# Hydr10n/DirectX-Physically-Based-Raytracer

Hardware: AMD Instinct MI355X
Metric: Mrays/s per GPU + frames/s at 1080p, Cornell Box 4spp/8bounce (higher is better)
Workload: dtype f32

## Files before the change

### directx-physically-based-raytracer_amd/csrc/pt_api.hip

```cpp
#include "pt_internal.hpp"

#include <cmath>
#include <cstdio>
#include <cstring>

using namespace pt;

static thread_local std::string g_createError;
namespace pt { std::string& create_error() { return g_createError; } }

int pt::fail(Context* c, int status, const std::string& msg)
{
    if (c) c->lastError = msg; else g_createError = msg;
    return status;
}
int pt::fail_hip(Context* c, hipError_t e, const char* what)
{
    return fail(c, e == hipErrorOutOfMemory ? PT_ERROR_OUT_OF_MEMORY : PT_ERROR_HIP, std::string(what) + ": " + hipGetErrorString(e));
}

static int poll_tlas_header(Context& c, bool wait);

extern "C" {

// ... 438 lines not shown
        const hipError_t es = hipStreamSynchronize(c.stream);
        if (e == hipSuccess) e = es;
    }
    if (e != hipSuccess) {
        if (newCopy) (void)hipStreamSynchronize(c.stream);
        return fail_hip(&c, e, "top-level build");
    }

    if (newBlob) c.blobDev = std::move(newCopy);
    for (Blas* b : adopting) { b->nodes.reset(); b->tris.reset(); b->idx.reset(); b->inBlob = true; }
    for (const auto& p : P.pieces) if (p.b->inBlob) { p.b->blobNodeAt = P.node_at(p); p.b->blobTriAt = P.tri_at(p); p.b->blobIdxAt = P.idx_at(p); }
    c.tlasHeaderPending = true;
    c.tlasNodeReserve = P.tlasNodeCap;
    SceneRefs& r = c.scene;
    r.instances = c.tlas.instances.data(); r.instanceCount = count; r.triangleCount = P.tris;
    r.blob.base = (const f4v*)c.blobDev.data();
    r.blob.nodeOff16 = (uint32_t)(P.nodeAt / 16); r.blob.triOff16 = (uint32_t)(P.triAt / 16); r.blob.idxOff16 = (uint32_t)(P.idxAt / 16);
    r.blob.instOff16 = (uint32_t)(P.instAt / 16); r.blob.leafInstOff16 = (uint32_t)(P.leafAt / 16); r.blob.enterOff16 = (uint32_t)(P.enterAt / 16);
    r.blob.instCount = count; r.blob.nodeCount = P.blobNodes; r.blob.triCount = P.blobTris; r.blob.bytes = (uint32_t)P.total;
    r.blasTable = dTable; r.blasTableCount = (uint32_t)P.table.size(); r.instSource = dSrc; r.blasTableMaxTris = 0;
    for (const BlasEntry& te : P.table) r.blasTableMaxTris = std::max(r.blasTableMaxTris, te.triCount);
    c.tlasBlasIds = P.pieceIds;
    if (P.objectEnd != c.tlasObjectEnd || count != c.tlasValidatedCount || P.bindingHash != c.tlasBindingHash) c.validated = false;
    c.tlasObjectEnd = P.objectEnd; c.tlasValidatedCount = count; c.tlasBindingHash = P.bindingHash;
    if (P.lightHash != c.tlasLightHash) c.lightListValid = false;
    c.tlasLightHash = P.lightHash;
    c.normalsShared = c.validated && c.sharedVerdict;
    c.haveTlas = true;
    return PT_OK;
}

int pt_share_scene(PtContext* ctx, PtContext* source)
{
    if (!ctx || !source || ctx == source) return PT_ERROR_INVALID_ARGUMENT;
    Context& c = ctx->c; Context& s = source->c;
    API_ARG(&c, c.device == s.device, "both contexts must live on the same device");
    API_ARG(&c, c.viewers.empty(), "other contexts view this context's scene");
    API_ARG(&c, !s.sceneOwner, "the source views another context's scene itself: share from the owner");
    API_HIP(&c, hipSetDevice(c.device));
    API_HIP(&c, hipStreamSynchronize(s.stream));
    API_HIP(&c, hipStreamSynchronize(c.stream));
    int st = poll_tlas_header(s, true);
    if (st != PT_OK) return fail(&c, st, s.lastError);
    if (!s.haveTlas) return fail(&c, PT_ERROR_NOT_READY, "the source context has no top-level acceleration structure");
    if (c.sceneOwner) detach_from_owner(c);
    else { API_HIP(&c, materialise_adopted(c)); c.tlas = Tlas(); c.blobDev.reset(); }
    drop_tlas(c);
    c.scene = s.scene;
    c.tlasObjectEnd = s.tlasObjectEnd; c.maxBlasDepth = s.maxBlasDepth;
    c.heapHost = s.heapHost; c.heapDirty = true;
    c.objects = s.objects; c.objectCount = s.objectCount; c.instanceData = s.instanceData; c.instanceDataCount = s.instanceDataCount;
    c.sceneOwner = &s; s.viewers.push_back(&c);
    c.tlasHeaderPending = false; c.validated = false;
    c.haveTlas = true;
    return PT_OK;
}

int pt_get_accel_stats(PtContext* ctx, PtAccelStats* out)
{
    if (!ctx || !out) return PT_ERROR_INVALID_ARGUMENT;
    Context& c = ctx->c;
    API_HIP(&c, hipSetDevice(c.device));
    API_HIP(&c, hipStreamSynchronize(c.stream));
    int st = poll_tlas_header(c, true);
    if (st != PT_OK) return st;
    memset(out, 0, sizeof *out);
    out->InstanceCount = c.scene.instanceCount;
    out->BottomLevelCount = (uint32_t)c.blas.size();
    out->TriangleCount = c.scene.triangleCount;
    out->NodeSizeBytes = sizeof(WideNode); out->TriangleSizeBytes = sizeof(TriPacket);
    uint64_t nb = (uint64_t)wide_node_capacity(c.scene.instanceCount) * sizeof(WideNode), tb = 0;
    for (auto& kv : c.blas) { nb += (uint64_t)kv.second.nodeCount * sizeof(WideNode); tb += (uint64_t)kv.second.triCount * sizeof(TriPacket); out->MaxBottomLevelDepth = std::max(out->MaxBottomLevelDepth, kv.second.depth); }
    out->BlobBytes = c.sceneOwner ? 0 : c.scene.blob.bytes;
    out->SharedScene = c.sceneOwner ? 1u : 0u;
    out->NormalRecords = c.normalsShared ? 1u : 0u;
    out->RoundObjectsInLds = round_objects_in_lds(c, c.objectCount, (bool)c.shadeGeomDev);
    out->RoundRecordsInLds = round_records_in_lds(c, c.objectCount, (bool)c.shadeGeomDev);
    if (c.tlasHeaderHost && !c.tlasHeaderPending) out->TopLevelDepth = c.tlasHeaderHost.data()->depth;
    out->NodeBytes = nb; out->TriangleBytes = tb;
    for (auto& kv : c.blas) if (!kv.second.inBlob) out->OwnedBottomLevelBytes += (uint64_t)kv.second.nodeCount * sizeof(WideNode) + (uint64_t)kv.second.triCount * (sizeof(TriPacket) + 16);
    return PT_OK;
}

int pt_set_camera(PtContext* ctx, const PtCamera* camera)
{
    if (!ctx) return PT_ERROR_INVALID_ARGUMENT;
    API_ARG(&ctx->c, camera, "camera is NULL");
    ctx->c.camera = *camera; ctx->c.haveCamera = true;
    return PT_OK;
}
int pt_set_scene_data(PtContext* ctx, const PtSceneData* scene_data)
{
    if (!ctx) return PT_ERROR_INVALID_ARGUMENT;
    API_ARG(&ctx->c, scene_data, "scene_data is NULL");
    ctx->c.sceneData = *scene_data; ctx->c.haveSceneData = true;
    return PT_OK;
}
int pt_set_object_data(PtContext* ctx, const PtObjectData* device_objects, uint32_t count)
{
    if (!ctx) return PT_ERROR_INVALID_ARGUMENT;
    API_ARG(&ctx->c, device_objects || count == 0, "device_objects is NULL");
    ctx->c.objects = device_objects; ctx->c.objectCount = count;
    return PT_OK;
}
int pt_invalidate_object_data(PtContext* ctx)
{
    if (!ctx) return PT_ERROR_INVALID_ARGUMENT;
    ctx->c.validated = false; ctx->c.normalsShared = false; ctx->c.sharedVerdict = false;
    ctx->c.objectDataGen++;
    return PT_OK;
}
int pt_set_instance_data(PtContext* ctx, const PtInstanceData* device_instances, uint32_t count)
{
    if (!ctx) return PT_ERROR_INVALID_ARGUMENT;
    ctx->c.instanceData = device_instances; ctx->c.instanceDataCount = count;
    return PT_OK;
}

int pt_set_sharding(PtContext* ctx, const PtSharding* s)
{
    if (!ctx) return PT_ERROR_INVALID_ARGUMENT;
    API_ARG(&ctx->c, s && s->RankCount >= 1 && s->RankIndex < s->RankCount && s->BandHeight >= 1, "invalid sharding");
    ctx->c.sharding = *s;
    return PT_OK;
}

int pt_local_rows(const PtSharding* s, uint32_t frame_height, uint32_t* out_rows)
{
    if (!s || !out_rows || s->RankCount == 0 || s->BandHeight == 0 || s->RankIndex >= s->RankCount) return PT_ERROR_INVALID_ARGUMENT;
    uint32_t rows = 0;
    for (uint32_t b = s->RankIndex; (uint64_t)b * s->BandHeight < frame_height; b += s->RankCount) {
        uint32_t y0 = b * s->BandHeight;
        rows += (frame_height - y0 < s->BandHeight) ? frame_height - y0 : s->BandHeight;
    }
    *out_rows = rows;
    return PT_OK;
}

int pt_deinterleave_bands(PtContext* ctx, void* dst_full, const void* gathered, const uint64_t* rank_offsets_host, uint32_t rank_count,
                          uint32_t band_height, uint32_t width, uint32_t height, uint32_t pixel_bytes)
{
    if (!ctx) return PT_ERROR_INVALID_ARGUMENT;
    Context& c = ctx->c;
    API_ARG(&c, dst_full && gathered && rank_offsets_host && rank_count >= 1 && band_height >= 1, "invalid de-interleave arguments");
    API_ARG(&c, pixel_bytes % 4 == 0, "pixel size must be a multiple of 4 bytes");
    API_HIP(&c, hipSetDevice(c.device));
    API_ARG(&c, rank_count <= 64, "at most 64 ranks");
    hipError_t e = launch_deinterleave(c.stream, dst_full, gathered, rank_offsets_host, rank_count, band_height, width, height, pixel_bytes);
    if (e != hipSuccess) return fail_hip(&c, e, "de-interleave");
    return PT_OK;
}

}

static int validate_scene(Context& c)
{
    if (c.validated && c.validatedObjects == c.objects && c.validatedObjectCount == c.objectCount) return PT_OK;
    const uint32_t heapCount = (uint32_t)c.heapHost.size();
    if (c.tlasObjectEnd > c.objectCount)
        return fail(&c, PT_ERROR_INVALID_ARGUMENT, "InstanceID + geometry count of an instance reaches ObjectData[" + std::to_string(c.tlasObjectEnd - 1)
                    + "] but only " + std::to_string(c.objectCount) + " objects are bound (pt_set_object_data)");
    if (c.instanceData && c.instanceDataCount < c.scene.instanceCount)
        return fail(&c, PT_ERROR_INVALID_ARGUMENT, "InstanceData holds fewer records than the top level has instances");
    uint32_t sharedMismatch = 0;
    if (c.objectCount) {
        API_HIP(&c, c.validateDev.reserve(8));
// ... 274 lines not shown
```

### directx-physically-based-raytracer_amd/csrc/pt_internal.hpp

```cpp
#pragma once
#include <hip/hip_runtime.h>

#include <algorithm>
#include <map>
#include <string>
#include <type_traits>
#include <vector>

#include "../../include/ptamd.h"
#include "pt_memory.hpp"
#include "pt_trace2.hpp"
#include "pt_sharc.hpp"

namespace pt {

struct WideHeader { uint32_t nodeCount, itemCount, depth, error; };

struct TreeBuffers {
    DeviceBuffer<float4> boxLo, boxHi; DeviceBuffer<uint32_t> bounds;
    DeviceBuffer<uint64_t> keys, keysSorted; DeviceBuffer<uint32_t> index, indexSorted;
    DeviceBuffer<uint8_t> sortTemp; size_t sortTempBytes = 0;
    DeviceBuffer<uint64_t> leafKeys; DeviceBuffer<float4> leafLo, leafHi;
    DeviceBuffer<int2> children; DeviceBuffer<int> parentInternal, parentLeaf;
    DeviceBuffer<float4> nodeLo, nodeHi; DeviceBuffer<uint32_t> arrival;
// ... 41 lines not shown

struct SceneView {
    AccelView accel;
    const PtObjectData* objects;
    const ShadeGeom* shadeGeom;
    const HeapEntry* shadeTex;
    const PtInstanceData* instanceData;
    const HeapEntry* heap;
    const float* srgbLut;
    uint32_t objectCount, heapCount;
};

struct FrameView {
    uint32_t width, height;
    uint32_t localRows;
    uint32_t rankIndex, rankCount, bandHeight;
};

struct PathQueue {
    float4* s0;
    float4* s1;
    float4* s2;
    float4* r0;
    float4* r1;
    uint4*  hit;
};

constexpr uint32_t kSubQueueShiftFused = 5, kSubQueueShiftStream = 7, kSubQueuesMax = 1u << kSubQueueShiftStream;

struct FrameConstants { PtCamera cam; PtSceneData sd; PtGraphicsSettings gs; };
struct RoundArgs;

struct DeviceCounters {
    unsigned long long primaryRays, secondaryRays, nodesVisited, trianglesTested;
    unsigned int mismatchCount, stackOverflows;
    float mismatchRay[16];
    unsigned int maxNodesPerRay, _pad2;
};

struct Context {
    int device = 0;
    hipStream_t stream = nullptr;
    std::string lastError;

    std::vector<HeapEntry> heapHost;
    DeviceBuffer<HeapEntry> heapDev; bool heapDirty = true;
    DeviceBuffer<float> srgbLutDev;
    bool heapHasTextures = false;

    std::map<uint64_t, Blas> blas; uint64_t nextBlasId = 1;
    TreeBuffers buildScratch;
    Tlas tlas; bool haveTlas = false;
    DeviceBuffer<uint8_t> blobDev;
    SceneRefs scene;
    Context* sceneOwner = nullptr;
    std::vector<Context*> viewers;
    uint32_t framesInFlight = 1;
    std::vector<uint64_t> tlasBlasIds;
    std::vector<uint8_t> tlasUploadHost; DeviceBuffer<uint8_t> tlasUploadDev;
    struct UploadStage { PinnedBuffer<uint8_t> host; Event event; };
    UploadStage tlasStage[2]; uint32_t tlasStageNext = 0;
    PinnedBuffer<WideHeader> tlasHeaderHost; Event tlasHeaderEvent; bool tlasHeaderPending = false;
    uint32_t maxBlasDepth = 0, tlasNodeReserve = 0;
    uint32_t tlasValidatedCount = ~0u, persistentGrid = 0;
    uint64_t tlasBindingHash = 0;
    uint64_t tlasObjectEnd = 0;
    DeviceBuffer<ShadeGeom> shadeGeomDev;
    DeviceBuffer<HeapEntry> shadeTexDev;
    DeviceBuffer<uint4> shadeRecA; DeviceBuffer<uint32_t> shadeRecB;
    bool normalsShared = false;
    bool sharedVerdict = false;
    bool validated = false; DeviceBuffer<uint32_t> validateDev;
    const void* validatedObjects = nullptr; uint32_t validatedObjectCount = 0;

    PtCamera camera{}; PtSceneData sceneData{}; PtGraphicsSettings settings{};
    bool haveCamera = false, haveSceneData = false, haveSettings = false;
    const PtObjectData* objects = nullptr; uint32_t objectCount = 0;
    const PtInstanceData* instanceData = nullptr; uint32_t instanceDataCount = 0;
    PtSharding sharding{0, 1, 16, 0};

    DeviceBuffer<uint4> queueArrays[2][6];
    PathQueue queue[2]{};
    DeviceBuffer<uint4> primaryRecords;
    DeviceBuffer<float2> pixelAux;
    DeviceBuffer<FrameConstants> frameConstants;
    GraphExec graphExec; std::string graphKey; bool disableGraphs = false;
    static constexpr uint32_t kMaxChains = 4;
    uint32_t chains = 0;
    Stream chainStream[kMaxChains - 1]; Event chainFork, chainJoin[kMaxChains - 1];
    GraphExec chainGraph[kMaxChains]; std::string chainGraphKey;
    DeviceBuffer<uint32_t> queueCounts;
    DeviceBuffer<RoundArgs> roundArgs; std::string roundArgsKey;
    DeviceBuffer<DeviceCounters> counters;
    uint64_t lastIterations = 0;
    uint32_t debugFlags = 0;

    void* comm = nullptr; bool commOwned = false; uint32_t commRank = 0, commWorld = 1;

    bool timing = false;
    std::vector<Event> evExtend, evShade, evRound;
    uint32_t nExtend = 0, nShade = 0, nRound = 0;

    PtDISettings diSettings{}; bool haveDISettings = false;
    uint64_t tlasLightHash = 0;
    uint32_t objectDataGen = 0;
    DeviceBuffer<uint4> lightList; uint32_t lightCount = 0;
    DeviceBuffer<uint32_t> lightInstStart;
    uint64_t lightListKey = 0; bool lightListValid = false;
    DeviceBuffer<PtTriangleLight> lightRecords; DeviceBuffer<float> lightCdf, lightBlockSums; uint32_t lightRecordCount = 0;
    PtDIResamplingSettings diReuse{}; bool diReuseOn = false;
    DeviceBuffer<PtDIReservoir> diResA, diResB;
    DeviceBuffer<int8_t> diOffsets;
    bool diHistoryValid = false; uint32_t diHistorySize[2] = {0, 0}; uint64_t diHistoryLightKey = 0; uint32_t diResCount = 0;
    PtDIVisibilitySettings diVisibility{}; bool diVisibilityOn = false;
    PtDILightSamplingSettings diSampling{};
    DeviceBuffer<PtDIPresampledLight> diTiles, diCells;
    uint32_t diTileCount = 0, diCellCount = 0;

    PtPostProcessSettings post{}; bool havePost = false;
    DeviceBuffer<ushort4> postLevels;
    uint32_t postDims[9][2] = {};
    size_t postOffset[9] = {};

    PtSHARCSettings sharcSettings{}; bool haveSharcSettings = false;
    uint32_t sharcCapacity = 0, sharcParity = 0;
    DeviceBuffer<unsigned long long> sharcKeys;
    DeviceBuffer<uint4> sharcVoxels[2];
    DeviceBuffer<SharcView> sharcView;
    DeviceBuffer<float> sharcRough[2];
    DeviceBuffer<PtSHARCPathScatter> sharcLogScatter;
    DeviceBuffer<PtSHARCPathVertex> sharcLog; uint32_t sharcLogPaths = 0, sharcLogBounces = 0;
};

std::string& create_error();
int fail(Context* c, int status, const std::string& msg);
int fail_hip(Context* c, hipError_t e, const char* what);
#define API_HIP(ctx, expr) do { hipError_t e_ = (expr); if (e_ != hipSuccess) return pt::fail_hip(ctx, e_, #expr); } while (0)
#define API_ARG(ctx, cond, msg) do { if (!(cond)) return pt::fail(ctx, PT_ERROR_INVALID_ARGUMENT, msg); } while (0)
int make_views(Context& c, uint32_t width, uint32_t height, SceneView& sv, FrameView& fv, bool needFrameInputs = true);
int check_raytrace_args(Context& c, const PtTextures* tx);

template <typename T>
int download_counted(Context& c, const T* src, uint32_t count, uint32_t row, T* host_dst, uint32_t capacity, uint32_t* out_count, uint32_t* out_row = nullptr)
{
    API_HIP(&c, hipSetDevice(c.device));
    API_HIP(&c, hipStreamSynchronize(c.stream));
    *out_count = count;
    if (out_row) *out_row = row;
    const size_t n = std::min((size_t)capacity, (size_t)count * row);
    if (n) API_HIP(&c, hipMemcpy(host_dst, src, sizeof(T) * n, hipMemcpyDeviceToHost));
    return PT_OK;
}

template <typename F> void with_flags(F&& f) { f(); }
template <typename F, typename... Rest> void with_flags(F&& f, bool first, Rest... rest)
{
    if (first) with_flags([&](auto... bs) { f(std::true_type{}, bs...); }, rest...);
    else with_flags([&](auto... bs) { f(std::false_type{}, bs...); }, rest...);
}

hipError_t build_blas_device(const PtGeometryDesc* geoms, uint32_t ngeoms, bool allowUpdate, hipStream_t stream, Blas& out);
hipError_t refit_blas_device(const PtGeometryDesc* geoms, uint32_t ngeoms, hipStream_t stream, Blas& b);
hipError_t build_tlas_prepare(Tlas& out, uint32_t n);
hipError_t build_tlas_device(const InstanceRecord* dInstances, const float* const* dBlasBounds, uint32_t n, hipStream_t stream, Tlas& out);
hipError_t launch_instance_records(const InstanceSource* src, const BlasEntry* table, uint32_t n, InstanceRecord* rec, const float** bounds, uint32_t* sceneBounds, hipStream_t stream);
hipError_t launch_blob_assembly(const InstanceRecord* inst, const Tlas& tlas, const BlasEntry* table, uint32_t n, InstanceT* outInst,
                                InstanceT* outLeafInst, const BlobCopy* jobs, uint32_t njobs, f4v* outEnter, hipStream_t stream);
__host__ __device__ void invert_3x4(const float m[12], float out[12]);

hipError_t launch_skin(hipStream_t stream, const void* skeletal, const float* transforms, void* vertices, void* motion, uint32_t count);

struct FramePlan {
    uint32_t rounds, segCap, grid, sqShift;
    bool streaming, fused, first;
    bool flat, lds;
    uint32_t ldsFixed, roundLds, extend2Lds;
    uint32_t objectsInLds, recordsInLds;
    bool recordsUsable;
    bool writeT, stats, di, textured, sharc;
    float2* aux;
    uint32_t nsq() const { return 1u << sqShift; }
    uint32_t cstride() const { return 3u * nsq(); }
};

hipError_t launch_shade(Context& c, const FramePlan& p, const SceneView& sv, const FrameView& fv, const PtTextures& tx, uint32_t round, uint32_t grid, hipStream_t stream,
                        uint32_t sqBase, uint32_t sqCount);
hipError_t launch_extend_stream(Context& c, const FramePlan& p, const AlphaContext& ac, uint32_t round, hipStream_t stream, uint32_t sqBase, uint32_t sqCount);

hipError_t launch_gbuffer(Context& c, const SceneView& sv, const FrameView& fv, uint32_t flags, const PtTextures& tx);
hipError_t launch_raytrace(Context& c, const SceneView& sv, const FrameView& fv, const PtTextures& tx, bool sharcQuery);
hipError_t launch_visibility(Context& c, const SceneView& sv, const void* rays, uint32_t count, void* out);
hipError_t launch_bsdf_evaluate(hipStream_t stream, const float* q, uint32_t count, float* r);
hipError_t launch_bsdf_sample(hipStream_t stream, const float* q, uint32_t count, float* r);
hipError_t launch_debug_trace(Context& c, const SceneView& sv, const float* ray8, uint32_t* devLog, uint32_t logCap);
hipError_t launch_debug_closest(Context& c, const SceneView& sv, const void* rays, uint32_t count, void* hits);
uint32_t round_objects_in_lds(const Context& c, uint32_t objectCount, bool haveShadeGeom);
uint32_t round_records_in_lds(const Context& c, uint32_t objectCount, bool haveShadeGeom);
inline bool normal_records_usable(const Context& c) { return c.normalsShared && c.scene.blasTable && c.scene.blasTableCount <= 65535u  && c.shadeRecB && c.scene.blob.triCount && c.scene.blob.triCount <= c.shadeRecB.capacity(); }
hipError_t launch_check_shared_geometry(hipStream_t stream, const InstanceSource* src, const BlasEntry* table, uint32_t n, const ShadeGeom* shadeGeom, uint32_t* out);
hipError_t launch_validate_objects(hipStream_t stream, const PtObjectData* objects, uint32_t count, const HeapEntry* heap, uint32_t heapCount, uint32_t* out, ShadeGeom* shadeGeom, HeapEntry* shadeTex);
hipError_t launch_deinterleave(hipStream_t stream, void* dst, const void* src, const uint64_t* rankOffsetsHost, uint32_t rankCount,
                               uint32_t bandHeight, uint32_t width, uint32_t height, uint32_t pixelBytes);

}

struct PtContext { pt::Context c; };
```

### directx-physically-based-raytracer_amd/csrc/pt_kernels.hip

```cpp
#include "pt_internal.hpp"

#include <cstring>

#include "pt_shade.hpp"

namespace pt {

template <bool STATS, bool TEXTURED, int MODE>
__global__ __launch_bounds__(256) void k_gbuffer(SceneView sv, FrameView fv, PtCamera cam, PtSceneData sd, uint32_t flags, PtTextures tx,
                                                 BlobView bv, DeviceCounters* counters)
{
    const uint32_t wv = threadIdx.x >> 6, ln = threadIdx.x & 63u;
    const uint32_t x = blockIdx.x * 16 + (wv & 1u) * 8u + (ln & 7u), ly = blockIdx.y * 16 + (wv >> 1) * 8u + (ln >> 3);
    const bool valid = x < fv.width && ly < fv.localRows;
    if (MODE == 0 && !valid) return;
    const uint32_t y = global_row(fv, valid ? ly : 0u);
    const size_t pi = (size_t)ly * fv.width + x;

    float4 Position = make_float4(INFINITY, INFINITY, INFINITY, INFINITY);
    float LinearDepth = INFINITY, NormalizedDepth = cam.IsNormalizedDepthReversed ? 0.0f : 1.0f;
    float u, v;
    const RayDesc ray = generate_pinhole_ray(cam, valid ? x : 0u, y, fv.width, fv.height, u, v);
    TraceStats st; st.nodes = 0; st.tris = 0; st.overflow = 0;
    Hit hit;
// ... 45 lines not shown
            float proj[4]; xform4(cam.WorldToProjection, h.Position, proj);
            LinearDepth = proj[3];
            NormalizedDepth = proj[2] / proj[3];
            if ((flags & PT_GB_MotionVector) && tx.MotionVector) {
                v3 prev = h.Position;
                if (!sd.IsStatic && sv.instanceData) {
                    const float* P = sv.instanceData[h.InstanceIndex].PreviousObjectToWorld; v3 q = h.ObjectPosition;
                    const PtMeshDescriptors md = sv.objects[h.ObjectIndex].MeshDescriptors;
                    if (md.MotionVectors != ~0u) {
                        const PT_GLOBAL_AS uint16_t* mvb = gptr<uint16_t>(sv.heap[md.MotionVectors].ptr);
                        const HeapEntry ib = sv.heap[md.Indices];
                        v3 m3[3];
                        for (int kk = 0; kk < 3; kk++) {
                            const uint32_t vi = load_index_dev(ib.ptr, ib.stride, 3 * h.PrimitiveIndex + kk);
                            m3[kk] = V3(f16_to_f32(mvb[4 * (size_t)vi]), f16_to_f32(mvb[4 * (size_t)vi + 1]), f16_to_f32(mvb[4 * (size_t)vi + 2]));
                        }
                        q = q + interp3(m3[0], m3[1], m3[2], hit.u, hit.v);
                    }
                    prev = V3(sop3t(P[0], q.x, P[1], q.y, P[2], q.z, P[3]), sop3t(P[4], q.x, P[5], q.y, P[6], q.z, P[7]), sop3t(P[8], q.x, P[9], q.y, P[10], q.z, P[11]));
                }
                float clip[4], view[4];
                xform4(cam.PreviousWorldToProjection, prev, clip);
                xform4(cam.PreviousWorldToView, prev, view);
                float su = (clip[0] / clip[3]) * 0.5f + 0.5f, svv = (clip[1] / clip[3]) * -0.5f + 0.5f;
                ushort4 mv = make_ushort4(f32_to_f16((su - u) * (float)fv.width), f32_to_f16((svv - v) * (float)fv.height), f32_to_f16(view[2] - LinearDepth), 0);
                ((ushort4*)tx.MotionVector)[pi] = mv;
            }
        }
        BSDFSample bs; bs.Roughness = 0.0f;
        if (flags & PT_GB_Material) {
            const PtMaterial m = surface_material<TEXTURED>(sv, h);
            bs.Initialize(V3(m.BaseColor), m.Metallic, m.Roughness, m.IOR, m.Transmission, h.IsFrontFace);
            if (tx.BaseColorMetalness)
                ((uchar4*)tx.BaseColorMetalness)[pi] = make_uchar4(f32_to_unorm8(bs.BaseColor.x), f32_to_unorm8(bs.BaseColor.y), f32_to_unorm8(bs.BaseColor.z), f32_to_unorm8(bs.Metallic));
            if (flags & PT_GB_Albedo) {
                const float NoV = fabsf(dot(h.ShadingNormal, -ray.d));
                const v3 Fe = ml_env_term_rtg(bs.F0, NoV, bs.Roughness);
                if ((flags & PT_GB_DiffuseAlbedo) && tx.DiffuseAlbedo)
                    ((ushort4*)tx.DiffuseAlbedo)[pi] = make_ushort4(f32_to_f16((1.0f - Fe.x) * bs.Albedo.x * 0.99f + 0.01f), f32_to_f16((1.0f - Fe.y) * bs.Albedo.y * 0.99f + 0.01f),
                                                                     f32_to_f16((1.0f - Fe.z) * bs.Albedo.z * 0.99f + 0.01f), 0);
                if ((flags & PT_GB_SpecularAlbedo) && tx.SpecularAlbedo)
                    ((ushort4*)tx.SpecularAlbedo)[pi] = make_ushort4(f32_to_f16(Fe.x * 0.99f + 0.01f), f32_to_f16(Fe.y * 0.99f + 0.01f), f32_to_f16(Fe.z * 0.99f + 0.01f), 0);
            }
            if (tx.IOR) ((uint16_t*)tx.IOR)[pi] = f32_to_f16(m.IOR);
            if (bs.Metallic < 1.0f && tx.Transmission) ((uint8_t*)tx.Transmission)[pi] = f32_to_unorm8(bs.Transmission);
            if ((flags & PT_GB_Radiance) && tx.Radiance) {
                v3 e = material_emission(m);
                ((ushort4*)tx.Radiance)[pi] = make_ushort4(f32_to_f16(e.x), f32_to_f16(e.y), f32_to_f16(e.z), 0);
            }
        }
        if ((flags & PT_GB_NormalRoughness) && tx.NormalRoughness) {
            float r = (flags & PT_GB_Material) ? bs.Roughness : 0.0f;
            ((short4*)tx.NormalRoughness)[pi] = make_short4(f32_to_snorm16(h.ShadingNormal.x), f32_to_snorm16(h.ShadingNormal.y), f32_to_snorm16(h.ShadingNormal.z), f32_to_snorm16(r));
        }
    } else {
        if ((flags & PT_GB_MotionVector) && tx.MotionVector) {
            v3 far = ray.o + ray.d * 1e8f;
            float proj[4], clip[4], view[4];
            xform4(cam.WorldToProjection, far, proj);
            xform4(cam.PreviousWorldToProjection, far, clip);
            xform4(cam.PreviousWorldToView, far, view);
            float su = (clip[0] / clip[3]) * 0.5f + 0.5f, svv = (clip[1] / clip[3]) * -0.5f + 0.5f;
            ((ushort4*)tx.MotionVector)[pi] = make_ushort4(f32_to_f16((su - u) * (float)fv.width), f32_to_f16((svv - v) * (float)fv.height), f32_to_f16(view[2] - proj[3]), 0);
        }
        if ((flags & PT_GB_Radiance) && tx.Radiance) {
            v3 e = environment_light_color(sv, sd, ray.d);
            ((ushort4*)tx.Radiance)[pi] = make_ushort4(f32_to_f16(e.x), f32_to_f16(e.y), f32_to_f16(e.z), 0);
        }
    }
    if ((flags & PT_GB_Position) && tx.Position) ((float4*)tx.Position)[pi] = Position;
    if ((flags & PT_GB_LinearDepth) && tx.LinearDepth) ((float*)tx.LinearDepth)[pi] = LinearDepth;
    if ((flags & PT_GB_NormalizedDepth) && tx.NormalizedDepth) ((float*)tx.NormalizedDepth)[pi] = NormalizedDepth;
}

__global__ void k_set_constants(FrameConstants v, FrameConstants* dst, uint32_t* queueCounts, uint32_t countWords)
{
    const uint32_t* s = (const uint32_t*)&v; uint32_t* d = (uint32_t*)dst;
    for (uint32_t i = threadIdx.x; i < sizeof(FrameConstants) / 4; i += blockDim.x) d[i] = s[i];
    for (uint32_t i = threadIdx.x; i < countWords; i += blockDim.x) queueCounts[i] = 0u;
}


__global__ __launch_bounds__(256) void k_pt_init(FrameView fv, const FrameConstants* __restrict__ fc, PtTextures tx, PathQueue q, float2* aux, uint32_t segCap, uint32_t* countFresh,
                                                 uint4* __restrict__ primary, uint32_t sqShift)
{
    __shared__ uint32_t lds[8];
    const PtGraphicsSettings& gs = fc->gs;
    const uint32_t npix = fv.width * fv.localRows;
    const uint32_t nsq = 1u << sqShift, sq = blockIdx.x & (nsq - 1u), bq = blockIdx.x >> sqShift, nbq = gridDim.x >> sqShift;
    for (uint32_t j = bq; (j * nsq + sq) * 256u < npix; j += nbq) {
        const uint32_t p = (j * nsq + sq) * 256u + threadIdx.x;
        bool alive = false;
        if (p < npix) alive = isfinite(((const float*)tx.Position)[4 * (size_t)p + 3]);
        const uint32_t slot = sq * segCap + (segCap - 1u - block_reserve(alive, &countFresh[sq], lds));
        if (alive) {
            const uint32_t x = p % fv.width, y = global_row(fv, p / fv.width);
            q.s0[slot] = make_float4(1.0f, 1.0f, 1.0f, __uint_as_float(p));
            q.s1[slot] = make_float4(0.0f, 0.0f, 0.0f, __uint_as_float(rng_init(x, y, gs.FrameIndex)));
            q.s2[slot] = make_float4(0.0f, 0.0f, 0.0f, __uint_as_float(0u));
            if (aux) aux[p] = make_float2(INFINITY, 1.0f);
            const uint2 nr = ((const uint2*)tx.NormalRoughness)[p], rad = ((const uint2*)tx.Radiance)[p];
            primary[3 * (size_t)p] = ((const uint4*)tx.Position)[p];
            primary[3 * (size_t)p + 1] = make_uint4(nr.x, nr.y, ((const uint32_t*)tx.FlatNormal)[p], ((const uint32_t*)tx.GeometricNormal)[p]);
            primary[3 * (size_t)p + 2] = make_uint4(((const uint32_t*)tx.BaseColorMetalness)[p], rad.x, rad.y,
                                                    (uint32_t)((const uint16_t*)tx.IOR)[p] | ((uint32_t)((const uint8_t*)tx.Transmission)[p] << 16));
        }
    }
}

template <bool DI, bool SHARC = false>
__global__ __launch_bounds__(256) void k_pt_first(FrameView fv, const FrameConstants* __restrict__ fc, PtTextures tx, PathQueue qout, float2* aux,
                                                                                             uint32_t segCap, uint32_t* countOut, uint4* __restrict__ primary, uint32_t sqShift,
                                                                                             float* roughOut = nullptr)
{
    __shared__ uint32_t lds[32];
    uint32_t emits = 0;
    const PtCamera& cam = fc->cam; const PtGraphicsSettings& gs = fc->gs;
    const uint32_t npix = fv.width * fv.localRows;
    const uint32_t nsq = 1u << sqShift, sq = blockIdx.x & (nsq - 1u), bq = blockIdx.x >> sqShift, nbq = gridDim.x >> sqShift;
    const uint32_t seg = sq * segCap;
    for (uint32_t j = bq; (j * nsq + sq) * 256u < npix; j += nbq) {
        const uint32_t pix = (j * nsq + sq) * 256u + threadIdx.x;
        bool alive = false;
        if (pix < npix) alive = isfinite(((const float*)tx.Position)[4 * (size_t)pix + 3]);
        bool toTraced = false, toFresh = false;
        PathRegs p; p.thr = V3(1.0f, 1.0f, 1.0f); p.srad = V3(0, 0, 0); p.rsum = V3(0, 0, 0); p.pixel = pix; p.rng = 0; p.sample = 0; p.bounce = 0;
        v3 newO = V3(0, 0, 0), newD = V3(0, 0, 1);
        float pr = 0.0f;
        if (alive) {
            const uint32_t x = pix % fv.width, y = global_row(fv, pix / fv.width);
            p.rng = rng_init(x, y, gs.FrameIndex);
            if (aux) aux[pix] = make_float2(INFINITY, 1.0f);
            const uint2 nr = ((const uint2*)tx.NormalRoughness)[pix], rad = ((const uint2*)tx.Radiance)[pix];
            const uint4 r0 = ((const uint4*)tx.Position)[pix];
            const uint4 r1 = make_uint4(nr.x, nr.y, ((const uint32_t*)tx.FlatNormal)[pix], ((const uint32_t*)tx.GeometricNormal)[pix]);
            const uint4 r2 = make_uint4(((const uint32_t*)tx.BaseColorMetalness)[pix], rad.x, rad.y,
                                        (uint32_t)((const uint16_t*)tx.IOR)[pix] | ((uint32_t)((const uint8_t*)tx.Transmission)[pix] << 16));
            primary[3 * (size_t)pix] = r0; primary[3 * (size_t)pix + 1] = r1; primary[3 * (size_t)pix + 2] = r2;
            shade_fresh_record<DI, SHARC>(fv, cam, gs, tx, aux, r0, r1, r2, p, toTraced, toFresh, newO, newD, &pr);
        }
        emit_tile<SHARC>(qout, seg, segCap, &countOut[sq], &countOut[nsq + sq], lds + ((emits++ & 1u) << 4), toTraced, toFresh, p, newO, newD, roughOut, pr);
    }
}

__global__ __launch_bounds__(256) void k_extend_brute(AccelView av, BlobView bv, AlphaContext ac, PathQueue q, uint32_t segCap, const uint32_t* count, DeviceCounters* counters, uint32_t sqShift)
{
    const uint32_t nsq = 1u << sqShift, sq = blockIdx.x & (nsq - 1u), bq = blockIdx.x >> sqShift, nbq = gridDim.x >> sqShift;
    const uint32_t n = count[sq];
    if (bq == 0 && threadIdx.x == 0) atomicAdd(&counters->secondaryRays, (unsigned long long)n);
    __shared__ uint2 ldsStack[kLdsStackDepth * 256];
    uint2 spill[kStackSize - kLdsStackDepth];
    GroupStack<kLdsStackDepth> stack; stack.init((PT_LDS_AS void*)ldsStack, spill);
    BlobReader<false> blob; blob.p = bv.base;
    TraceStats st; st.nodes = 0; st.tris = 0; st.overflow = 0;
    for (uint32_t local = bq * 256u + threadIdx.x; local < n; local += nbq * 256u) {
        const uint32_t i = sq * segCap + local;
        const float4 o = q.r0[i], d = q.r1[i];
        const Hit h = trace_brute_force(av, ac, V3(o.x, o.y, o.z), V3(d.x, d.y, d.z), o.w, d.w);
        const Hit b = trace_single<false, false, false>(blob, bv, ac, V3(o.x, o.y, o.z), V3(d.x, d.y, d.z), o.w, d.w, stack, &st, nullptr);
        if (b.inst != h.inst || (h.inst != ~0u && (b.slot != h.slot || b.u != h.u || b.v != h.v))) {
            if (atomicAdd(&counters->mismatchCount, 1u) == 0u) {
                float* m = counters->mismatchRay;
                m[0] = o.x; m[1] = o.y; m[2] = o.z; m[3] = o.w; m[4] = d.x; m[5] = d.y; m[6] = d.z; m[7] = d.w;
                m[8] = __uint_as_float(b.inst); m[9] = __uint_as_float(b.slot); m[10] = b.t; m[11] = 0.0f;
                m[12] = __uint_as_float(h.inst); m[13] = __uint_as_float(h.slot); m[14] = h.t; m[15] = 0.0f;
            }
        }
        q.hit[i] = make_uint4(h.inst, h.slot, __float_as_uint(h.u), __float_as_uint(h.v));
    }
    if (st.overflow) atomicAdd(&counters->stackOverflows, st.overflow);
}

constexpr int kStackLds2 = 8;
constexpr uint32_t kStackLds2Bytes = (uint32_t)kStackLds2 * 256u * 8u;
constexpr uint32_t kExtendLdsFixed = kStackLds2Bytes + (uint32_t)kCandidates * 256u * 4u + 4u * kPhasedWaveLds;
constexpr uint32_t kBlobLdsMax = 40u * 1024u;

template <bool STATS, bool LDS, bool WRITE_T = false, bool FLAT = false>
__global__ __launch_bounds__(256) void k_extend2(BlobView bv, AlphaContext ac, PathQueue q, uint32_t segCap, const uint32_t* count, DeviceCounters* counters, uint32_t sqShift)
{
    extern __shared__ __attribute__((aligned(16))) unsigned char smem[];
    constexpr uint32_t kFixed = FLAT ? kFlatLdsFixed : kExtendLdsFixed;
    const uint32_t nsq = 1u << sqShift, sq = blockIdx.x & (nsq - 1u), bq = blockIdx.x >> sqShift, nbq = gridDim.x >> sqShift;
    const uint32_t n = count[sq];
    if (bq == 0 && threadIdx.x == 0) atomicAdd(&counters->secondaryRays, (unsigned long long)n);
    if (bq * 256u >= n) return;
    PT_LDS_AS void* ldsStack = (PT_LDS_AS void*)smem;
    BlobReader<LDS> blob;
    if constexpr (LDS) {
        f4v* dst = (f4v*)(smem + kFixed);
        const uint32_t n16 = bv.bytes / 16u;
        for (uint32_t i = threadIdx.x; i < n16; i += 256u) dst[i] = bv.base[i];
        __syncthreads();
        blob.p = (const PT_LDS_AS f4v*)(smem + kFixed);
    } else {
        blob.p = bv.base;
    }
    TraceStats st; st.nodes = 0; st.tris = 0; st.overflow = 0;
    if constexpr (FLAT) {
        unsigned char* ldsWave = smem + (uint32_t)kStackLdsFlat * 256u * 8u + (threadIdx.x >> 6) * kFlatWaveLds;
        for (uint32_t base = bq * 256u; base < n; base += nbq * 256u) {
            const uint32_t local = base + threadIdx.x;
            const bool valid = local < n;
            const uint32_t i = sq * segCap + (valid ? local : base);
            float4 o = q.r0[i], d = q.r1[i];
            if (!valid) { o.w = 1.0f; d.w = 0.0f; }
            const Hit h = trace_closest_flat<STATS, LDS>(blob, bv, ac, V3(o.x, o.y, o.z), V3(d.x, d.y, d.z), o.w, d.w, ldsStack, ldsWave, &st);
            if (valid) {
                q.hit[i] = make_uint4(h.inst, h.slot, __float_as_uint(h.u), __float_as_uint(h.v));
                if (WRITE_T) q.r1[i].w = h.t;
            }
        }
    } else {
        uint32_t* ldsCand = (uint32_t*)(smem + kStackLds2Bytes);
        unsigned char* ldsWave = smem + kStackLds2Bytes + (uint32_t)kCandidates * 256u * 4u + (threadIdx.x >> 6) * kPhasedWaveLds;
        for (uint32_t base = bq * 256u; base < n; base += nbq * 256u) {
            const uint32_t local = base + threadIdx.x;
            const bool valid = local < n;
            const uint32_t i = sq * segCap + (valid ? local : base);
            float4 o = q.r0[i], d = q.r1[i];
            if (!valid) { o.w = 1.0f; d.w = 0.0f; }
            const Hit h = trace_closest_v2<STATS, LDS, kStackLds2>(blob, bv, ac, V3(o.x, o.y, o.z), V3(d.x, d.y, d.z), o.w, d.w, ldsStack, ldsCand, ldsWave, &st);
            if (valid) {
                q.hit[i] = make_uint4(h.inst, h.slot, __float_as_uint(h.u), __float_as_uint(h.v));
                if (WRITE_T) q.r1[i].w = h.t;
            }
        }
    }
    if (STATS) { atomicAdd(&counters->nodesVisited, (unsigned long long)st.nodes); atomicAdd(&counters->trianglesTested, (unsigned long long)st.tris); }
    if (st.overflow) atomicAdd(&counters->stackOverflows, st.overflow);
}

struct RoundArgs {
    SceneView sv; FrameView fv; PtTextures tx; BlobView bv; PathQueue qin, qout;
    const FrameConstants* fc; float2* aux; const uint32_t* countIn; uint32_t* countOut; DeviceCounters* counters; uint32_t segCap;
    uint32_t objectsInLds;
    const uint4* recA; const uint32_t* recB;
    uint32_t recordsInLds, sqShift;
    const uint4* primary;
    const SharcView* sharc; const float* roughIn; float* roughOut;
};

template <bool TEXTURED, bool LDS, bool FLAT, bool DI, bool SHARC = false>
__global__ __launch_bounds__(256) __attribute__((amdgpu_waves_per_eu(4, 4))) void k_round(const RoundArgs* __restrict__ A, uint32_t sqBase, uint32_t sqCount)
{
    const SceneView& sv = A->sv; const FrameView& fv = A->fv; const PtTextures& tx = A->tx; const BlobView& bv = A->bv;
    const PathQueue& qin = A->qin; const PathQueue& qout = A->qout;
    const FrameConstants* __restrict__ fc = A->fc; float2* aux = A->aux; const uint32_t segCap = A->segCap;
    const uint32_t* countIn = A->countIn; uint32_t* countOut = A->countOut; DeviceCounters* counters = A->counters;
    const uint4* __restrict__ primary = A->primary;
    extern __shared__ __attribute__((aligned(16))) unsigned char smem[];
    __shared__ uint32_t lds[32];
    uint32_t emits = 0;
    constexpr uint32_t kFixed = FLAT ? kFlatLdsFixed : kExtendLdsFixed;
    const PtCamera& cam = fc->cam; const PtSceneData& sd = fc->sd; const PtGraphicsSettings& gs = fc->gs;
    const uint32_t sqShift = A->sqShift;
    const uint32_t nsq = 1u << sqShift, bq = blockIdx.x / sqCount, sq = sqBase + (blockIdx.x - bq * sqCount), nbq = gridDim.x / sqCount;
    const uint32_t nT = countIn[sq], nF = countIn[nsq + sq];
    const uint32_t seg = sq * segCap;
    if (bq == 0 && threadIdx.x == 0) atomicAdd(&counters->secondaryRays, (unsigned long long)nT);

#ifdef PT_ROUND_PROF
    RoundProf profData; RoundProf* prof = &profData;
    for (int k = 0; k < 16; k++) profData.acc[k] = 0;
    profData.last = __builtin_readcyclecounter();
#else
    RoundProf* prof = nullptr;
#endif
    if (bq * 256u < nT) {
        PT_LDS_AS void* ldsStack = (PT_LDS_AS void*)smem;
        BlobReader<LDS> blob;
        ShadeTables tables;
        tables.recA = A->recA; tables.recB = A->recB;
        if constexpr (LDS) {
            f4v* dst = (f4v*)(smem + kFixed);
            const uint32_t n16 = bv.bytes / 16u;
            for (uint32_t k = threadIdx.x; k < n16; k += 256u) dst[k] = bv.base[k];
            const uint32_t nobj = A->objectsInLds;
            for (uint32_t k = threadIdx.x; k < nobj * kObjLds16; k += 256u) {
                const uint32_t o = k / kObjLds16, part = k - o * kObjLds16;
                dst[n16 + k] = part < 2u ? ((const f4v*)&sv.shadeGeom[o])[part] : ((const f4v*)&sv.objects[o].Material)[part - 2u];
            }
            const uint32_t nrec = A->recordsInLds, recBase = n16 + nobj * kObjLds16;
            for (uint32_t k = threadIdx.x; k < nrec; k += 256u) {
                const uint4 a = A->recA[k];
                dst[recBase + k] = (f4v){ __uint_as_float(a.x), __uint_as_float(a.y), __uint_as_float(a.z), __uint_as_float(a.w) };
                ((uint32_t*)(dst + recBase + nrec))[k] = A->recB[k];
            }
            __syncthreads();
            blob.p = (const PT_LDS_AS f4v*)(smem + kFixed);
            if (nobj) tables.objects = (ObjectTableLds)(smem + kFixed) + n16;
            if (nrec) { tables.recALds = (const PT_LDS_AS f4v*)(smem + kFixed) + recBase; tables.recBLds = (const PT_LDS_AS uint32_t*)((const PT_LDS_AS f4v*)(smem + kFixed) + recBase + nrec); }
        } else {
            blob.p = bv.base;
        }
        const AlphaContext ac = alpha_context(sv);
        TraceStats st; st.nodes = 0; st.tris = 0; st.overflow = 0;
        for (uint32_t base = bq * 256u; base < nT; base += nbq * 256u) {
            const uint32_t local = base + threadIdx.x;
            const bool valid = local < nT;
            const uint32_t i = seg + (valid ? local : base);
            float4 o = qin.r0[i], d = qin.r1[i];
            PathRegs p = load_path(qin, i);
            float pr = 0.0f;
            if constexpr (SHARC) pr = A->roughIn[i];
            if (!valid) { o.w = 1.0f; d.w = 0.0f; }
            PT_PROF_MARK(prof, 0);
            Hit h;
            if constexpr (FLAT) {
                unsigned char* ldsWave = smem + (uint32_t)kStackLdsFlat * 256u * 8u + (threadIdx.x >> 6) * kFlatWaveLds;
                h = trace_closest_flat<false, LDS>(blob, bv, ac, V3(o.x, o.y, o.z), V3(d.x, d.y, d.z), o.w, d.w, ldsStack, ldsWave, &st, prof);
            } else {
                uint32_t* ldsCand = (uint32_t*)(smem + kStackLds2Bytes);
                unsigned char* ldsWave = smem + kStackLds2Bytes + (uint32_t)kCandidates * 256u * 4u + (threadIdx.x >> 6) * kPhasedWaveLds;
                h = trace_closest_v2<false, LDS, kStackLds2>(blob, bv, ac, V3(o.x, o.y, o.z), V3(d.x, d.y, d.z), o.w, d.w, ldsStack, ldsCand, ldsWave, &st);
            }
            bool toTraced = false, toFresh = false;
            v3 newO = V3(0, 0, 0), newD = V3(0, 0, 1);
            if (valid) {
                shade_traced<TEXTURED, DI, SHARC>(sv, GeometryFromBlob<LDS>{ blob, bv, tables }, sd, gs, tx, aux, p, make_uint4(h.inst, h.slot, __float_as_uint(h.u), __float_as_uint(h.v)), h.t,
                                       V3(d.x, d.y, d.z), toTraced, toFresh, newO, newD, prof, A->sharc, &pr);
            }
            PT_PROF_MARK(prof, 6);
            emit_tile<SHARC>(qout, seg, segCap, &countOut[sq], &countOut[nsq + sq], lds + ((emits++ & 1u) << 4), toTraced, toFresh, p, newO, newD, A->roughOut, pr);
            PT_PROF_MARK(prof, 7);
#ifdef PT_ROUND_PROF
            prof->acc[11] += 1u;
#endif
        }
        if (st.overflow) atomicAdd(&counters->stackOverflows, st.overflow);
    }
    for (uint32_t tile = bq; tile * 256u < nF; tile += nbq) {
        const uint32_t local = tile * 256u + threadIdx.x;
        bool toTraced = false, toFresh = false;
        PathRegs p; v3 newO = V3(0, 0, 0), newD = V3(0, 0, 1);
        float pr = 0.0f;
        if (local < nF) {
            p = load_path(qin, seg + (segCap - 1u - local));
            PT_PROF_WAIT(); PT_PROF_MARK(prof, 12);
            shade_fresh<DI, SHARC>(fv, cam, gs, tx, aux, primary, p, toTraced, toFresh, newO, newD, prof, &pr);
        }
        PT_PROF_MARK(prof, 14);
        emit_tile<SHARC>(qout, seg, segCap, &countOut[sq], &countOut[nsq + sq], lds + ((emits++ & 1u) << 4), toTraced, toFresh, p, newO, newD, A->roughOut, pr);
        PT_PROF_MARK(prof, 15);
    }
#ifdef PT_ROUND_PROF
    PT_PROF_MARK(prof, 8);
    if ((threadIdx.x & 63u) == 0u) for (int k = 0; k < 16; k++) atomicAdd((unsigned int*)&counters->mismatchRay[k], (k < 9 || k >= 12) ? (prof->acc[k] >> 6) : prof->acc[k]);
#endif
}

template <bool STATS>
__global__ __launch_bounds__(256) void k_extend(BlobView bv, AlphaContext ac, PathQueue q, uint32_t segCap, const uint32_t* count, DeviceCounters* counters, uint32_t sqShift)
{
    const uint32_t nsq = 1u << sqShift, sq = blockIdx.x & (nsq - 1u), bq = blockIdx.x >> sqShift, nbq = gridDim.x >> sqShift;
    const uint32_t n = count[sq];
    if (bq == 0 && threadIdx.x == 0) atomicAdd(&counters->secondaryRays, (unsigned long long)n);
    __shared__ uint2 ldsStack[kLdsStackDepth * 256];
    uint2 spill[kStackSize - kLdsStackDepth];
    GroupStack<kLdsStackDepth> stack; stack.init((PT_LDS_AS void*)ldsStack, spill);
    BlobReader<false> blob; blob.p = bv.base;
    TraceStats st; st.nodes = 0; st.tris = 0; st.overflow = 0;
    for (uint32_t local = bq * 256u + threadIdx.x; local < n; local += nbq * 256u) {
        const uint32_t i = sq * segCap + local;
        const float4 o = q.r0[i], d = q.r1[i];
        const Hit h = trace_single<STATS, false, false>(blob, bv, ac, V3(o.x, o.y, o.z), V3(d.x, d.y, d.z), o.w, d.w, stack, &st, nullptr);
        q.hit[i] = make_uint4(h.inst, h.slot, __float_as_uint(h.u), __float_as_uint(h.v));
    }
    if (STATS) { atomicAdd(&counters->nodesVisited, (unsigned long long)st.nodes); atomicAdd(&counters->trianglesTested, (unsigned long long)st.tris); }
    if (st.overflow) atomicAdd(&counters->stackOverflows, st.overflow);
}

static uint32_t persistent_grid(Context& c);

__global__ __launch_bounds__(256) void k_visibility(BlobView bv, AlphaContext ac, const float4* __restrict__ rays, uint32_t count, float4* __restrict__ out,
                                                    DeviceCounters* counters)
{
    __shared__ uint2 ldsStack[kLdsStackDepth * 256];
    uint2 spill[kStackSize - kLdsStackDepth];
    GroupStack<kLdsStackDepth> stack; stack.init((PT_LDS_AS void*)ldsStack, spill);
    BlobReader<false> blob; blob.p = bv.base;
    TraceStats st; st.nodes = 0; st.tris = 0; st.overflow = 0;
    for (uint32_t i = blockIdx.x * blockDim.x + threadIdx.x; i < count; i += gridDim.x * blockDim.x) {
        const float4 o = rays[2 * (size_t)i], d = rays[2 * (size_t)i + 1];
        v3 vis;
        const Hit h = trace_single<false, false, true>(blob, bv, ac, V3(o.x, o.y, o.z), V3(d.x, d.y, d.z), o.w, d.w, stack, &st, &vis);
        out[i] = make_float4(vis.x, vis.y, vis.z, h.inst == ~0u ? 1.0f : 0.0f);
    }
    if (st.overflow) atomicAdd(&counters->stackOverflows, st.overflow);
}

__global__ __launch_bounds__(256) void k_debug_trace(BlobView bv, AlphaContext ac, float4 o, float4 d, uint32_t* log, uint32_t logCap)
{
    __shared__ uint2 ldsStack[kLdsStackDepth * 256];
    uint2 spill[kStackSize - kLdsStackDepth];
    GroupStack<kLdsStackDepth> stack; stack.init((PT_LDS_AS void*)ldsStack, spill);
    BlobReader<false> blob; blob.p = bv.base;
    TraceStats st; st.nodes = 0; st.tris = 0; st.overflow = 0;
    const float a = 0.02f * (float)threadIdx.x, ca = cosf(a), sa = sinf(a);
    const v3 dd = V3(d.x * ca - d.z * sa, d.y, d.x * sa + d.z * ca);
    trace_single<false, false, false, GroupStack<kLdsStackDepth>, true>(blob, bv, ac, V3(o.x, o.y, o.z), dd, o.w, d.w, stack, &st, nullptr, log, threadIdx.x == 0 ? logCap : 0u);
}

hipError_t launch_debug_trace(Context& c, const SceneView& sv, const float* ray8, uint32_t* devLog, uint32_t logCap)
{
    k_debug_trace<<<1, 256, 0, c.stream>>>(c.scene.blob, alpha_context(sv), make_float4(ray8[0], ray8[1], ray8[2], ray8[3]), make_float4(ray8[4], ray8[5], ray8[6], ray8[7]), devLog, logCap);
    return hipGetLastError();
}

template <bool BRUTE>
__global__ __launch_bounds__(256) void k_debug_closest(AccelView av, BlobView bv, AlphaContext ac, const float4* __restrict__ rays, uint32_t count, uint4* __restrict__ out,
                                                       DeviceCounters* counters)
{
    __shared__ uint2 ldsStack[kLdsStackDepth * 256];
    uint2 spill[kStackSize - kLdsStackDepth];
    GroupStack<kLdsStackDepth> stack; stack.init((PT_LDS_AS void*)ldsStack, spill);
    BlobReader<false> blob; blob.p = bv.base;
    TraceStats st; st.nodes = 0; st.tris = 0; st.overflow = 0;
    for (uint32_t i = blockIdx.x * blockDim.x + threadIdx.x; i < count; i += gridDim.x * blockDim.x) {
        const float4 o = rays[2 * (size_t)i], d = rays[2 * (size_t)i + 1];
        const Hit h = BRUTE ? trace_brute_force(av, ac, V3(o.x, o.y, o.z), V3(d.x, d.y, d.z), o.w, d.w)
                            : trace_single<false, false, false>(blob, bv, ac, V3(o.x, o.y, o.z), V3(d.x, d.y, d.z), o.w, d.w, stack, &st, nullptr);
        out[2 * (size_t)i] = make_uint4(__float_as_uint(h.t), __float_as_uint(h.u), __float_as_uint(h.v), h.inst);
// ... 117 lines not shown
    const bool ok = b.Sample(sv, V, w, rnd, L, lobe);
    float pdf = 0.0f; v3 f = V3(0.0f, 0.0f, 0.0f);
    if (ok) b.EvaluateLobe(sv, L, V, w, lobe, ext, pdf, f);
    float* o = r + 12 * (size_t)i;
    o[0] = L.x; o[1] = L.y; o[2] = L.z; o[3] = pdf; o[4] = f.x; o[5] = f.y; o[6] = f.z; o[7] = w[0]; o[8] = w[1]; o[9] = w[2];
    o[10] = __uint_as_float((uint32_t)lobe); o[11] = __uint_as_float(ok ? 1u : 0u);
}

hipError_t launch_visibility(Context& c, const SceneView& sv, const void* rays, uint32_t count, void* out)
{
    if (!count) return hipSuccess;
    k_visibility<<<persistent_grid(c), 256, 0, c.stream>>>(c.scene.blob, alpha_context(sv), (const float4*)rays, count, (float4*)out, c.counters.data());
    return hipGetLastError();
}

hipError_t launch_debug_closest(Context& c, const SceneView& sv, const void* rays, uint32_t count, void* hits)
{
    if (!count) return hipSuccess;
    if (c.debugFlags & PT_DEBUG_BRUTE_FORCE)
        k_debug_closest<true><<<persistent_grid(c), 256, 0, c.stream>>>(sv.accel, c.scene.blob, alpha_context(sv), (const float4*)rays, count, (uint4*)hits, c.counters.data());
    else
        k_debug_closest<false><<<persistent_grid(c), 256, 0, c.stream>>>(sv.accel, c.scene.blob, alpha_context(sv), (const float4*)rays, count, (uint4*)hits, c.counters.data());
    return hipGetLastError();
}

hipError_t launch_bsdf_evaluate(hipStream_t stream, const float* q, uint32_t count, float* r)
{
    if (!count) return hipSuccess;
    k_bsdf_evaluate<<<(count + 255) / 256, 256, 0, stream>>>(q, count, r);
    return hipGetLastError();
}

hipError_t launch_bsdf_sample(hipStream_t stream, const float* q, uint32_t count, float* r)
{
    if (!count) return hipSuccess;
    k_bsdf_sample<<<(count + 255) / 256, 256, 0, stream>>>(q, count, r);
    return hipGetLastError();
}


struct RankOffsets { uint64_t v[64]; };

__global__ void k_deinterleave(uint8_t* dst, const uint8_t* src, RankOffsets rankOffsets, uint32_t rankCount, uint32_t bandHeight,
                               uint32_t width, uint32_t height, uint32_t pixelBytes)
{
    const uint64_t rowBytes = (uint64_t)width * pixelBytes, chunks = rowBytes / 4;
    const uint64_t total = chunks * height;
    for (uint64_t t = (uint64_t)blockIdx.x * blockDim.x + threadIdx.x; t < total; t += (uint64_t)gridDim.x * blockDim.x) {
        const uint32_t y = (uint32_t)(t / chunks); const uint64_t cx = t % chunks;
        const uint32_t band = y / bandHeight, rank = band % rankCount, localRow = (band / rankCount) * bandHeight + (y - band * bandHeight);
        ((uint32_t*)(dst + (uint64_t)y * rowBytes))[cx] = ((const uint32_t*)(src + rankOffsets.v[rank] + (uint64_t)localRow * rowBytes))[cx];
    }
}

static uint32_t persistent_grid(Context& c)
{
    if (!c.persistentGrid) {
        hipDeviceProp_t p;
        const uint32_t g = hipGetDeviceProperties(&p, c.device) == hipSuccess ? (uint32_t)p.multiProcessorCount * 8u : 1024u;
        c.persistentGrid = (g + kSubQueuesMax - 1) / kSubQueuesMax * kSubQueuesMax;
    }
    return c.persistentGrid;
}

static bool gbuffer_flat(const Context& c)
{
    return c.scene.blob.base && c.scene.blob.instCount <= kFlatInstances &&
           !(c.debugFlags & (PT_DEBUG_TRAVERSAL_V1 | PT_DEBUG_TRAVERSAL_PHASED | PT_DEBUG_BRUTE_FORCE));
}

hipError_t launch_gbuffer(Context& c, const SceneView& sv, const FrameView& fv, uint32_t flags, const PtTextures& tx)
{
    if (fv.localRows == 0 || fv.width == 0) return hipSuccess;
    dim3 grid((fv.width + 15) / 16, (fv.localRows + 15) / 16);
    const int mode = !gbuffer_flat(c) ? 0 : (c.scene.blob.bytes <= kBlobLdsMax ? 1 : 2);
    const uint32_t smem = mode == 0 ? 0u : kFlatLdsFixed + (mode == 1 ? c.scene.blob.bytes : 0u);
    with_flags([&](auto S, auto T) {
        auto launch = [&](auto M) { k_gbuffer<S(), T(), M()><<<grid, 256, smem, c.stream>>>(sv, fv, c.camera, c.sceneData, flags, tx, c.scene.blob, c.counters.data()); };
        if (mode == 0) launch(std::integral_constant<int, 0>{}); else if (mode == 1) launch(std::integral_constant<int, 1>{}); else launch(std::integral_constant<int, 2>{});
    }, (c.debugFlags & PT_DEBUG_TRAVERSAL_STATS) != 0, c.heapHasTextures);
    return hipGetLastError();
}

static hipError_t ensure_queues(Context& c, uint32_t capacity, uint32_t iterations)
{
    hipError_t e = hipSuccess;
    for (auto& arrays : c.queueArrays) for (auto& a : arrays) if (e == hipSuccess) e = a.reserve(capacity);
    for (int k = 0; k < 2; k++) {
        DeviceBuffer<uint4>* a = c.queueArrays[k];
        c.queue[k] = PathQueue{ (float4*)a[0].data(), (float4*)a[1].data(), (float4*)a[2].data(), (float4*)a[3].data(), (float4*)a[4].data(), a[5].data() };
    }
    if (e != hipSuccess) return e;
    if ((e = c.primaryRecords.reserve(3 * (size_t)capacity)) != hipSuccess) return e;
    return c.queueCounts.reserve(iterations);
}

static void timing_begin(Context& c, std::vector<Event>& ev, uint32_t k)
{
    if (!c.timing) return;
    while (ev.size() < 2 * (size_t)(k + 1)) { hipEvent_t e; hipEventCreate(&e); ev.emplace_back(e); }
    hipEventRecord(ev[2 * k].get(), c.stream);
}
static void timing_end(Context& c, std::vector<Event>& ev, uint32_t k) { if (c.timing) hipEventRecord(ev[2 * k + 1].get(), c.stream); }

static uint32_t lds_bytes_of_records(uint32_t n) { return (n * 20u + 15u) / 16u * 16u; }
static uint32_t round_lds_bytes(bool flat, uint32_t blobBytes, uint32_t objects, uint32_t records)
{
    return (flat ? kFlatLdsFixed : kExtendLdsFixed) + blobBytes + objects * kObjLds16 * 16u + lds_bytes_of_records(records);
}
static bool round_lds_fits(uint32_t bytes) { return (bytes + 128u + 511u) / 512u * 512u <= 160u * 1024u / 4u; }
static bool lockstep_flat(const Context& c) { return c.scene.blob.instCount <= kFlatInstances && !(c.debugFlags & PT_DEBUG_TRAVERSAL_PHASED); }

uint32_t round_objects_in_lds(const Context& c, uint32_t objectCount, bool haveShadeGeom)
{
    if (c.scene.blob.bytes > kBlobLdsMax || !objectCount || !haveShadeGeom) return 0u;
    return round_lds_fits(round_lds_bytes(lockstep_flat(c), c.scene.blob.bytes, objectCount, 0u)) ? objectCount : 0u;
}
uint32_t round_records_in_lds(const Context& c, uint32_t objectCount, bool haveShadeGeom)
{
    const uint32_t nobj = round_objects_in_lds(c, objectCount, haveShadeGeom);
    if (!nobj || !normal_records_usable(c)) return 0u;
    return round_lds_fits(round_lds_bytes(lockstep_flat(c), c.scene.blob.bytes, nobj, c.scene.blob.triCount)) ? c.scene.blob.triCount : 0u;
}

static void plan_frame(FramePlan& p, Context& c, const SceneView& sv, const FrameView& fv, bool sharcQuery)
{
    std::memset(&p, 0, sizeof p);
    const PtGraphicsSettings& gs = c.settings;
    const uint32_t tiles = (fv.width * fv.localRows + 255u) / 256u;
    p.rounds = gs.SamplesPerPixel * (gs.Bounces + 1u);
    p.lds = c.scene.blob.bytes <= kBlobLdsMax;
    p.sqShift = p.lds ? kSubQueueShiftFused : kSubQueueShiftStream;
    p.segCap = (tiles + p.nsq() - 1) / p.nsq() * 256u;
    p.grid = std::min(persistent_grid(c), (tiles + p.nsq() - 1) / p.nsq() * p.nsq());
    const uint32_t lockStepFlags = PT_DEBUG_LOCKSTEP | PT_DEBUG_TRAVERSAL_PHASED | PT_DEBUG_BRUTE_FORCE | PT_DEBUG_TRAVERSAL_V1 | PT_DEBUG_UNFUSED_ROUNDS;
    const uint32_t pairOnlyFlags = PT_DEBUG_TRAVERSAL_STATS | PT_DEBUG_BRUTE_FORCE | PT_DEBUG_TRAVERSAL_V1 | PT_DEBUG_UNFUSED_ROUNDS;
    p.streaming = !p.lds && !(c.debugFlags & lockStepFlags);
    p.fused = !p.streaming && !(c.debugFlags & pairOnlyFlags);
    p.first = p.streaming || p.fused;
    p.flat = lockstep_flat(c);
    p.ldsFixed = p.flat ? kFlatLdsFixed : kExtendLdsFixed;
    p.recordsUsable = normal_records_usable(c);
    p.objectsInLds = round_objects_in_lds(c, sv.objectCount, sv.shadeGeom != nullptr);
    p.recordsInLds = round_records_in_lds(c, sv.objectCount, sv.shadeGeom != nullptr);
    p.extend2Lds = round_lds_bytes(p.flat, p.lds ? c.scene.blob.bytes : 0u, 0u, 0u);
    p.roundLds = round_lds_bytes(p.flat, p.lds ? c.scene.blob.bytes : 0u, p.objectsInLds, p.recordsInLds);
    p.aux = gs.Denoiser != PT_DENOISER_NONE ? c.pixelAux.data() : nullptr;
    p.sharc = sharcQuery;
    p.writeT = p.aux != nullptr || p.sharc;
    p.stats = (c.debugFlags & PT_DEBUG_TRAVERSAL_STATS) != 0;
    p.di = gs.IsDIEnabled != 0u;
    p.textured = c.heapHasTextures;
}

constexpr uint32_t kStreamingChains = 3;
static uint32_t frame_chains(const Context& c, const FramePlan& p, bool ownStreams)
{
    if (!p.first) return 1u;
    const uint32_t choice = (p.streaming && c.framesInFlight <= 1) ? kStreamingChains : 1u;
    const uint32_t want = c.chains ? c.chains : (ownStreams ? choice : 1u);
    return std::max(1u, std::min({ want, Context::kMaxChains, p.nsq() }));
}

static hipError_t enqueue_preamble(Context& c, const FramePlan& p, const SceneView& sv, const FrameView& fv, const PtTextures& tx)
{
    if (p.recordsUsable)
        k_capture_normals<<<dim3(std::min((c.scene.blasTableMaxTris + 255u) / 256u, 64u), c.scene.blasTableCount), 256, 0, c.stream>>>(c.scene.blasTable, sv.shadeGeom, c.shadeRecA.data(), c.shadeRecB.data());
    if (p.first)
        with_flags([&](auto S, auto D) {
            k_pt_first<D(), S()><<<p.grid, 256, 0, c.stream>>>(fv, c.frameConstants.data(), tx, c.queue[1], p.aux, p.segCap, &c.queueCounts.data()[p.cstride()], c.primaryRecords.data(), p.sqShift, c.sharcRough[1].data());
        }, p.sharc, p.di);
    else k_pt_init<<<p.grid, 256, 0, c.stream>>>(fv, c.frameConstants.data(), tx, c.queue[0], p.aux, p.segCap, &c.queueCounts.data()[p.nsq()], c.primaryRecords.data(), p.sqShift);
    return hipGetLastError();
}

static hipError_t enqueue_chain(Context& c, const FramePlan& p, const SceneView& sv, const FrameView& fv, const PtTextures& tx, uint32_t g, uint32_t chains, hipStream_t s)
{
    const uint32_t nsq = p.nsq(), perSq = std::max(1u, p.grid / nsq);
    const uint32_t sqBase = (uint32_t)((uint64_t)nsq * g / chains), sqCount = (uint32_t)((uint64_t)nsq * (g + 1) / chains) - sqBase;
    if (p.streaming) {
        const AlphaContext ac = alpha_context(sv);
        for (uint32_t r = 0; r <= p.rounds; r++) {
            if (r > 0) {
                timing_begin(c, c.evShade, c.nShade);
                launch_shade(c, p, sv, fv, tx, r, perSq * sqCount, s, sqBase, sqCount);
                timing_end(c, c.evShade, c.nShade); c.nShade++;
            }
            if (r == p.rounds) break;
            timing_begin(c, c.evExtend, c.nExtend);
            launch_extend_stream(c, p, ac, r, s, sqBase, sqCount);
            timing_end(c, c.evExtend, c.nExtend); c.nExtend++;
        }
        return hipGetLastError();
    }
    for (uint32_t r = 1; r <= p.rounds; r++) {
        timing_begin(c, c.evRound, c.nRound);
        with_flags([&](auto T, auto L, auto F, auto D, auto S) {
            k_round<T(), L(), F(), D(), S()><<<perSq * sqCount, 256, p.roundLds, s>>>(c.roundArgs.data() + r, sqBase, sqCount);
        }, p.textured, p.lds, p.flat, p.di, p.sharc);
        timing_end(c, c.evRound, c.nRound); c.nRound++;
    }
    return hipGetLastError();
}

static hipError_t enqueue_validation_rounds(Context& c, const FramePlan& p, const SceneView& sv, const FrameView& fv, const PtTextures& tx)
{
    const AlphaContext ac = alpha_context(sv);
    for (uint32_t r = 0; r <= p.rounds; r++) {
        PathQueue& qout = c.queue[(r + 1) & 1];
        uint32_t* cout = &c.queueCounts.data()[(r + 1) * p.cstride()];
        timing_begin(c, c.evShade, c.nShade);
        launch_shade(c, p, sv, fv, tx, r, p.grid, c.stream, 0u, p.nsq());
        timing_end(c, c.evShade, c.nShade); c.nShade++;
        if (r == p.rounds) break;
        timing_begin(c, c.evExtend, c.nExtend);
        if (c.debugFlags & PT_DEBUG_BRUTE_FORCE) k_extend_brute<<<p.grid, 256, 0, c.stream>>>(sv.accel, c.scene.blob, ac, qout, p.segCap, cout, c.counters.data(), p.sqShift);
        else if (c.debugFlags & PT_DEBUG_TRAVERSAL_V1)
            with_flags([&](auto S) { k_extend<S()><<<p.grid, 256, 0, c.stream>>>(c.scene.blob, ac, qout, p.segCap, cout, c.counters.data(), p.sqShift); }, p.stats);
        else
            with_flags([&](auto S, auto L, auto W, auto F) {
                k_extend2<S(), L(), W(), F()><<<p.grid, 256, p.extend2Lds, c.stream>>>(c.scene.blob, ac, qout, p.segCap, cout, c.counters.data(), p.sqShift);
            }, p.stats, p.lds, p.writeT, p.flat);
        timing_end(c, c.evExtend, c.nExtend); c.nExtend++;
    }
    return hipGetLastError();
}

static hipError_t enqueue_frame(Context& c, const FramePlan& p, const SceneView& sv, const FrameView& fv, const PtTextures& tx, uint32_t chains)
{
    hipError_t e = enqueue_preamble(c, p, sv, fv, tx);
    if (e != hipSuccess) return e;
    if (!p.first) return enqueue_validation_rounds(c, p, sv, fv, tx);
    for (uint32_t g = 0; g < chains && e == hipSuccess; g++) e = enqueue_chain(c, p, sv, fv, tx, g, chains, c.stream);
    return e;
}

template <typename T> static void key_add(std::string& k, const T& v) { k.append((const char*)&v, sizeof v); }

hipError_t launch_raytrace(Context& c, const SceneView& sv, const FrameView& fv, const PtTextures& tx, bool sharcQuery)
{
    const PtGraphicsSettings& gs = c.settings;
    const uint32_t npix = fv.width * fv.localRows;
    c.lastIterations = 0;
    if (c.normalsShared && c.scene.blasTable && c.scene.blob.triCount > c.shadeRecB.capacity()) {
        hipError_t ea = hipStreamSynchronize(c.stream);
        if (ea != hipSuccess) return ea;
        c.shadeRecA.reset(); c.shadeRecB.reset();
        if ((ea = c.shadeRecA.reserve(c.scene.blob.triCount)) != hipSuccess) return ea;
        if ((ea = c.shadeRecB.reserve(c.scene.blob.triCount)) != hipSuccess) return ea;
    }
    if (npix == 0 || gs.SamplesPerPixel == 0) return hipSuccess;
    hipError_t e;
    if (gs.Denoiser != PT_DENOISER_NONE && (e = c.pixelAux.reserve(npix)) != hipSuccess) return e;
    FramePlan plan; plan_frame(plan, c, sv, fv, sharcQuery);
    const FramePlan& p = plan;
    const uint32_t rounds = p.rounds, nsq = p.nsq(), cstride = p.cstride();
    if ((e = ensure_queues(c, p.segCap * nsq, (rounds + 2) * cstride)) != hipSuccess) return e;
    if ((e = c.frameConstants.reserve(1)) != hipSuccess) return e;
    if (p.sharc) for (auto& a : c.sharcRough) if ((e = a.reserve((size_t)p.segCap * nsq)) != hipSuccess) return e;
    FrameConstants fc; fc.cam = c.camera; fc.sd = c.sceneData; fc.gs = c.settings;
    k_set_constants<<<1, 256, 0, c.stream>>>(fc, c.frameConstants.data(), c.queueCounts.data(), (rounds + 2u) * cstride);
    c.lastIterations = rounds + 1;

    std::string key;
    key_add(key, sv); key_add(key, fv); key_add(key, tx); key_add(key, plan);
    key_add(key, c.queue[0]); key_add(key, c.queue[1]); key_add(key, c.queueCounts.data()); key_add(key, c.scene.blob);
    key_add(key, c.frameConstants.data()); key_add(key, c.primaryRecords.data()); key_add(key, c.stream); key_add(key, c.pixelAux.data()); key_add(key, gs.Denoiser); key_add(key, c.debugFlags);
    key_add(key, c.framesInFlight); key_add(key, c.chains);
    key_add(key, c.sharcView.data()); key_add(key, c.sharcRough[0].data()); key_add(key, c.sharcRough[1].data());
    key_add(key, c.shadeRecA.data()); key_add(key, c.scene.blasTable); key_add(key, c.scene.blasTableCount); key_add(key, c.scene.blasTableMaxTris);
    if (key != c.roundArgsKey || !c.roundArgs.data()) {
        if ((e = c.roundArgs.reserve(rounds + 1)) != hipSuccess) return e;
        std::vector<RoundArgs> host(rounds + 1);
        for (uint32_t r = 0; r <= rounds; r++) {
            RoundArgs& a = host[r];
            std::memset(&a, 0, sizeof a);
            a.sv = sv; a.fv = fv; a.tx = tx; a.bv = c.scene.blob; a.qin = c.queue[r & 1]; a.qout = c.queue[(r + 1) & 1];
            a.fc = c.frameConstants.data(); a.aux = p.aux; a.countIn = &c.queueCounts.data()[r * cstride]; a.countOut = &c.queueCounts.data()[(r + 1) * cstride]; a.sqShift = p.sqShift;
            a.counters = c.counters.data(); a.segCap = p.segCap; a.primary = c.primaryRecords.data(); a.objectsInLds = p.objectsInLds;
            if (p.recordsUsable) { a.recA = c.shadeRecA.data(); a.recB = c.shadeRecB.data(); a.recordsInLds = p.recordsInLds; }
            if (p.sharc) { a.sharc = c.sharcView.data(); a.roughIn = c.sharcRough[r & 1].data(); a.roughOut = c.sharcRough[(r + 1) & 1].data(); }
        }
        if ((e = hipMemcpyAsync(c.roundArgs.data(), host.data(), sizeof(RoundArgs) * (rounds + 1), hipMemcpyHostToDevice, c.stream)) != hipSuccess) return e;
        if ((e = hipStreamSynchronize(c.stream)) != hipSuccess) return e;
        c.roundArgsKey = key;
    }

    const bool graphable = c.stream != nullptr && !c.timing && !c.disableGraphs &&
                           (c.debugFlags & ~(PT_DEBUG_UNFUSED_ROUNDS | PT_DEBUG_TRAVERSAL_PHASED | PT_DEBUG_LOCKSTEP | PT_DEBUG_GATHER_LOCAL_ONLY | PT_DEBUG_GATHER_SELF_EXCHANGE | PT_DEBUG_SHARC_LOG_PATHS | PT_DEBUG_SHARC_SKIP_UPDATE)) == 0;
    auto capture = [&](hipStream_t s, GraphExec& exec, auto&& body) -> hipError_t {
        if (exec) { hipStreamSynchronize(c.stream); exec.reset(); }
        hipGraph_t graph = nullptr;
        hipError_t ce = hipStreamBeginCapture(s, hipStreamCaptureModeRelaxed);
        if (ce == hipSuccess) {
            const hipError_t e2 = body();
            ce = hipStreamEndCapture(s, &graph);
            if (ce == hipSuccess) ce = e2;
        }
        hipGraphExec_t ge = nullptr;
        if (ce == hipSuccess) ce = hipGraphInstantiate(&ge, graph, nullptr, nullptr, 0);
        if (graph) hipGraphDestroy(graph);
        if (ce == hipSuccess) exec.reset(ge); else (void)hipGetLastError();
        return ce;
    };
    const uint32_t chains = frame_chains(c, p, graphable);
    if (graphable && chains > 1) {
        if (!c.chainFork && (e = create_event(c.chainFork, hipEventDisableTiming)) != hipSuccess) return e;
        for (uint32_t g = 1; g < chains; g++) {
            if (!c.chainStream[g - 1] && (e = create_stream(c.chainStream[g - 1], hipStreamNonBlocking)) != hipSuccess) return e;
            if (!c.chainJoin[g - 1] && (e = create_event(c.chainJoin[g - 1], hipEventDisableTiming)) != hipSuccess) return e;
        }
        if (key != c.chainGraphKey) {
            c.chainGraphKey.clear();
            for (uint32_t g = 0; g < chains; g++) {
                hipStream_t s = g == 0 ? c.stream : c.chainStream[g - 1].get();
                if (capture(s, c.chainGraph[g], [&] { return enqueue_chain(c, p, sv, fv, tx, g, chains, s); }) != hipSuccess) { c.disableGraphs = true; break; }
            }
            if (!c.disableGraphs) c.chainGraphKey = key;
        }
        if (!c.disableGraphs) {
            if ((e = enqueue_preamble(c, p, sv, fv, tx)) != hipSuccess) return e;
            if ((e = hipEventRecord(c.chainFork.get(), c.stream)) != hipSuccess) return e;
            for (uint32_t g = 1; g < chains; g++) {
                hipStream_t s = c.chainStream[g - 1].get();
                if ((e = hipStreamWaitEvent(s, c.chainFork.get(), 0)) != hipSuccess) return e;
                if ((e = hipGraphLaunch(c.chainGraph[g].get(), s)) != hipSuccess) return e;
                if ((e = hipEventRecord(c.chainJoin[g - 1].get(), s)) != hipSuccess) return e;
            }
            if ((e = hipGraphLaunch(c.chainGraph[0].get(), c.stream)) != hipSuccess) return e;
            for (uint32_t g = 1; g < chains; g++) if ((e = hipStreamWaitEvent(c.stream, c.chainJoin[g - 1].get(), 0)) != hipSuccess) return e;
            return hipSuccess;
        }
    } else if (graphable) {
        if (key != c.graphKey || !c.graphExec) {
            c.graphKey.clear();
            if (capture(c.stream, c.graphExec, [&] { return enqueue_frame(c, p, sv, fv, tx, 1u); }) != hipSuccess) c.disableGraphs = true;
            else c.graphKey = key;
        }
        if (c.graphExec) return hipGraphLaunch(c.graphExec.get(), c.stream);
    }
    return enqueue_frame(c, p, sv, fv, tx, frame_chains(c, p, false));
}

hipError_t launch_deinterleave(hipStream_t stream, void* dst, const void* src, const uint64_t* rankOffsetsHost, uint32_t rankCount,
                               uint32_t bandHeight, uint32_t width, uint32_t height, uint32_t pixelBytes)
{
    RankOffsets ro;
    for (uint32_t r = 0; r < 64; r++) ro.v[r] = r < rankCount ? rankOffsetsHost[r] : 0;
    k_deinterleave<<<1024, 256, 0, stream>>>((uint8_t*)dst, (const uint8_t*)src, ro, rankCount, bandHeight, width, height, pixelBytes);
    return hipGetLastError();
}

}
```

### directx-physically-based-raytracer_amd/csrc/pt_math.hpp

```cpp
#pragma once
#include <hip/hip_runtime.h>
#include <stdint.h>

namespace pt {

struct v3 { float x, y, z; };

#define PT_DEV __device__ __forceinline__

PT_DEV v3 V3(float x, float y, float z) { v3 r; r.x = x; r.y = y; r.z = z; return r; }
PT_DEV v3 V3(const float* p) { return V3(p[0], p[1], p[2]); }
PT_DEV v3 operator+(v3 a, v3 b) { return V3(a.x + b.x, a.y + b.y, a.z + b.z); }
PT_DEV v3 operator-(v3 a, v3 b) { return V3(a.x - b.x, a.y - b.y, a.z - b.z); }
PT_DEV v3 operator*(v3 a, v3 b) { return V3(a.x * b.x, a.y * b.y, a.z * b.z); }
PT_DEV v3 operator*(v3 a, float s) { return V3(a.x * s, a.y * s, a.z * s); }
PT_DEV v3 operator-(v3 a) { return V3(-a.x, -a.y, -a.z); }
PT_DEV v3 vabs(v3 a) { return V3(fabsf(a.x), fabsf(a.y), fabsf(a.z)); }
PT_DEV float mad(float a, float b, float c) { return __builtin_fmaf(a, b, c); }
PT_DEV float sop3(float a0, float b0, float a1, float b1, float a2, float b2) { return mad(a2, b2, mad(a1, b1, a0 * b0)); }
PT_DEV float sop3t(float a0, float b0, float a1, float b1, float a2, float b2, float t) { return mad(a2, b2, mad(a1, b1, mad(a0, b0, t))); }
PT_DEV float dot(v3 a, v3 b) { return sop3(a.x, b.x, a.y, b.y, a.z, b.z); }
PT_DEV v3 cross(v3 a, v3 b) { return V3(mad(a.y, b.z, -(a.z * b.y)), mad(a.z, b.x, -(a.x * b.z)), mad(a.x, b.y, -(a.y * b.x))); }
PT_DEV v3 madd(v3 a, float s, v3 b) { return V3(mad(a.x, s, b.x), mad(a.y, s, b.y), mad(a.z, s, b.z)); }
PT_DEV v3 madd(v3 a, v3 s, v3 b) { return V3(mad(a.x, s.x, b.x), mad(a.y, s.y, b.y), mad(a.z, s.z, b.z)); }
// ... 170 lines not shown
    float FdL = mad(f, ml_pow5_01(1.0f - NoL), 1.0f);
    return PT_DIV_CONST(FdV * FdL, kPi);
}
PT_DEV v3 ml_env_term_rtg(v3 F0, float NoV, float roughness)
{
    float m = roughness * roughness;
    float X1 = NoV, X2 = NoV * NoV, X3 = NoV * X2;
    float Y1 = m, Y3 = m * (m * m);
    float b0 = mad(-1.28514f, X1, 0.99044f);
    float b1 = mad(-0.755907f, X1, 1.29678f);
    float bn = mad(b1, Y1, b0);
    float c0 = mad(59.4188f, X3, mad(2.92338f, X1, 1.0f));
    float c1 = mad(222.592f, X3, mad(-27.0302f, X1, 20.3225f));
    float c2 = mad(316.627f, X3, mad(626.13f, X1, 121.563f));
    float bd = mad(c2, Y3, mad(c1, Y1, c0));
    float bias = bn * ml_positive_rcp(bd);
    float s0 = mad(3.32707f, X1, 0.0365463f);
    float s1 = mad(-9.04756f, X1, 9.0632f);
    float sn = mad(s1, Y1, s0);
    float d0 = mad(-1.36772f, X3, mad(3.59685f, X2, 1.0f));
    float d1 = mad(9.22949f, X3, mad(-16.3174f, X2, 9.04401f));
    float d2 = mad(-20.2123f, X3, mad(19.7886f, X2, 5.56589f));
    float sd = mad(d2, Y3, mad(d1, Y1, d0));
    float scale = sn * ml_positive_rcp(sd);
    return V3(saturate(mad(F0.x, scale, bias)), saturate(mad(F0.y, scale, bias)), saturate(mad(F0.z, scale, bias)));
}
PT_DEV v3 ml_vndf_get_ray(float u0, float u1, float roughness, v3 Vl)
{
    float m = roughness * roughness;
    v3 Vh = normalize(V3(m * Vl.x, m * Vl.y, Vl.z));
    float s, c; sincos_2pi(u0, s, c);
    float z = mad(1.0f - u1, 1.0f + Vh.z, -Vh.z);
    float sinT = ml_sqrt01(mad(-z, z, 1.0f));
    v3 h = V3(mad(sinT, c, Vh.x), mad(sinT, s, Vh.y), z + Vh.z);
    return normalize(V3(m * h.x, m * h.y, fmaxf(h.z, 0.0f)));
}
PT_DEV float ml_vndf_pdf(v3 Vl, float NoH, float roughness)
{
    float m = roughness * roughness;
    float D = ml_distribution_ggx(roughness, NoH);
    float ax = m * Vl.x, ay = m * Vl.y;
    float len2 = mad(ay, ay, ax * ax);
    float t = sqrtf(mad(Vl.z, Vl.z, len2));
    if (Vl.z >= 0.0f) return D / (2.0f * (Vl.z + t));
    return D * (t - Vl.z) / (2.0f * len2);
}
PT_DEV float ml_from_srgb1(float x)
{
    x = saturate(x);
    return x >= 0.04045f ? powf(x * (1.0f / 1.055f) + (0.055f / 1.055f), 2.4f) : x * (1.0f / 12.92f);
}

struct SurfaceVectors {
    v3 FrontGeometricNormal, ShadingNormal;
    basis3 ShadingBasis;
};
PT_DEV SurfaceVectors surface_vectors(bool isFront, v3 geometricNormal, v3 shadingNormal)
{
    SurfaceVectors sv;
    sv.FrontGeometricNormal = isFront ? geometricNormal : -geometricNormal;
    sv.ShadingNormal = shadingNormal;
    sv.ShadingBasis = ml_get_basis(shadingNormal);
    return sv;
}

constexpr float kMinRoughness = 2e-3f;
enum : int { LOBE_DIFFUSE = 0, LOBE_SPECULAR = 1, LOBE_TRANSMISSION = 2 };
constexpr uint32_t kExtLambertianOnly = 0x1u;

struct BSDFSample {
    v3 BaseColor; float Metallic; v3 Albedo; float Roughness, IORi, IORo; v3 F0; float Transmission;

    PT_DEV void Initialize(v3 baseColor, float metallic, float roughness, float IOR, float transmission, bool isFrontFace)
    {
        BaseColor = baseColor;
        Metallic = metallic;
        Albedo = baseColor * (1.0f - metallic);
        Roughness = fmaxf(kMinRoughness, roughness);
        IORi = 1.0f; IORo = IOR;
        if (!isFrontFace) { IORi = IOR; IORo = 1.0f; }
        float r = (IORi - IORo) / (IORi + IORo);
        float r2 = r * r;
        F0 = V3(mad(metallic, baseColor.x - r2, r2), mad(metallic, baseColor.y - r2, r2), mad(metallic, baseColor.z - r2, r2));
        Transmission = transmission;
    }

    PT_DEV float EstimateDiffuseProbability(float NoV) const
    {
        v3 Fenv = ml_env_term_rtg(F0, NoV, Roughness);
        float diffuse = ml_luminance(Albedo * V3(1.0f - Fenv.x, 1.0f - Fenv.y, 1.0f - Fenv.z));
        float specular = ml_luminance(Fenv);
        float sum = diffuse + specular;
        float p = sum > 0.0f ? diffuse / sum : 1.0f;
        if (0.0f < p && p < 1.0f) return clampf(p, 0.05f, 0.95f);
        return p;
    }

    PT_DEV void ComputeLobeWeights(const SurfaceVectors& sv, v3 V, uint32_t ext, float w[3]) const
    {
        if (ext & kExtLambertianOnly) { w[0] = 1.0f; w[1] = 0.0f; w[2] = 0.0f; return; }
        float NoV = fabsf(dot(sv.ShadingNormal, V));
        float tw = Transmission * (1.0f - Metallic);
        float rw = 1.0f - tw;
        float dw = EstimateDiffuseProbability(NoV);
        float sw = 1.0f - dw;
        w[LOBE_DIFFUSE] = dw * rw;
        w[LOBE_SPECULAR] = sw * rw;
        w[LOBE_TRANSMISSION] = tw;
    }

    PT_DEV static v3 reflect(v3 i, v3 n) { float d = dot(n, i); return madd(n, -(2.0f * d), i); }
    PT_DEV static v3 refract(v3 i, v3 n, float eta)
    {
        float d = dot(n, i);
        float k = mad(-(eta * eta), mad(-d, d, 1.0f), 1.0f);
        if (k < 0.0f) return V3(0.0f, 0.0f, 0.0f);
        float s = mad(eta, d, sqrtf(k));
        return madd(n, -s, i * eta);
    }

    PT_DEV bool Sample(const SurfaceVectors& sv, v3 V, const float w[3], const float rnd[4], v3& L, int& lobe) const
    {
        lobe = 0;
        {
            float weight = w[2];
            if (rnd[0] < weight) lobe = 2;
            else { weight += w[1]; if (rnd[0] < weight) lobe = 1; }
        }
        if (lobe == LOBE_DIFFUSE) {
            L = rotate_vector_inv(sv.ShadingBasis, ml_cosine_get_ray(rnd[1], rnd[2]));
            return dot(sv.FrontGeometricNormal, L) > 0.0f;
        }
        v3 Vlocal = rotate_vector(sv.ShadingBasis, V);
        v3 H = rotate_vector_inv(sv.ShadingBasis, ml_vndf_get_ray(rnd[1], rnd[2], Roughness, Vlocal));
        if (lobe == LOBE_SPECULAR) {
            L = reflect(-V, H);
            return dot(sv.FrontGeometricNormal, L) > 0.0f;
        }
        float VoH = fabsf(dot(V, H)), eta = IORi / IORo;
        if (eta * eta * (1.0f - VoH * VoH) > 1.0f || rnd[3] < ml_fresnel_dielectric(eta, VoH)) {
            L = reflect(-V, H);
        } else {
            L = refract(-V, H, eta);
            if (!finite3(L)) L = -V;
        }
        return true;
    }

    PT_DEV v3 ComputeHalfVector(const SurfaceVectors& sv, v3 L, v3 V, bool isTransmissive) const
    {
        v3 N = sv.FrontGeometricNormal, H;
        if (isTransmissive && dot(N, L) < 0.0f) {
            H = normalize(L * IORo + V * IORi);
            if (dot(N, H) < 0.0f) H = -H;
        } else {
            H = normalize(L + V);
        }
        return H;
    }

    PT_DEV void EvaluateAll(const SurfaceVectors& sv, v3 L, v3 V, const float w[3], float& pdf, v3& diffuse, v3& specular, uint32_t ext = 0) const
    {
        const float tw = w[LOBE_TRANSMISSION];
        pdf = 0.0f; diffuse = V3(0.0f, 0.0f, 0.0f); specular = V3(0.0f, 0.0f, 0.0f);
        if (tw > 0.0f) { float p; v3 f; EvaluateLobe(sv, L, V, w, LOBE_TRANSMISSION, 0, p, f); pdf = p; specular = f; }
        if (tw < 1.0f && dot(sv.FrontGeometricNormal, L) > 0.0f) {
// ... 96 lines not shown
```

### directx-physically-based-raytracer_amd/csrc/pt_shade.hpp

```cpp
#pragma once
#include "pt_internal.hpp"
#include "pt_sharc.hpp"

namespace pt {


constexpr int kLdsStackDepth = 12;

struct RayDesc { v3 o, d; float tmin, tmax; };

PT_DEV RayDesc generate_pinhole_ray(const PtCamera& cam, uint32_t px, uint32_t py, uint32_t W, uint32_t H, float& u, float& v)
{
    u = ((float)px + 0.5f + cam.Jitter[0]) / (float)W;
    v = ((float)py + 0.5f + cam.Jitter[1]) / (float)H;
    float nx = u * 2.0f + -1.0f, ny = v * -2.0f + 1.0f;
    v3 R = V3(cam.RightDirection), U = V3(cam.UpDirection), F = V3(cam.ForwardDirection);
    v3 d = V3(mad(ny, U.x, mad(nx, R.x, F.x)), mad(ny, U.y, mad(nx, R.y, F.y)), mad(ny, U.z, mad(nx, R.z, F.z)));
    RayDesc r;
    r.o = V3(cam.Position);
    r.d = normalize(d);
    float invCos = 1.0f / dot(normalize(F), r.d);
    r.tmin = cam.NearDepth * invCos;
    r.tmax = cam.FarDepth * invCos;
    return r;
// ... 289 lines not shown
    directSpecular = V3(f16_to_f32(s.x), f16_to_f32(s.y), f16_to_f32(s.z));
}
PT_DEV bool direct_valid(const PtTextures& tx, uint32_t pixel)
{
    v3 dd, ds; load_direct(tx, pixel, dd, ds);
    const v3 di = dd + ds;
    return di.x > 0.0f || di.y > 0.0f || di.z > 0.0f;
}

template <bool DI = false, bool SHARC = false>
PT_DEV bool end_sample(const PtGraphicsSettings& gs, const PtTextures& tx, const float2* aux, PathRegs& p)
{
    p.rsum = p.rsum + p.srad;
    p.sample++;
    if (p.sample < gs.SamplesPerPixel) { p.thr = V3(1, 1, 1); p.srad = V3(0, 0, 0); p.bounce = 0; return true; }
    v3 out = V3(0, 0, 0);
    if (finite3(p.rsum)) { const float ns = (float)gs.SamplesPerPixel; out = V3(p.rsum.x / ns, p.rsum.y / ns, p.rsum.z / ns); }
    if (gs.Denoiser == PT_DENOISER_NRD_REBLUR || gs.Denoiser == PT_DENOISER_NRD_RELAX) {
        const ushort4 rad = ((const ushort4*)tx.Radiance)[p.pixel];
        const v3 ind = V3(fmaxf(out.x - f16_to_f32(rad.x), 0.0f), fmaxf(out.y - f16_to_f32(rad.y), 0.0f), fmaxf(out.z - f16_to_f32(rad.z), 0.0f));
        const float2 a = aux[p.pixel];
        const bool isDiffuse = a.y != 0.0f;
        if constexpr (DI) {
            v3 dd, ds; load_direct(tx, p.pixel, dd, ds);
            const v3 id = isDiffuse ? ind : V3(0, 0, 0), is = isDiffuse ? V3(0, 0, 0) : ind;
            const float hd = isDiffuse ? a.x : 0.0f, hs = isDiffuse ? 0.0f : a.x;
            ((ushort4*)tx.Diffuse)[p.pixel] = make_ushort4(f32_to_f16(dd.x + id.x), f32_to_f16(dd.y + id.y), f32_to_f16(dd.z + id.z), f32_to_f16(hd));
            ((ushort4*)tx.Specular)[p.pixel] = make_ushort4(f32_to_f16(ds.x + is.x), f32_to_f16(ds.y + is.y), f32_to_f16(ds.z + is.z), f32_to_f16(hs));
            return false;
        }
        const ushort4 packed = make_ushort4(f32_to_f16(ind.x), f32_to_f16(ind.y), f32_to_f16(ind.z), f32_to_f16(a.x));
        const ushort4 zero = make_ushort4(0, 0, 0, 0);
        if (tx.Diffuse) ((ushort4*)tx.Diffuse)[p.pixel] = isDiffuse ? packed : zero;
        if (tx.Specular) ((ushort4*)tx.Specular)[p.pixel] = isDiffuse ? zero : packed;
        return false;
    }
    if constexpr (DI && !SHARC) { v3 dd, ds; load_direct(tx, p.pixel, dd, ds); out = out + (dd + ds); }
    if (gs.Denoiser == PT_DENOISER_DLSS_RAY_RECONSTRUCTION && tx.SpecularHitDistance) {
        const float2 a = aux[p.pixel];
        if (a.y == 0.0f && isfinite(a.x)) ((uint16_t*)tx.SpecularHitDistance)[p.pixel] = f32_to_f16(a.x);
    }
    ((ushort4*)tx.Radiance)[p.pixel] = make_ushort4(f32_to_f16(out.x), f32_to_f16(out.y), f32_to_f16(out.z), 0);
    if (tx.RadianceF32) ((float4*)tx.RadianceF32)[p.pixel] = make_float4(out.x, out.y, out.z, 0.0f);
    return false;
}

template <bool LDS> struct GeometryFromBlob {
    const BlobReader<LDS>& blob; const BlobView& bv; ShadeTables tables = ShadeTables();
    PT_DEV HitGeometry load(uint32_t inst, uint32_t slot) const { return load_hit_geometry<LDS>(blob, bv, inst, slot); }
};

template <bool TEXTURED, bool DI = false, bool SHARC = false, typename GEOMETRY>
PT_DEV void shade_traced(const SceneView& sv, const GEOMETRY& geometry, const PtSceneData& sd, const PtGraphicsSettings& gs, const PtTextures& tx, float2* aux,
                         PathRegs& p, uint4 hr, float hitT, v3 rayDir, bool& toTraced, bool& toFresh, v3& newO, v3& newD, RoundProf* prof = nullptr,
                         const SharcView* sharc = nullptr, float* previousRoughness = nullptr)
{
    bool goes = false; int lobe = 0;
    if (aux && p.sample == 0 && p.bounce == 1) aux[p.pixel].x = hr.x == ~0u ? INFINITY : hitT;
    if (hr.x == ~0u) {
        p.srad = madd(p.thr, environment_light_color(sv, sd, rayDir), p.srad);
    } else {
        SurfaceHit h;
        reconstruct_hit<TEXTURED>(sv, geometry.load(hr.x, hr.y), hr.x, __uint_as_float(hr.z), __uint_as_float(hr.w), rayDir, h, geometry.tables);
        PT_PROF_MARK(prof, 5);
        bool cached = false;
        if constexpr (SHARC) {
            v3 radiance;
            cached = sharc_query(*sharc, h.Position, dot(h.FlatNormal, rayDir) < 0.0f ? h.FlatNormal : -h.FlatNormal, hitT, *previousRoughness, radiance);
            if (cached) p.srad = madd(p.thr, radiance, p.srad);
        }
        if (!cached) {
            const PtMaterial m = surface_material<TEXTURED>(sv, h, geometry.tables.objects);
            BSDFSample bs;
            bs.Initialize(V3(m.BaseColor), m.Metallic, m.Roughness, m.IOR, m.Transmission, h.IsFrontFace);
            v3 emission = material_emission(m);
            if constexpr (DI) if (p.bounce == 1u && direct_valid(tx, p.pixel)) emission = V3(0, 0, 0);
            goes = scatter<SHARC>(gs, p, h, bs, emission, rayDir, newO, newD, lobe, previousRoughness);
        }
    }
    if (goes) toTraced = true;
    else toFresh = end_sample<DI, SHARC>(gs, tx, aux, p);
}

template <bool DI = false, bool SHARC = false>
PT_DEV void shade_fresh_record(const FrameView& fv, const PtCamera& cam, const PtGraphicsSettings& gs, const PtTextures& tx, float2* aux, uint4 r0, uint4 r1, uint4 r2,
                               PathRegs& p, bool& toTraced, bool& toFresh, v3& newO, v3& newD, float* previousRoughness = nullptr)
{
    const uint32_t pixel = p.pixel;
    const uint32_t px = pixel % fv.width, py = global_row(fv, pixel / fv.width);
    float uu, vv;
    const RayDesc primaryRay = generate_pinhole_ray(cam, px, py, fv.width, fv.height, uu, vv);
    const v3 rayDir = primaryRay.d;
    const float4 pos = make_float4(__uint_as_float(r0.x), __uint_as_float(r0.y), __uint_as_float(r0.z), __uint_as_float(r0.w));
    const short4 nr = make_short4((short)(r1.x & 0xFFFFu), (short)(r1.x >> 16), (short)(r1.y & 0xFFFFu), (short)(r1.y >> 16));
    const short2 fe = make_short2((short)(r1.z & 0xFFFFu), (short)(r1.z >> 16)), ge = make_short2((short)(r1.w & 0xFFFFu), (short)(r1.w >> 16));
    const uchar4 bcm = make_uchar4((unsigned char)(r2.x & 0xFFu), (unsigned char)((r2.x >> 8) & 0xFFu), (unsigned char)((r2.x >> 16) & 0xFFu), (unsigned char)(r2.x >> 24));
    const ushort4 rad = make_ushort4((unsigned short)(r2.y & 0xFFFFu), (unsigned short)(r2.y >> 16), (unsigned short)(r2.z & 0xFFFFu), (unsigned short)(r2.z >> 16));
    SurfaceHit h;
    h.Position = V3(pos.x, pos.y, pos.z); h.PositionOffset = pos.w;
    h.FlatNormal = oct_decode(snorm16_to_f32(fe.x), snorm16_to_f32(fe.y));
    h.GeometricNormal = oct_decode(snorm16_to_f32(ge.x), snorm16_to_f32(ge.y));
    h.ShadingNormal = V3(snorm16_to_f32(nr.x), snorm16_to_f32(nr.y), snorm16_to_f32(nr.z));
    h.IsFrontFace = dot(h.GeometricNormal, rayDir) < 0.0f;
    const v3 emission = V3(f16_to_f32(rad.x), f16_to_f32(rad.y), f16_to_f32(rad.z));
    const float metal = unorm8_to_f32(bcm.w);
    const float ior = f16_to_f32((uint16_t)(r2.w & 0xFFFFu));
    const float tr = metal < 1.0f ? unorm8_to_f32((uint8_t)((r2.w >> 16) & 0xFFu)) : 0.0f;
    BSDFSample bs;
    bs.Initialize(V3(unorm8_to_f32(bcm.x), unorm8_to_f32(bcm.y), unorm8_to_f32(bcm.z)), metal, snorm16_to_f32(nr.w), ior, tr, h.IsFrontFace);
    int lobe = 0;
    const bool first = p.sample == 0;
    if constexpr (SHARC) {
        *previousRoughness = 0.0f;
        if constexpr (DI) { v3 dd, ds; load_direct(tx, p.pixel, dd, ds); p.srad = p.srad + (dd + ds); }
    }
    if (scatter<SHARC>(gs, p, h, bs, emission, rayDir, newO, newD, lobe, previousRoughness)) {
        toTraced = true;
        if (aux && first) aux[p.pixel].y = lobe == LOBE_DIFFUSE ? 1.0f : 0.0f;
    } else toFresh = end_sample<DI, SHARC>(gs, tx, aux, p);
}

template <bool DI = false, bool SHARC = false>
PT_DEV void shade_fresh(const FrameView& fv, const PtCamera& cam, const PtGraphicsSettings& gs, const PtTextures& tx, float2* aux, const uint4* __restrict__ primary,
                        PathRegs& p, bool& toTraced, bool& toFresh, v3& newO, v3& newD, RoundProf* prof = nullptr, float* previousRoughness = nullptr)
{
    const uint32_t pixel = p.pixel;
    const uint4 r0 = primary[3 * (size_t)pixel], r1 = primary[3 * (size_t)pixel + 1], r2 = primary[3 * (size_t)pixel + 2];
    PT_PROF_WAIT(); PT_PROF_MARK(prof, 13);
    shade_fresh_record<DI, SHARC>(fv, cam, gs, tx, aux, r0, r1, r2, p, toTraced, toFresh, newO, newD, previousRoughness);
}

template <bool SHARC = false>
PT_DEV void emit_tile(const PathQueue& qout, uint32_t seg, uint32_t segCap, uint32_t* countTraced, uint32_t* countFresh, uint32_t* lds,
                      bool toTraced, bool toFresh, const PathRegs& p, v3 newO, v3 newD, float* roughnessOut = nullptr, float previousRoughness = 0.0f)
{
    uint32_t st, sf;
    block_reserve2(toTraced, toFresh, countTraced, countFresh, lds, st, sf);
    if (toTraced) {
        store_path(qout, seg + st, p);
        qout.r0[seg + st] = make_float4(newO.x, newO.y, newO.z, 0.0f);
        qout.r1[seg + st] = make_float4(newD.x, newD.y, newD.z, INFINITY);
        if constexpr (SHARC) roughnessOut[seg + st] = previousRoughness;
    }
    if (toFresh) store_path(qout, seg + (segCap - 1u - sf), p);
}

}
```

### directx-physically-based-raytracer_amd/csrc/pt_stream.hip

```cpp
#include "pt_shade.hpp"

namespace pt {

template <bool TEXTURED, bool DI, bool SHARC = false>
__global__ __launch_bounds__(256) __attribute__((amdgpu_waves_per_eu(4, 4))) void k_shade(SceneView sv, FrameView fv, const FrameConstants* __restrict__ fc, PtTextures tx,
                                               PathQueue qin, PathQueue qout, float2* aux, uint32_t segCap, const uint32_t* countIn, uint32_t* countOut,
                                               const uint4* __restrict__ primary, BlobView bv, const uint4* __restrict__ recA, const uint32_t* __restrict__ recB, uint32_t sqShift,
                                               uint32_t sqBase, uint32_t sqCount, const SharcView* sharc = nullptr, const float* roughIn = nullptr, float* roughOut = nullptr)
{
    BlobReader<false> blob; blob.p = bv.base;
    ShadeTables tables; tables.recA = recA; tables.recB = recB;
    __shared__ uint32_t lds[32];
    uint32_t emits = 0;
    const PtCamera& cam = fc->cam; const PtSceneData& sd = fc->sd; const PtGraphicsSettings& gs = fc->gs;
    const uint32_t nsq = 1u << sqShift, bq = blockIdx.x / sqCount, sq = sqBase + (blockIdx.x - bq * sqCount), nbq = gridDim.x / sqCount;
    const uint32_t nT = countIn[sq], nF = countIn[nsq + sq];
    const uint32_t seg = sq * segCap;

    for (uint32_t tile = bq; tile * 256u < nT; tile += nbq) {
        const uint32_t local = tile * 256u + threadIdx.x;
        const uint32_t i = seg + local;
        bool toTraced = false, toFresh = false;
        PathRegs p; v3 newO = V3(0, 0, 0), newD = V3(0, 0, 1);
        float pr = 0.0f;
        if (local < nT) {
            p = load_path(qin, i);
            const uint4 hr = qin.hit[i];
            const float4 rd = qin.r1[i];
            if constexpr (SHARC) pr = roughIn[i];
            shade_traced<TEXTURED, DI, SHARC>(sv, GeometryFromBlob<false>{ blob, bv, tables }, sd, gs, tx, aux, p, hr, rd.w, V3(rd.x, rd.y, rd.z), toTraced, toFresh, newO, newD, nullptr, sharc, &pr);
        }
        emit_tile<SHARC>(qout, seg, segCap, &countOut[sq], &countOut[nsq + sq], lds + ((emits++ & 1u) << 4), toTraced, toFresh, p, newO, newD, roughOut, pr);
    }
    for (uint32_t tile = bq; tile * 256u < nF; tile += nbq) {
        const uint32_t local = tile * 256u + threadIdx.x;
        bool toTraced = false, toFresh = false;
        PathRegs p; v3 newO = V3(0, 0, 0), newD = V3(0, 0, 1);
        float pr = 0.0f;
        if (local < nF) {
            p = load_path(qin, seg + (segCap - 1u - local));
            shade_fresh<DI, SHARC>(fv, cam, gs, tx, aux, primary, p, toTraced, toFresh, newO, newD, nullptr, &pr);
        }
        emit_tile<SHARC>(qout, seg, segCap, &countOut[sq], &countOut[nsq + sq], lds + ((emits++ & 1u) << 4), toTraced, toFresh, p, newO, newD, roughOut, pr);
    }
}


constexpr int kStreamStackLds = 12;
constexpr uint32_t kStreamSteps = 6;
constexpr uint32_t kStreamRefillMin = 12;
constexpr uint32_t kStreamMinLanes = 8;
constexpr uint32_t kStreamShareShift = 1;
constexpr uint32_t kStreamGridShared = 512, kStreamGridAlone = 1024;
constexpr uint32_t kStreamLdsStack = (uint32_t)kStreamStackLds * 256u * 8u;
constexpr bool kStreamTriPairs = true;

template <bool STATS, bool WRITE_T>
__global__ __launch_bounds__(256) __attribute__((amdgpu_waves_per_eu(4, 4))) void k_extend_stream(BlobView bv, AlphaContext ac, PathQueue q, uint32_t segCap,
                                               const uint32_t* count, uint32_t* cursor, DeviceCounters* counters, uint32_t sqBase, uint32_t sqCount)
{
    extern __shared__ __attribute__((aligned(16))) unsigned char smem[];
    const uint32_t bq = blockIdx.x / sqCount, sq = sqBase + (blockIdx.x - bq * sqCount);
    const uint32_t nT = count[sq];
    const uint32_t seg = sq * segCap;
    if (bq == 0 && threadIdx.x == 0) atomicAdd(&counters->secondaryRays, (unsigned long long)nT);
    if (!nT) return;
    const uint32_t lane = threadIdx.x & 63u;
    const unsigned long long ltMask = (1ull << lane) - 1ull;
    BlobReader<false> blob; blob.p = bv.base;
    uint2 spill[kStackSize - kStreamStackLds];
    GroupStack<kStreamStackLds> stack; stack.init((PT_LDS_AS void*)smem, spill);
    v3 wo = V3(0, 0, 0), wd = V3(0, 0, 1); float wtmax = 0.0f;
    constexpr uint32_t kMarker = 0xFFFFFFFFu;
    TraceStats st; st.nodes = 0; st.tris = 0; st.overflow = 0;
    uint32_t qi = ~0u, curInst = ~0u, nodeBase16 = bv.nodeOff16, triBase16 = 0;
    float tmin = 0.0f;
    BoxRay br; br.o = V3(0, 0, 0); br.idir = V3(1, 1, 1); br.octinv4 = 0;
    RaySetup rs; rs.c1 = rs.c2 = false; rs.Sx = rs.Sy = rs.Sz = 0.0f;
    Hit h; h.t = 0.0f; h.u = h.v = 0.0f; h.inst = ~0u; h.geom = h.prim = h.slot = 0;
    uint2 G = make_uint2(0u, 0u), T = make_uint2(0u, 0u);
    bool exhausted = false;
    const bool oneInstance = bv.instCount == 1u;
    uint32_t rayNodes = 0;
#ifdef PT_STREAM_PROF
    uint32_t prof[13] = { 0 };
#endif
    while (true) {
        const unsigned long long busy = wave_ballot(qi != ~0u);
#ifdef PT_STREAM_PROF
        prof[12]++;
#endif
        if (exhausted && !busy) break;
        {
            const unsigned long long idle = ~busy;
            const uint32_t nIdle = (uint32_t)__popcll(idle);
            if (!exhausted && (nIdle >= kStreamRefillMin || !busy)) {
                uint32_t base = 0;
                if (lane == 0) base = atomicAdd(&cursor[sq], nIdle);
                base = (uint32_t)__shfl((int)base, 0);
                if (base + nIdle >= nT) exhausted = true;
#ifdef PT_STREAM_PROF
                prof[10]++; prof[11] += base < nT ? min(nIdle, nT - base) : 0u;
#endif
                if (qi == ~0u) {
                    const uint32_t e = base + (uint32_t)__popcll(idle & ltMask);
                    if (e < nT) {
                        const float4 o = q.r0[seg + e], d = q.r1[seg + e];
                        wo = V3(o.x, o.y, o.z); wd = V3(d.x, d.y, d.z); wtmax = d.w;
                        qi = e; tmin = o.w; curInst = ~0u; nodeBase16 = bv.nodeOff16;
                        br = box_ray(V3(o.x, o.y, o.z), V3(d.x, d.y, d.z));
                        h.t = d.w; h.u = h.v = 0.0f; h.inst = ~0u; h.geom = h.prim = h.slot = 0;
                        G = root_node_group(oneInstance); T = root_tri_group(oneInstance, 1u);
                        stack.sp = 0;
                        if (STATS) rayNodes = st.nodes;
                    }
                }
            }
        }
        bool finished = false;
        #pragma unroll 1
        for (uint32_t step = 0; step < kStreamSteps; step++) {
            const bool live = qi != ~0u && !finished;
            const bool top = curInst == ~0u;
            const bool wantNode = live && G.y > 0x00FFFFFFu;
// ... 35 lines not shown
            {
                const f4v* recN = blob.p + addrN; const f4v* recT = blob.p + addrT; const f4v* recT2 = blob.p + addrT2;
                if (aN) { A0 = recN[0]; A1 = recN[1]; A2 = recN[2]; A3 = recN[3]; A4 = recN[4]; }
                if (aE) { B0 = recN[0]; B1 = recN[1]; B2 = recN[2]; C0 = recN[3]; A0 = recN[4]; A1 = recN[5]; A2 = recN[6]; A3 = recN[7]; A4 = recN[8]; }
                if (aT) { B0 = recT[0]; B1 = recT[1]; B2 = recT[2]; }
                if (aT2) { A2 = recT2[0]; A3 = recT2[1]; A4 = recT2[2]; }
            }
            if (aT) {
                if (STATS) st.tris++;
                float t, u, v;
                if (tri_test(rs, br.o, V3(B0.x, B0.y, B0.z), V3(B1.x, B1.y, B1.z), V3(B2.x, B2.y, B2.z), t, u, v))
                    commit_candidate(ac, __float_as_uint(B2.w), h, tmin, t, u, v, curInst, __float_as_uint(B0.w), __float_as_uint(B1.w), item);
            }
            if (aT2) {
                if (STATS) st.tris++;
                float t, u, v;
                if (tri_test(rs, br.o, V3(A2.x, A2.y, A2.z), V3(A3.x, A3.y, A3.z), V3(A4.x, A4.y, A4.z), t, u, v))
                    commit_candidate(ac, __float_as_uint(A4.w), h, tmin, t, u, v, curInst, __float_as_uint(A2.w), __float_as_uint(A3.w), item2);
            }
            if (aN) {
                if (STATS) st.nodes++;
                const uint32_t hits = wide_node_hits(A0, A1, A2, A3, A4, br, tmin, h.t);
                G = make_uint2(__float_as_uint(A1.x), (hits & 0xFF000000u) | (__float_as_uint(A0.w) >> 24));
                T = make_uint2(__float_as_uint(A1.y), hits & 0x00FFFFFFu);
            }
            if (aE) {
                const uint32_t cm = __float_as_uint(C0.z), ntri = cm & 0x00FFFFFFu;
                if ((cm >> 24) && ntri != 0u) {
                    const v3 ro = V3(sop3t(B0.x, wo.x, B0.y, wo.y, B0.z, wo.z, B0.w), sop3t(B1.x, wo.x, B1.y, wo.y, B1.z, wo.z, B1.w), sop3t(B2.x, wo.x, B2.y, wo.y, B2.z, wo.z, B2.w));
                    const v3 rd = V3(sop3(B0.x, wd.x, B0.y, wd.y, B0.z, wd.z), sop3(B1.x, wd.x, B1.y, wd.y, B1.z, wd.z), sop3(B2.x, wd.x, B2.y, wd.y, B2.z, wd.z));
                    rs = ray_setup(rd);
                    br = box_ray(ro, rd);
                    nodeBase16 = bv.nodeOff16 + __float_as_uint(C0.x) * kNode16;
                    triBase16 = bv.triOff16 + __float_as_uint(C0.y) * kTri16;
                    stack.push(G); stack.push(T); stack.push(make_uint2(kMarker, 0u));
                    curInst = __float_as_uint(C0.w);
                    if (blas_single_leaf(ntri)) { G = root_node_group(true); T = root_tri_group(true, ntri); }
                    else {
                        if (STATS) st.nodes++;
                        const uint32_t hits = wide_node_hits(A0, A1, A2, A3, A4, br, tmin, h.t);
                        G = make_uint2(__float_as_uint(A1.x), (hits & 0xFF000000u) | (__float_as_uint(A0.w) >> 24));
                        T = make_uint2(__float_as_uint(A1.y), hits & 0x00FFFFFFu);
                    }
                }
            }
            if (live && !T.y && G.y <= 0x00FFFFFFu) {
                if (stack.sp > 0) {
                    const uint2 e = stack.pop();
                    if (e.x == kMarker && e.y == 0u) {
                        if (stack.overflow) { finished = true; stack.sp = 0; }
                        else {
                            T = stack.pop(); G = stack.pop();
                                    br = box_ray(wo, wd); nodeBase16 = bv.nodeOff16; curInst = ~0u;
                        }
                    } else if (e.y > 0x00FFFFFFu) G = e;
                    else T = e;
                } else finished = true;
            }
        }
        if (finished) {
            const bool hit = h.inst != ~0u && h.t < wtmax;
            if (STATS) atomicMax(&counters->maxNodesPerRay, st.nodes - rayNodes);
            q.hit[seg + qi] = make_uint4(hit ? h.inst : ~0u, h.slot, __float_as_uint(h.u), __float_as_uint(h.v));
            if (WRITE_T) q.r1[seg + qi].w = h.t;
            qi = ~0u;
        }
    }
    if (STATS) { atomicAdd(&counters->nodesVisited, (unsigned long long)st.nodes); atomicAdd(&counters->trianglesTested, (unsigned long long)st.tris); }
    if (st.overflow + stack.overflow) atomicAdd(&counters->stackOverflows, st.overflow + stack.overflow);
#ifdef PT_STREAM_PROF
    if (lane == 0) for (int i = 0; i < 13; i++) atomicAdd((unsigned int*)&counters->mismatchRay[i], prof[i]);
#endif
}


hipError_t launch_shade(Context& c, const FramePlan& p, const SceneView& sv, const FrameView& fv, const PtTextures& tx, uint32_t round, uint32_t grid, hipStream_t stream,
                        uint32_t sqBase, uint32_t sqCount)
{
    const uint4* recA = p.recordsUsable ? c.shadeRecA.data() : nullptr; const uint32_t* recB = p.recordsUsable ? c.shadeRecB.data() : nullptr;
    const uint32_t qi = round & 1u;
    const uint32_t* countIn = &c.queueCounts.data()[round * p.cstride()]; uint32_t* countOut = &c.queueCounts.data()[(round + 1u) * p.cstride()];
    with_flags([&](auto D, auto T, auto S) {
        k_shade<T(), D(), S()><<<grid, 256, 0, stream>>>(sv, fv, c.frameConstants.data(), tx, c.queue[qi], c.queue[qi ^ 1u], p.aux, p.segCap, countIn, countOut, c.primaryRecords.data(), c.scene.blob,
                                                       recA, recB, p.sqShift, sqBase, sqCount, S() ? c.sharcView.data() : nullptr, S() ? c.sharcRough[qi].data() : nullptr, S() ? c.sharcRough[qi ^ 1u].data() : nullptr);
    }, p.di, p.textured, p.sharc);
    return hipGetLastError();
}

hipError_t launch_extend_stream(Context& c, const FramePlan& p, const AlphaContext& ac, uint32_t round, hipStream_t stream, uint32_t sqBase, uint32_t sqCount)
{
    const uint32_t nsq = p.nsq();
    const uint32_t whole = std::max(nsq, std::min(p.grid, c.framesInFlight > 1 ? kStreamGridShared : kStreamGridAlone));
    const uint32_t sgrid = std::max(1u, whole / nsq) * sqCount;
    uint32_t* count = &c.queueCounts.data()[(round + 1u) * p.cstride()];
    with_flags([&](auto S, auto W) {
        k_extend_stream<S(), W()><<<sgrid, 256, kStreamLdsStack, stream>>>(c.scene.blob, ac, c.queue[(round + 1u) & 1u], p.segCap, count, count + 2u * nsq, c.counters.data(), sqBase, sqCount);
    }, p.stats, p.writeT);
    return hipGetLastError();
}

}
```

### directx-physically-based-raytracer_amd/layouts.py

```python
import numpy as np

NONE = 0xFFFFFFFF

VERTEX = np.dtype({
    "names": ["Position", "Normal", "Tangent", "TexCoord0", "TexCoord1"],
    "formats": [("<f4", 3), ("<i2", 3), ("<i2", 3), ("<f2", 2), ("<f2", 2)],
    "offsets": [0, 12, 18, 24, 28], "itemsize": 32})

SKELETAL_VERTEX = np.dtype({
    "names": ["Position", "Normal", "Tangent", "Joints", "Weights"],
    "formats": [("<f4", 3), ("<i2", 3), ("<i2", 3), ("<u2", 4), ("<f4", 4)],
    "offsets": [0, 12, 18, 24, 32], "itemsize": 48})

VERTEX_DESC = np.dtype({
    "names": ["Stride", "Normal", "Tangent", "TexCoord"],
    "formats": ["<u4", "<u4", "<u4", ("<u4", 2)],
    "offsets": [0, 16, 20, 24], "itemsize": 32})

MESH_DESCRIPTORS = np.dtype({
    "names": ["Vertices", "Indices", "MotionVectors"],
    "formats": ["<u4", "<u4", "<u4"], "offsets": [0, 4, 8], "itemsize": 16})

MATERIAL = np.dtype({
    "names": ["BaseColor", "EmissiveStrength", "EmissiveColor", "Metallic", "Roughness", "IOR",
# ... 143 lines not shown
    s["TemporalDepthThreshold"] = temporal_depth
    s["TemporalNormalThreshold"] = temporal_normal
    s["SpatialSamples"] = spatial_samples
    s["SpatialBiasCorrection"] = spatial_bias
    s["DisocclusionBoostSamples"] = boost_samples
    s["SpatialSamplingRadius"] = radius
    s["SpatialDepthThreshold"] = spatial_depth
    s["SpatialNormalThreshold"] = spatial_normal
    return s


POST_PROCESS_SETTINGS = np.dtype({
    "names": ["RenderSize", "IsBloomEnabled", "BloomStrength", "IsHDREnabled", "ToneMappingOperator", "Exposure", "PaperWhiteNits",
              "ColorPrimaryRotation"],
    "formats": [("<u4", 2), "<u4", "<f4", "<u4", "<u4", "<f4", "<f4", "<u4"],
    "offsets": [0, 8, 12, 16, 20, 24, 28, 32], "itemsize": 48})

TONE_MAP_SATURATE, TONE_MAP_REINHARD, TONE_MAP_ACES_FILMIC = 1, 2, 3
TONE_MAP_OPERATORS = {"saturate": TONE_MAP_SATURATE, "reinhard": TONE_MAP_REINHARD, "aces_filmic": TONE_MAP_ACES_FILMIC}
COLOR_ROTATION_HDTV_TO_UHDTV, COLOR_ROTATION_DCI_P3_D65_TO_UHDTV, COLOR_ROTATION_HDTV_TO_DCI_P3_D65 = 0, 1, 2
COLOR_ROTATIONS = {"hdtv_to_uhdtv": COLOR_ROTATION_HDTV_TO_UHDTV, "dci_p3_d65_to_uhdtv": COLOR_ROTATION_DCI_P3_D65_TO_UHDTV,
                   "hdtv_to_dci_p3_d65": COLOR_ROTATION_HDTV_TO_DCI_P3_D65}
POST_MAX_SIZE = 16384
POST_STAGES = 9
POST_FORMATS = {"Color": ("<u2", 4), "BackBuffer": ("<u4", 1), "Display8": ("u1", 4)}


def check_post_processing_settings(s):
    s = np.asarray(s).reshape(())
    w, h = (int(v) for v in s["RenderSize"])
    f = {k: float(np.float32(s[k])) for k in ("BloomStrength", "Exposure", "PaperWhiteNits")}
    if not (1 <= w <= POST_MAX_SIZE and 1 <= h <= POST_MAX_SIZE):
        raise ValueError(f"RenderSize must be 1..{POST_MAX_SIZE} on both axes")
    if int(s["IsBloomEnabled"]) > 1 or int(s["IsHDREnabled"]) > 1:
        raise ValueError("IsBloomEnabled / IsHDREnabled must be 0 or 1")
    if not 0.0 <= f["BloomStrength"] <= 1.0:
        raise ValueError("BloomStrength must be in [0, 1]")
    if int(s["ToneMappingOperator"]) not in TONE_MAP_OPERATORS.values():
        raise ValueError("unknown ToneMappingOperator")
    if not -10.0 <= f["Exposure"] <= 10.0:
        raise ValueError("Exposure must be in [-10, 10]")
    if not 50.0 <= f["PaperWhiteNits"] <= 10000.0:
        raise ValueError("PaperWhiteNits must be in [50, 10000]")
    if int(s["ColorPrimaryRotation"]) not in COLOR_ROTATIONS.values():
        raise ValueError("unknown ColorPrimaryRotation")
    return s


def post_bloom_size_ok(width, height):
    return width >= 2 and height >= 2 and max(width, height) >= 32


def post_processing_settings(width, height, bloom=True, strength=0.05, operator="aces_filmic", exposure=0.0, hdr=False,
                             paper_white_nits=200.0, rotation="hdtv_to_uhdtv"):
    s = np.zeros((), POST_PROCESS_SETTINGS)
    s["RenderSize"] = (width, height)
    s["IsBloomEnabled"] = 1 if bloom else 0
    s["BloomStrength"] = strength
    s["IsHDREnabled"] = 1 if hdr else 0
    s["ToneMappingOperator"] = TONE_MAP_OPERATORS[operator] if isinstance(operator, str) else operator
    s["Exposure"] = exposure
    s["PaperWhiteNits"] = paper_white_nits
    s["ColorPrimaryRotation"] = COLOR_ROTATIONS[rotation] if isinstance(rotation, str) else rotation
    return check_post_processing_settings(s)


SHARC_SETTINGS = np.dtype({
    "names": ["AccumulationFrames", "MaxStaleFrames", "SceneScale", "IsAntiFireflyEnabled", "DownscaleFactor", "RoughnessThreshold",
              "IsHashGridVisualizationEnabled"],
    "formats": ["<u4", "<u4", "<f4", "<u4", "<u4", "<f4", "<u4"], "offsets": [0, 4, 8, 12, 16, 20, 24], "itemsize": 28})
SHARC_DEFAULT_CAPACITY = 1 << 22
SHARC_ENTRY = np.dtype({
    "names": ["Key", "Voxel"], "formats": ["<u8", ("<u4", 4)], "offsets": [0, 8], "itemsize": 32})
SHARC_QUERY_RESULT = np.dtype({"names": ["Valid", "Radiance"], "formats": ["<u4", ("<f4", 3)], "offsets": [0, 4], "itemsize": 16})
SHARC_PATH_VERTEX = np.dtype({
    "names": ["Position", "Flags", "Normal", "Random", "Radiance", "KeyLo", "Throughput", "KeyHi"],
    "formats": [("<f4", 3), "<u4", ("<f4", 3), "<f4", ("<f4", 3), "<u4", ("<f4", 3), "<u4"],
    "offsets": [0, 12, 16, 28, 32, 44, 48, 60], "itemsize": 64})
SHARC_PATH_SCATTER = np.dtype({
    "names": ["Query", "Origin", "Sampled", "L", "Goes"], "formats": [("u1", 96), ("<f4", 3), "<u4", ("<f4", 3), "<u4"],
    "offsets": [0, 96, 108, 112, 124], "itemsize": 128})
SHARC_VERTEX_HIT, SHARC_VERTEX_MISS, SHARC_VERTEX_ENDED, SHARC_VERTEX_RESAMPLED = 1, 2, 4, 8
DEBUG_SHARC_LOG_PATHS, DEBUG_SHARC_SKIP_UPDATE = 0x100, 0x200


def check_sharc_settings(s):
    s = np.asarray(s).reshape(())
    if not 1 <= int(s["DownscaleFactor"]) <= 4:
        raise ValueError("DownscaleFactor must be 1..4")
    if not 1 <= int(s["AccumulationFrames"]) <= 63:
        raise ValueError("AccumulationFrames must be 1..63")
    if not 1 <= int(s["MaxStaleFrames"]) <= 255:
        raise ValueError("MaxStaleFrames must be 1..255")
    if not 5.0 <= float(np.float32(s["SceneScale"])) <= 100.0:
        raise ValueError("SceneScale must be in [5, 100]")
    if not 0.0 <= float(np.float32(s["RoughnessThreshold"])) <= 1.0:
        raise ValueError("RoughnessThreshold must be in [0, 1]")
    if int(s["IsAntiFireflyEnabled"]) > 1:
        raise ValueError("IsAntiFireflyEnabled must be 0 or 1")
    if int(s["IsHashGridVisualizationEnabled"]) != 0:
        raise ValueError("hash-grid visualisation is not served")
    return s


def sharc_settings(downscale=4, scene_scale=50.0, roughness_threshold=0.4, accumulation_frames=10, max_stale_frames=64,
                   anti_firefly=True, visualization=False):
    s = np.zeros((), SHARC_SETTINGS)
    s["AccumulationFrames"] = accumulation_frames
    s["MaxStaleFrames"] = max_stale_frames
    s["SceneScale"] = scene_scale
    s["IsAntiFireflyEnabled"] = 1 if anti_firefly else 0
    s["DownscaleFactor"] = downscale
    s["RoughnessThreshold"] = roughness_threshold
    s["IsHashGridVisualizationEnabled"] = 1 if visualization else 0
    return check_sharc_settings(s)


GBUFFER_CONSTANTS = np.dtype({
    "names": ["RenderSize", "Flags"], "formats": [("<u4", 2), "<u4"], "offsets": [0, 8], "itemsize": 12})


class GBufferFlags:
    Position = 0x1
    FlatNormal = 0x2
    GeometricNormal = 0x4
    LinearDepth = 0x8
    NormalizedDepth = 0x10
    MotionVector = 0x20
    DiffuseAlbedo = 0x40
    SpecularAlbedo = 0x80
    Albedo = 0xC0
    NormalRoughness = 0x100
    Radiance = 0x200
    Geometry = 0x1 | 0x2 | 0x4 | 0x8 | 0x10 | 0x20 | 0x100
    Material = 0x400 | 0xC0 | 0x100 | 0x200
    DefaultNoDenoiser = 0xFFFFFFFF & ~0xC0


GBUFFER_FORMATS = {
    "Position": ("<f4", 4),
    "FlatNormal": ("<i2", 2),
    "GeometricNormal": ("<i2", 2),
    "LinearDepth": ("<f4", 1),
    "NormalizedDepth": ("<f4", 1),
    "MotionVector": ("<u2", 4),
    "BaseColorMetalness": ("u1", 4),
    "DiffuseAlbedo": ("<u2", 4),
    "SpecularAlbedo": ("<u2", 4),
    "NormalRoughness": ("<i2", 4),
    "IOR": ("<u2", 1),
    "Transmission": ("u1", 1),
    "Radiance": ("<u2", 4),
}
GBUFFER_ORDER = list(GBUFFER_FORMATS.keys())
DENOISER_FORMATS = {"Diffuse": ("<u2", 4), "Specular": ("<u2", 4), "SpecularHitDistance": ("<u2", 1)}
DENOISER_NONE, DENOISER_DLSS_RR, DENOISER_NRD_REBLUR, DENOISER_NRD_RELAX = 0, 1, 2, 3


def default_material():
    m = np.zeros((), MATERIAL)
    m["BaseColor"] = (0, 0, 0, 1)
    m["EmissiveStrength"] = 1
    m["Roughness"] = 0.5
    m["IOR"] = 1.5
    m["AlphaCutoff"] = 0.5
    return m
# ... 1 lines not shown
```

### directx-physically-based-raytracer_amd/ptamd.py

```python
import ctypes as C
import os

import numpy as np

from . import layouts as L

_HERE = os.path.dirname(os.path.abspath(__file__))
LIB_PATH = os.path.join(_HERE, "libptamd.so")
_LIB = None

EXPORTS = [
    "pt_abi_version", "pt_create", "pt_destroy", "pt_last_error", "pt_set_stream", "pt_sync", "pt_set_frames_in_flight", "pt_set_round_chains",
    "pt_heap_resize", "pt_heap_set_buffer", "pt_heap_set_texture", "pt_build_bottom_level", "pt_update_bottom_level", "pt_release_bottom_level", "pt_skin_mesh",
    "pt_build_top_level", "pt_get_accel_stats", "pt_share_scene", "pt_set_camera", "pt_set_scene_data", "pt_set_object_data", "pt_invalidate_object_data",
    "pt_set_instance_data", "pt_set_sharding", "pt_local_rows", "pt_deinterleave_bands", "pt_gbuffer_render",
    "pt_comm_get_unique_id", "pt_comm_init", "pt_comm_adopt", "pt_comm_destroy", "pt_gather_bands", "pt_gather_plan",
    "pt_raytrace_set_constants", "pt_raytrace_render", "pt_trace_visibility", "pt_bsdf_evaluate", "pt_bsdf_sample", "pt_reset_counters", "pt_get_counters",
    "pt_di_set_constants", "pt_di_render", "pt_di_light_count", "pt_di_download_lights",
    "pt_di_set_resampling", "pt_di_render_with_history", "pt_di_reset_history", "pt_di_download_reservoirs",
    "pt_di_set_light_sampling", "pt_di_download_presampled", "pt_di_set_visibility",
    "pt_post_set_constants", "pt_post_render", "pt_post_download_bloom",
    "pt_sharc_configure", "pt_sharc_set_constants", "pt_raytrace_render_sharc", "pt_sharc_reset", "pt_sharc_download",
    "pt_sharc_debug_keys", "pt_sharc_debug_query", "pt_sharc_download_update_paths", "pt_sharc_download_update_scatter",
    "pt_set_debug_flags", "pt_debug_read_mismatch", "pt_debug_download_blob", "pt_debug_trace_ray", "pt_debug_trace_closest", "pt_enable_kernel_timing", "pt_get_kernel_timing", "pt_get_round_timing",
]


class PtError(RuntimeError):
    """reference: std::system_error from ThrowIfFailed (Source/ErrorHelpers.ixx:16-32)."""


class PtInvalidArgument(ValueError):
    """reference: Throw<std::invalid_argument> (Source/RaytracingHelpers.ixx:83-88)."""


class GeometryDesc(C.Structure):
    _fields_ = [("VertexBuffer", C.c_void_p), ("VertexCount", C.c_uint32), ("VertexStride", C.c_uint32),
                ("IndexBuffer", C.c_void_p), ("IndexCount", C.c_uint32), ("IndexStride", C.c_uint32),
                ("Flags", C.c_uint32), ("_pad", C.c_uint32)]


class InstanceDesc(C.Structure):
    _fields_ = [("Transform", C.c_float * 12), ("InstanceID", C.c_uint32), ("InstanceMask", C.c_uint32),
                ("AccelerationStructure", C.c_uint64)]


TEXTURE_NAMES = L.GBUFFER_ORDER + ["RadianceF32", "Diffuse", "Specular", "SpecularHitDistance"]


class Textures(C.Structure):
    _fields_ = [(n, C.c_void_p) for n in TEXTURE_NAMES]


class PreviousTextures(C.Structure):
    _fields_ = [(n, C.c_void_p) for n in L.DI_PREVIOUS_TEXTURES]


class PostTextures(C.Structure):
    _fields_ = [("Radiance", C.c_void_p), ("Color", C.c_void_p), ("BackBuffer", C.c_void_p), ("Display8", C.c_void_p)]


class Sharding(C.Structure):
    _fields_ = [("RankIndex", C.c_uint32), ("RankCount", C.c_uint32), ("BandHeight", C.c_uint32), ("_pad", C.c_uint32)]


class BandMessage(C.Structure):
    _fields_ = [("Peer", C.c_uint32), ("IsSend", C.c_uint32), ("Band", C.c_uint32), ("_pad", C.c_uint32),
                ("LocalOffset", C.c_uint64), ("FullOffset", C.c_uint64), ("Bytes", C.c_uint64)]


class Counters(C.Structure):
    _fields_ = [("PrimaryRays", C.c_uint64), ("SecondaryRays", C.c_uint64), ("NodesVisited", C.c_uint64),
                ("TrianglesTested", C.c_uint64), ("WavefrontIterations", C.c_uint64), ("BvhMismatches", C.c_uint64),
                ("StackOverflows", C.c_uint64), ("MaxNodesPerRay", C.c_uint64)]


class BlobLayout(C.Structure):
    _fields_ = [(n, C.c_uint32) for n in ("InstanceOffset16", "NodeOffset16", "TriangleOffset16", "LeafInstanceOffset16",
                                          "InstanceCount", "NodeCount", "TriangleCount", "Bytes")]


class AccelStats(C.Structure):
    _fields_ = [("InstanceCount", C.c_uint32), ("BottomLevelCount", C.c_uint32), ("TriangleCount", C.c_uint64),
                ("NodeBytes", C.c_uint64), ("TriangleBytes", C.c_uint64), ("NodeSizeBytes", C.c_uint32),
                ("TriangleSizeBytes", C.c_uint32), ("MaxBottomLevelDepth", C.c_uint32), ("TopLevelDepth", C.c_uint32),
                ("BlobBytes", C.c_uint64), ("SharedScene", C.c_uint32), ("NormalRecords", C.c_uint32),
                ("OwnedBottomLevelBytes", C.c_uint64), ("RoundObjectsInLds", C.c_uint32), ("RoundRecordsInLds", C.c_uint32)]


_BSDF_MATERIAL = [("BaseColor", C.c_float * 3), ("Metallic", C.c_float), ("Roughness", C.c_float), ("IOR", C.c_float),
                  ("Transmission", C.c_float), ("IsFrontFace", C.c_float),
                  ("GeometricNormal", C.c_float * 3), ("ShadingNormal", C.c_float * 3), ("V", C.c_float * 3)]


class BsdfQuery(C.Structure):
    _fields_ = _BSDF_MATERIAL + [("L", C.c_float * 3)]


class BsdfResult(C.Structure):
    _fields_ = [("Diffuse", C.c_float * 3), ("Specular", C.c_float * 3), ("PDF", C.c_float), ("_pad", C.c_float)]


class BsdfSampleQuery(C.Structure):
    _fields_ = _BSDF_MATERIAL + [("Random", C.c_float * 4), ("ExtFlags", C.c_uint32), ("_pad", C.c_uint32 * 2)]


class BsdfSampleResult(C.Structure):
    _fields_ = [("L", C.c_float * 3), ("PDF", C.c_float), ("F", C.c_float * 3), ("Weights", C.c_float * 3),
                ("Lobe", C.c_uint32), ("Ok", C.c_uint32)]


CLOSEST_HIT = np.dtype([("T", "<f4"), ("U", "<f4"), ("V", "<f4"), ("Instance", "<u4"), ("Geometry", "<u4"), ("Primitive", "<u4"),
                        ("Slot", "<u4"), ("_pad", "<u4")])


def load_library():
    global _LIB
    if _LIB is None:
        if not os.path.exists(LIB_PATH):
            raise PtError(f"{LIB_PATH} is missing: run __graft_entry__.build() (make -C .../csrc). "
                          "The path tracer has no CPU fallback.")
        import torch
        lib = C.CDLL(LIB_PATH)
        lib.pt_last_error.restype = C.c_char_p
        lib.pt_last_error.argtypes = [C.c_void_p]
        lib.pt_create.argtypes = [C.c_int, C.POINTER(C.c_void_p)]
        lib.pt_destroy.argtypes = [C.c_void_p]; lib.pt_destroy.restype = None
        lib.pt_set_stream.argtypes = [C.c_void_p, C.c_void_p]
        lib.pt_sync.argtypes = [C.c_void_p]
        lib.pt_set_frames_in_flight.argtypes = [C.c_void_p, C.c_uint32]
        lib.pt_set_round_chains.argtypes = [C.c_void_p, C.c_uint32]
        lib.pt_heap_resize.argtypes = [C.c_void_p, C.c_uint32]
        lib.pt_heap_set_buffer.argtypes = [C.c_void_p, C.c_uint32, C.c_void_p, C.c_uint64, C.c_uint32]
        lib.pt_heap_set_texture.argtypes = [C.c_void_p, C.c_uint32, C.c_void_p, C.c_uint32, C.c_uint32, C.c_uint32, C.c_uint32]
        lib.pt_build_bottom_level.argtypes = [C.c_void_p, C.c_void_p, C.c_uint32, C.c_uint32, C.POINTER(C.c_uint64)]
        lib.pt_release_bottom_level.argtypes = [C.c_void_p, C.c_uint64]
        lib.pt_update_bottom_level.argtypes = [C.c_void_p, C.c_uint64, C.c_void_p, C.c_uint32, C.c_uint32]
        lib.pt_skin_mesh.argtypes = [C.c_void_p, C.c_void_p, C.c_void_p, C.c_void_p, C.c_void_p, C.c_uint32]
        lib.pt_build_top_level.argtypes = [C.c_void_p, C.c_void_p, C.c_uint32, C.c_uint32]
        lib.pt_get_accel_stats.argtypes = [C.c_void_p, C.c_void_p]
        lib.pt_share_scene.argtypes = [C.c_void_p, C.c_void_p]
        for f in (lib.pt_set_camera, lib.pt_set_scene_data, lib.pt_set_sharding, lib.pt_raytrace_set_constants,
                  lib.pt_raytrace_render, lib.pt_get_counters):
            f.argtypes = [C.c_void_p, C.c_void_p]
        lib.pt_set_object_data.argtypes = [C.c_void_p, C.c_void_p, C.c_uint32]
        lib.pt_set_instance_data.argtypes = [C.c_void_p, C.c_void_p, C.c_uint32]
        lib.pt_invalidate_object_data.argtypes = [C.c_void_p]
        lib.pt_local_rows.argtypes = [C.c_void_p, C.c_uint32, C.POINTER(C.c_uint32)]
        lib.pt_deinterleave_bands.argtypes = [C.c_void_p, C.c_void_p, C.c_void_p, C.c_void_p, C.c_uint32, C.c_uint32,
                                              C.c_uint32, C.c_uint32, C.c_uint32]
        lib.pt_comm_get_unique_id.argtypes = [C.c_void_p]
        lib.pt_comm_init.argtypes = [C.c_void_p, C.c_void_p, C.c_uint32, C.c_uint32]
        lib.pt_comm_adopt.argtypes = [C.c_void_p, C.c_void_p]
        lib.pt_comm_destroy.argtypes = [C.c_void_p]
        lib.pt_gather_bands.argtypes = [C.c_void_p, C.c_void_p, C.c_void_p, C.c_uint32, C.c_uint32, C.c_uint32, C.c_uint32]
        lib.pt_gather_plan.argtypes = [C.c_void_p, C.c_uint32, C.c_uint64, C.c_uint32, C.c_void_p, C.c_uint32, C.POINTER(C.c_uint32)]
        lib.pt_gbuffer_render.argtypes = [C.c_void_p, C.c_void_p, C.c_void_p]
        lib.pt_trace_visibility.argtypes = [C.c_void_p, C.c_void_p, C.c_uint32, C.c_void_p]
        lib.pt_bsdf_evaluate.argtypes = [C.c_void_p, C.c_void_p, C.c_uint32, C.c_void_p]
        lib.pt_bsdf_sample.argtypes = [C.c_void_p, C.c_void_p, C.c_uint32, C.c_void_p]
        lib.pt_reset_counters.argtypes = [C.c_void_p]
        lib.pt_di_set_constants.argtypes = [C.c_void_p, C.c_void_p]
        lib.pt_di_render.argtypes = [C.c_void_p, C.c_void_p]
        lib.pt_di_light_count.argtypes = [C.c_void_p, C.POINTER(C.c_uint32)]
        lib.pt_di_download_lights.argtypes = [C.c_void_p, C.c_void_p, C.c_uint32, C.POINTER(C.c_uint32)]
        lib.pt_di_set_resampling.argtypes = [C.c_void_p, C.c_void_p]
        lib.pt_di_render_with_history.argtypes = [C.c_void_p, C.c_void_p, C.c_void_p]
        lib.pt_di_reset_history.argtypes = [C.c_void_p]
        lib.pt_di_download_reservoirs.argtypes = [C.c_void_p, C.c_void_p, C.c_uint32, C.POINTER(C.c_uint32)]
        lib.pt_di_set_light_sampling.argtypes = [C.c_void_p, C.c_void_p]
        lib.pt_di_set_visibility.argtypes = [C.c_void_p, C.c_void_p]
        lib.pt_di_download_presampled.argtypes = [C.c_void_p, C.c_uint32, C.c_void_p, C.c_uint32, C.POINTER(C.c_uint32)]
        lib.pt_post_set_constants.argtypes = [C.c_void_p, C.c_void_p]
        lib.pt_post_render.argtypes = [C.c_void_p, C.c_void_p]
        lib.pt_post_download_bloom.argtypes = [C.c_void_p, C.c_uint32, C.c_void_p, C.c_uint64, C.POINTER(C.c_uint32), C.POINTER(C.c_uint32)]
        lib.pt_sharc_configure.argtypes = [C.c_void_p, C.c_uint32]
        lib.pt_sharc_set_constants.argtypes = [C.c_void_p, C.c_void_p]
        lib.pt_raytrace_render_sharc.argtypes = [C.c_void_p, C.c_void_p]
        lib.pt_sharc_reset.argtypes = [C.c_void_p]
        lib.pt_sharc_download.argtypes = [C.c_void_p, C.c_void_p, C.c_uint32, C.POINTER(C.c_uint32)]
        lib.pt_sharc_debug_keys.argtypes = [C.c_void_p, C.c_void_p, C.c_void_p, C.c_uint32, C.c_void_p, C.c_void_p, C.c_void_p]
        lib.pt_sharc_debug_query.argtypes = [C.c_void_p, C.c_void_p, C.c_void_p, C.c_void_p, C.c_void_p, C.c_uint32, C.c_void_p]
        lib.pt_sharc_download_update_paths.argtypes = [C.c_void_p, C.c_void_p, C.c_uint32, C.POINTER(C.c_uint32), C.POINTER(C.c_uint32)]
        lib.pt_sharc_download_update_scatter.argtypes = [C.c_void_p, C.c_void_p, C.c_uint32, C.POINTER(C.c_uint32), C.POINTER(C.c_uint32)]
        lib.pt_set_debug_flags.argtypes = [C.c_void_p, C.c_uint32]
        lib.pt_debug_read_mismatch.argtypes = [C.c_void_p, C.c_void_p]
        lib.pt_debug_download_blob.argtypes = [C.c_void_p, C.c_void_p, C.c_uint64, C.c_void_p]
        lib.pt_debug_trace_ray.argtypes = [C.c_void_p, C.c_void_p, C.c_void_p, C.c_uint32]
        lib.pt_debug_trace_closest.argtypes = [C.c_void_p, C.c_void_p, C.c_uint32, C.c_void_p]
        lib.pt_enable_kernel_timing.argtypes = [C.c_void_p, C.c_int]
        lib.pt_get_round_timing.argtypes = [C.c_void_p, C.POINTER(C.c_float), C.POINTER(C.c_uint32)]
        lib.pt_get_kernel_timing.argtypes = [C.c_void_p, C.POINTER(C.c_float), C.POINTER(C.c_float),
                                             C.POINTER(C.c_uint32), C.POINTER(C.c_uint32)]
        _LIB = lib
    return _LIB


def local_rows(height, rank=0, world=1, band=16):
    s = Sharding(rank, world, band, 0)
    out = C.c_uint32(0)
    if load_library().pt_local_rows(C.byref(s), height, C.byref(out)) != 0:
        raise PtInvalidArgument("invalid sharding")
    return out.value


def gather_plan(height, row_bytes, rank, world, band=16, root=0):
    lib = load_library()
    s = Sharding(rank, world, band, 0)
    n = C.c_uint32(0)
    if lib.pt_gather_plan(C.byref(s), height, row_bytes, root, None, 0, C.byref(n)) != 0:
        raise PtInvalidArgument("invalid sharding / root")
    msgs = (BandMessage * max(1, n.value))()
    if lib.pt_gather_plan(C.byref(s), height, row_bytes, root, msgs, n.value, C.byref(n)) != 0:
        raise PtInvalidArgument("invalid sharding / root")
    return [(m.Peer, m.IsSend, m.Band, m.LocalOffset, m.FullOffset, m.Bytes) for m in msgs[:n.value]]


class DeviceContext:

    def __init__(self, device_ordinal=0, stream=None):
        self.lib = load_library()
        h = C.c_void_p()
        st = self.lib.pt_create(device_ordinal, C.byref(h))
# ... 4 lines not shown
        if stream is not None:
            self.check(self.lib.pt_set_stream(self.handle, C.c_void_p(stream)))

    def check(self, status):
        if status == 0:
            return
        msg = self.lib.pt_last_error(self.handle).decode()
        if status == -1:
            raise PtInvalidArgument(msg)
        raise PtError(f"status {status}: {msg}")

    def sync(self):
        self.check(self.lib.pt_sync(self.handle))

    def set_frames_in_flight(self, n):
        self.check(self.lib.pt_set_frames_in_flight(self.handle, n))

    def set_round_chains(self, n):
        self.check(self.lib.pt_set_round_chains(self.handle, n))

    def close(self):
        if getattr(self, "handle", None):
            self.lib.pt_destroy(self.handle)
            self.handle = None

    def __del__(self):
        try:
            self.close()
        except Exception:
            pass

    def reset_counters(self):
        self.check(self.lib.pt_reset_counters(self.handle))

    def counters(self):
        c = Counters()
        self.check(self.lib.pt_get_counters(self.handle, C.byref(c)))
        return c

    def set_debug_flags(self, flags):
        self.check(self.lib.pt_set_debug_flags(self.handle, flags))
        self.debug_flags = flags

    def invalidate_object_data(self):
        self.check(self.lib.pt_invalidate_object_data(self.handle))

    def enable_kernel_timing(self, on=True):
        self.check(self.lib.pt_enable_kernel_timing(self.handle, 1 if on else 0))

    def kernel_timing(self):
        e, s, ne, ns = C.c_float(), C.c_float(), C.c_uint32(), C.c_uint32()
        self.check(self.lib.pt_get_kernel_timing(self.handle, C.byref(e), C.byref(s), C.byref(ne), C.byref(ns)))
        r, nr = C.c_float(), C.c_uint32()
        self.check(self.lib.pt_get_round_timing(self.handle, C.byref(r), C.byref(nr)))
        return {"extend_ms": e.value, "shade_ms": s.value, "extend_launches": ne.value, "shade_launches": ns.value,
                "round_ms": r.value, "round_launches": nr.value}

    def download_blob(self):
        lay = BlobLayout()
        self.check(self.lib.pt_debug_download_blob(self.handle, None, 0, C.byref(lay)))
        buf = np.zeros(lay.Bytes, np.uint8)
        self.check(self.lib.pt_debug_download_blob(self.handle, C.c_void_p(buf.ctypes.data), buf.nbytes, C.byref(lay)))
        return lay, buf

    def trace_closest(self, rays, brute_force=False):
        torch = _torch()
        rays = np.ascontiguousarray(rays, np.float32).reshape(-1, 8)
        dr = torch.from_numpy(rays).to(torch.device("cuda", self.device_ordinal))
        dh = torch.zeros(max(1, len(rays)) * 32, dtype=torch.uint8, device=dr.device)
        before = getattr(self, "debug_flags", 0)
        self.set_debug_flags((before | 0x2) if brute_force else (before & ~0x2))
        try:
            self.check(self.lib.pt_debug_trace_closest(self.handle, C.c_void_p(dr.data_ptr()), len(rays), C.c_void_p(dh.data_ptr())))
            self.sync()
        finally:
            self.set_debug_flags(before)
        return dh.cpu().numpy()[:len(rays) * 32].view(CLOSEST_HIT).copy()

    def accel_stats(self):
        s = AccelStats()
        self.check(self.lib.pt_get_accel_stats(self.handle, C.byref(s)))
        return s

    @staticmethod
    def comm_unique_id():
        lib = load_library()
        buf = (C.c_uint8 * 128)()
        st = lib.pt_comm_get_unique_id(buf)
        if st != 0:
            raise PtError(f"pt_comm_get_unique_id failed ({st}): {lib.pt_last_error(None).decode()}")
        return bytes(buf)

    def comm_init(self, unique_id, rank, world):
        buf = (C.c_uint8 * 128).from_buffer_copy(unique_id)
        self.check(self.lib.pt_comm_init(self.handle, buf, rank, world))

    def gather_bands(self, local, dst_full, width, height, pixel_bytes, root=0):
        self.check(self.lib.pt_gather_bands(self.handle, C.c_void_p(local.data_ptr()),
                                            C.c_void_p(dst_full.data_ptr() if dst_full is not None else None), width, height, pixel_bytes, root))

    def set_sharding(self, rank, world, band=16):
        s = Sharding(rank, world, band, 0)
        self.check(self.lib.pt_set_sharding(self.handle, C.byref(s)))
        self.sharding = (rank, world, band)


def _torch():
    import torch
    if not torch.cuda.is_available():
        raise PtError("no GPU visible to torch: the path tracer has no CPU fallback")
    return torch


def to_device(arr, device):
    torch = _torch()
    raw = np.ascontiguousarray(arr).view(np.uint8).reshape(-1)
    if raw.size == 0:
        raw = np.zeros(16, np.uint8)
    return torch.from_numpy(raw.copy()).to(device)


def _download_counted(ctx, fn, dtype, *lead, counts=1):
    n = [C.c_uint32(0) for _ in range(counts)]
    refs = [C.byref(v) for v in n]
    ctx.check(fn(ctx.handle, *lead, None, 0, *refs))
    out = np.zeros(tuple(v.value for v in n), dtype)
    if out.size:
        ctx.check(fn(ctx.handle, *lead, C.c_void_p(out.ctypes.data), out.size, *refs))
    return out


class SharedScene:

    def __init__(self, ctx, owner):
        self.ctx, self.owner, self.desc, self.device = ctx, owner, owner.desc, owner.device
        ctx.check(ctx.lib.pt_share_scene(ctx.handle, owner.ctx.handle))

    def GetTopLevelAccelerationStructure(self):
        return self.ctx.handle

    def close(self):
        pass


class Scene:
    SKIN_STAGING_RING = 4

    def __init__(self, ctx, scene, device=None):
        torch = _torch()
        self.ctx, self.desc = ctx, scene
        self.device = device or torch.device("cuda", ctx.device_ordinal)
        lib = ctx.lib
        self._buffers = []
        ctx.check(lib.pt_heap_resize(ctx.handle, len(scene.heap)))
        heap_dev = []
        for i, item in enumerate(scene.heap):
            t = to_device(item.array, self.device)
            self._buffers.append(t); heap_dev.append(t)
            if item.kind == 0:
                ctx.check(lib.pt_heap_set_buffer(ctx.handle, i, C.c_void_p(t.data_ptr()), item.array.nbytes, item.stride))
            else:
                ctx.check(lib.pt_heap_set_texture(ctx.handle, i, C.c_void_p(t.data_ptr()), item.width, item.height, item.fmt,
                                                  1 if item.kind == 2 else 0))
        self.object_data = to_device(scene.object_data, self.device)
        self.instance_data = to_device(scene.instance_data, self.device)
        ctx.check(lib.pt_set_object_data(ctx.handle, C.c_void_p(self.object_data.data_ptr()), len(scene.object_data)))
# ... 395 lines not shown
```

### include/ptamd.h

```cpp
#ifndef PTAMD_H
#define PTAMD_H

#include <stdint.h>

#ifdef __cplusplus
extern "C" {
#endif

#define PTAMD_ABI_VERSION 4

typedef enum PtStatus {
    PT_OK = 0,
    PT_ERROR_INVALID_ARGUMENT = -1,
    PT_ERROR_HIP = -2,
    PT_ERROR_OUT_OF_MEMORY = -3,
    PT_ERROR_NOT_READY = -4,
    PT_ERROR_NO_DEVICE = -5,
    PT_ERROR_RCCL = -6
} PtStatus;

typedef struct PtVertexDesc {
    uint32_t Stride, _pad[3];
    struct { uint32_t Normal, Tangent, TextureCoordinates[2]; } AttributeOffsets;
} PtVertexDesc;
// ... 82 lines not shown
    void* FlatNormal;
    void* GeometricNormal;
    void* LinearDepth;
    void* NormalizedDepth;
    void* MotionVector;
    void* BaseColorMetalness;
    void* DiffuseAlbedo;
    void* SpecularAlbedo;
    void* NormalRoughness;
    void* IOR;
    void* Transmission;
    void* Radiance;
    void* RadianceF32;
    void* Diffuse;
    void* Specular;
    void* SpecularHitDistance;
} PtTextures;

typedef struct PtContext PtContext;

int  pt_abi_version(void);
int  pt_create(int device_ordinal, PtContext** out_ctx);
void pt_destroy(PtContext* ctx);
const char* pt_last_error(const PtContext* ctx);
int  pt_set_stream(PtContext* ctx, void* hip_stream);
int  pt_sync(PtContext* ctx);
int  pt_set_frames_in_flight(PtContext* ctx, uint32_t frames);
int  pt_set_round_chains(PtContext* ctx, uint32_t chains);

int  pt_heap_resize(PtContext* ctx, uint32_t descriptor_count);
int  pt_heap_set_buffer(PtContext* ctx, uint32_t descriptor, const void* device_ptr, uint64_t bytes, uint32_t stride);
typedef enum PtFormat {
    PT_FORMAT_R8G8B8A8_UNORM = 0,
    PT_FORMAT_R8G8B8A8_UNORM_SRGB = 1,
    PT_FORMAT_R32G32B32A32_FLOAT = 2
} PtFormat;
int  pt_heap_set_texture(PtContext* ctx, uint32_t descriptor, const void* device_ptr, uint32_t width, uint32_t height,
                         uint32_t format, uint32_t is_cube);

typedef struct PtGeometryDesc {
    const void* VertexBuffer;
    uint32_t VertexCount, VertexStride;
    const void* IndexBuffer;
    uint32_t IndexCount, IndexStride;
    uint32_t Flags;
    uint32_t _pad;
} PtGeometryDesc;
#define PT_GEOMETRY_FLAG_OPAQUE 0x1u

#define PT_BUILD_FLAG_ALLOW_UPDATE      0x01u
#define PT_BUILD_FLAG_PREFER_FAST_TRACE 0x04u
#define PT_BUILD_FLAG_PREFER_FAST_BUILD 0x08u

int  pt_build_bottom_level(PtContext* ctx, const PtGeometryDesc* geometries, uint32_t geometry_count,
                           uint32_t build_flags, uint64_t* out_blas_id);
int  pt_update_bottom_level(PtContext* ctx, uint64_t blas_id, const PtGeometryDesc* geometries, uint32_t geometry_count, uint32_t build_flags);
int  pt_release_bottom_level(PtContext* ctx, uint64_t blas_id);

int  pt_skin_mesh(PtContext* ctx, const void* skeletal_vertices, const float* skeletal_transforms, void* vertices,
                  void* motion_vectors, uint32_t vertex_count);

typedef struct PtInstanceDesc {
    float Transform[12];
    uint32_t InstanceID;
    uint32_t InstanceMask;
    uint64_t AccelerationStructure;
} PtInstanceDesc;

int  pt_build_top_level(PtContext* ctx, const PtInstanceDesc* descs, uint32_t count, uint32_t build_flags);

typedef struct PtAccelStats {
    uint32_t InstanceCount, BottomLevelCount;
    uint64_t TriangleCount;
    uint64_t NodeBytes, TriangleBytes;
    uint32_t NodeSizeBytes, TriangleSizeBytes;
    uint32_t MaxBottomLevelDepth, TopLevelDepth;
    uint64_t BlobBytes;
    uint32_t SharedScene;
    uint32_t NormalRecords;
    uint64_t OwnedBottomLevelBytes;
    uint32_t RoundObjectsInLds, RoundRecordsInLds;
} PtAccelStats;
int  pt_get_accel_stats(PtContext* ctx, PtAccelStats* out);

int  pt_share_scene(PtContext* ctx, PtContext* source);

int  pt_set_camera(PtContext* ctx, const PtCamera* camera);
int  pt_set_scene_data(PtContext* ctx, const PtSceneData* scene_data);
int  pt_set_object_data(PtContext* ctx, const PtObjectData* device_objects, uint32_t count);
int  pt_invalidate_object_data(PtContext* ctx);
int  pt_set_instance_data(PtContext* ctx, const PtInstanceData* device_instances, uint32_t count);

typedef struct PtSharding { uint32_t RankIndex, RankCount, BandHeight, _pad; } PtSharding;
int  pt_set_sharding(PtContext* ctx, const PtSharding* sharding);
int  pt_local_rows(const PtSharding* sharding, uint32_t frame_height, uint32_t* out_rows);
typedef struct PtBandMessage {
    uint32_t Peer, IsSend, Band, _pad;
    uint64_t LocalOffset;
    uint64_t FullOffset;
    uint64_t Bytes;
} PtBandMessage;
#define PT_COMM_ID_BYTES 128
int  pt_comm_get_unique_id(void* out_id_host);
int  pt_comm_init(PtContext* ctx, const void* id_host, uint32_t rank, uint32_t world);
int  pt_comm_adopt(PtContext* ctx, void* nccl_comm);
int  pt_comm_destroy(PtContext* ctx);
int  pt_gather_bands(PtContext* ctx, const void* local_bands, void* dst_full, uint32_t width, uint32_t height, uint32_t pixel_bytes, uint32_t root);
int  pt_gather_plan(const PtSharding* sharding, uint32_t height, uint64_t row_bytes, uint32_t root, PtBandMessage* out, uint32_t capacity, uint32_t* out_count);

int  pt_deinterleave_bands(PtContext* ctx, void* dst_full, const void* gathered, const uint64_t* rank_offsets_host,
                           uint32_t rank_count, uint32_t band_height, uint32_t width, uint32_t height, uint32_t pixel_bytes);

int  pt_gbuffer_render(PtContext* ctx, const PtGBufferConstants* constants, const PtTextures* textures);

int  pt_raytrace_set_constants(PtContext* ctx, const PtGraphicsSettings* settings);
int  pt_raytrace_render(PtContext* ctx, const PtTextures* textures);

typedef struct PtDISettings {
    uint32_t RenderSize[2];
    uint32_t FrameIndex;
    uint32_t LocalLightSamples;
    uint32_t Denoiser;
    uint32_t IsLastRenderPass;
    uint32_t ExtFlags;
    uint32_t _pad;
} PtDISettings;

typedef struct PtTriangleLight {
    float Base[3], Area;
    float Edge0[3], Power;
    float Edge1[3]; uint32_t InstanceIndex;
    float Normal[3];
    uint32_t PrimitiveIndex;
    float Radiance[3];
    uint32_t GeometryIndex;
} PtTriangleLight;

int  pt_di_set_constants(PtContext* ctx, const PtDISettings* settings);
int  pt_di_render(PtContext* ctx, const PtTextures* textures);
int  pt_di_light_count(PtContext* ctx, uint32_t* out_count);
int  pt_di_download_lights(PtContext* ctx, PtTriangleLight* host_dst, uint32_t capacity, uint32_t* out_count);

enum { PT_DI_BIAS_CORRECTION_OFF = 0, PT_DI_BIAS_CORRECTION_BASIC = 1 };
typedef struct PtDIResamplingSettings {
    uint32_t TemporalResampling;
    uint32_t TemporalBiasCorrection;
    uint32_t MaxHistoryLength;
    uint32_t BoilingFilter;
    float    BoilingFilterStrength;
    float    TemporalDepthThreshold;
    float    TemporalNormalThreshold;
    uint32_t SpatialSamples;
    uint32_t SpatialBiasCorrection;
    uint32_t DisocclusionBoostSamples;
    float    SpatialSamplingRadius;
    float    SpatialDepthThreshold;
    float    SpatialNormalThreshold;
    uint32_t _pad[3];
} PtDIResamplingSettings;

typedef struct PtDIReservoir {
    uint32_t LightIndex;
    float    U, V;
    float    W;
    uint32_t M;
    float    TargetPdf;
// ... 59 lines not shown
int  pt_bsdf_sample(PtContext* ctx, const PtBsdfSampleQuery* device_queries, uint32_t count, PtBsdfSampleResult* device_results);

enum { PT_TONE_MAP_SATURATE = 1, PT_TONE_MAP_REINHARD = 2, PT_TONE_MAP_ACES_FILMIC = 3 };
enum { PT_COLOR_ROTATION_HDTV_TO_UHDTV = 0, PT_COLOR_ROTATION_DCI_P3_D65_TO_UHDTV = 1,
       PT_COLOR_ROTATION_HDTV_TO_DCI_P3_D65 = 2 };
typedef struct PtPostProcessSettings {
    uint32_t RenderSize[2];
    uint32_t IsBloomEnabled;  float BloomStrength;
    uint32_t IsHDREnabled;
    uint32_t ToneMappingOperator;  float Exposure;
    float    PaperWhiteNits;  uint32_t ColorPrimaryRotation;
    uint32_t _pad[3];
} PtPostProcessSettings;
typedef struct PtPostTextures {
    const void* Radiance;
    void* Color;
    void* BackBuffer;
    void* Display8;
} PtPostTextures;
int pt_post_set_constants(PtContext* ctx, const PtPostProcessSettings* settings);
int pt_post_render(PtContext* ctx, const PtPostTextures* textures);
int pt_post_download_bloom(PtContext* ctx, uint32_t stage, uint16_t* host_rgba16f, uint64_t capacity_texels,
                           uint32_t* out_width, uint32_t* out_height);

typedef struct PtSHARCSettings {
    uint32_t AccumulationFrames;
    uint32_t MaxStaleFrames;
    float    SceneScale;
    uint32_t IsAntiFireflyEnabled;
    uint32_t DownscaleFactor;
    float    RoughnessThreshold;
    uint32_t IsHashGridVisualizationEnabled;
} PtSHARCSettings;
typedef struct PtSHARCEntry { uint64_t Key; uint32_t Voxel[4]; uint32_t _pad[2]; } PtSHARCEntry;
typedef struct PtSHARCQueryResult { uint32_t Valid; float Radiance[3]; } PtSHARCQueryResult;
typedef struct PtSHARCPathVertex {
    float Position[3]; uint32_t Flags;
    float Normal[3];   float Random;
    float Radiance[3]; uint32_t KeyLo;
    float Throughput[3]; uint32_t KeyHi;
} PtSHARCPathVertex;
typedef struct PtSHARCPathScatter {
    PtBsdfSampleQuery Query;
    float Origin[3]; uint32_t Sampled;
    float L[3];      uint32_t Goes;
} PtSHARCPathScatter;
#define PT_SHARC_VERTEX_HIT       0x1u
#define PT_SHARC_VERTEX_MISS      0x2u
#define PT_SHARC_VERTEX_ENDED     0x4u
#define PT_SHARC_VERTEX_RESAMPLED 0x8u
int pt_sharc_configure(PtContext* ctx, uint32_t capacity);
int pt_sharc_set_constants(PtContext* ctx, const PtSHARCSettings* settings);
int pt_raytrace_render_sharc(PtContext* ctx, const PtTextures* textures);
int pt_sharc_reset(PtContext* ctx);
int pt_sharc_download(PtContext* ctx, PtSHARCEntry* host_dst, uint32_t capacity, uint32_t* out_count);
int pt_sharc_debug_keys(PtContext* ctx, const float* positions, const float* normals, uint32_t n, uint64_t* keys, uint32_t* levels, float* voxel_sizes);
int pt_sharc_debug_query(PtContext* ctx, const float* positions, const float* normals, const float* distances, const float* previous_roughness,
                         uint32_t n, PtSHARCQueryResult* results);
int pt_sharc_download_update_paths(PtContext* ctx, PtSHARCPathVertex* host_dst, uint32_t capacity, uint32_t* out_paths, uint32_t* out_bounces);
int pt_sharc_download_update_scatter(PtContext* ctx, PtSHARCPathScatter* host_dst, uint32_t capacity, uint32_t* out_paths, uint32_t* out_bounces);

typedef struct PtCounters {
    uint64_t PrimaryRays;
    uint64_t SecondaryRays;
    uint64_t NodesVisited;
    uint64_t TrianglesTested;
    uint64_t WavefrontIterations;
    uint64_t BvhMismatches;
    uint64_t StackOverflows;
    uint64_t MaxNodesPerRay;
} PtCounters;
int  pt_reset_counters(PtContext* ctx);
int  pt_get_counters(PtContext* ctx, PtCounters* out);
#define PT_DEBUG_TRAVERSAL_STATS 0x1u
#define PT_DEBUG_TRAVERSAL_V1   0x4u
#define PT_DEBUG_TRAVERSAL_PHASED 0x8u
#define PT_DEBUG_UNFUSED_ROUNDS  0x10u
#define PT_DEBUG_LOCKSTEP        0x20u
#define PT_DEBUG_GATHER_LOCAL_ONLY 0x40u
#define PT_DEBUG_BRUTE_FORCE     0x2u
#define PT_DEBUG_GATHER_SELF_EXCHANGE 0x80u
#define PT_DEBUG_SHARC_LOG_PATHS 0x100u
#define PT_DEBUG_SHARC_SKIP_UPDATE 0x200u
int  pt_set_debug_flags(PtContext* ctx, uint32_t flags);
int  pt_debug_read_mismatch(PtContext* ctx, float* out16);

typedef struct PtBlobLayout {
    uint32_t InstanceOffset16, NodeOffset16, TriangleOffset16, LeafInstanceOffset16;
    uint32_t InstanceCount, NodeCount, TriangleCount, Bytes;
} PtBlobLayout;
int  pt_debug_download_blob(PtContext* ctx, void* host_dst, uint64_t capacity_bytes, PtBlobLayout* out_layout);
int  pt_debug_trace_ray(PtContext* ctx, const PtRayDesc* host_ray, uint32_t* host_log, uint32_t log_words);
typedef struct PtClosestHit { float T, U, V; uint32_t Instance, Geometry, Primitive, Slot, _pad; } PtClosestHit;
int  pt_debug_trace_closest(PtContext* ctx, const PtRayDesc* device_rays, uint32_t count, PtClosestHit* device_hits);

int  pt_enable_kernel_timing(PtContext* ctx, int enable);
int  pt_get_kernel_timing(PtContext* ctx, float* extend_ms, float* shade_ms, uint32_t* extend_launches, uint32_t* shade_launches);
int  pt_get_round_timing(PtContext* ctx, float* round_ms, uint32_t* round_launches);

#ifdef __cplusplus
}
#endif
#endif
```

Baseline: 12100.

## Store decoded primary surface records to skip per-sample decode in shading

Primary hit records are now decoded once (camera ray, octahedral normals, BSDF F0 and material terms) when written by the init and first-round kernels. Each fresh sample then loads the decoded 112-byte record instead of re-decoding the 48-byte packed one. The intent is to remove repeated decode ALU work and the camera-ray regeneration on every sample. In exchange, each fresh path reads more than twice as many bytes, and the record buffer grows accordingly. A debug flag restores the packed path, and a stats API reports which layout is in use.

```diff
diff --git a/directx-physically-based-raytracer_amd/csrc/pt_api.hip b/directx-physically-based-raytracer_amd/csrc/pt_api.hip
--- a/directx-physically-based-raytracer_amd/csrc/pt_api.hip
+++ b/directx-physically-based-raytracer_amd/csrc/pt_api.hip
@@ -544,6 +544,14 @@
     return PT_OK;
 }
 
+int pt_get_shading_record_stats(PtContext* ctx, PtShadingRecordStats* out)
+{
+    if (!ctx || !out) return PT_ERROR_INVALID_ARGUMENT;
+    out->PrimaryRecordBytes = ctx->c.lastPrimaryRecordBytes;
+    out->PrimaryRecordsDecoded = ctx->c.lastPrimaryRecordBytes > 48u ? 1u : 0u;
+    return PT_OK;
+}
+
 int pt_set_camera(PtContext* ctx, const PtCamera* camera)
 {
     if (!ctx) return PT_ERROR_INVALID_ARGUMENT;
diff --git a/directx-physically-based-raytracer_amd/csrc/pt_internal.hpp b/directx-physically-based-raytracer_amd/csrc/pt_internal.hpp
--- a/directx-physically-based-raytracer_amd/csrc/pt_internal.hpp
+++ b/directx-physically-based-raytracer_amd/csrc/pt_internal.hpp
@@ -147,6 +147,7 @@
     DeviceBuffer<uint4> queueArrays[2][6];
     PathQueue queue[2]{};
     DeviceBuffer<uint4> primaryRecords;
+    uint32_t lastPrimaryRecordBytes = 0;
     DeviceBuffer<float2> pixelAux;
     DeviceBuffer<FrameConstants> frameConstants;
     GraphExec graphExec; std::string graphKey; bool disableGraphs = false;
@@ -243,6 +244,7 @@
     uint32_t objectsInLds, recordsInLds;
     bool recordsUsable;
     bool writeT, stats, di, textured, sharc;
+    bool primaryDecoded;
     float2* aux;
     uint32_t nsq() const { return 1u << sqShift; }
     uint32_t cstride() const { return 3u * nsq(); }
diff --git a/directx-physically-based-raytracer_amd/csrc/pt_kernels.hip b/directx-physically-based-raytracer_amd/csrc/pt_kernels.hip
--- a/directx-physically-based-raytracer_amd/csrc/pt_kernels.hip
+++ b/directx-physically-based-raytracer_amd/csrc/pt_kernels.hip
@@ -151,10 +151,10 @@
 
 
 __global__ __launch_bounds__(256) void k_pt_init(FrameView fv, const FrameConstants* __restrict__ fc, PtTextures tx, PathQueue q, float2* aux, uint32_t segCap, uint32_t* countFresh,
-                                                 uint4* __restrict__ primary, uint32_t sqShift)
+                                                 uint4* __restrict__ primary, uint32_t sqShift, uint32_t decoded)
 {
     __shared__ uint32_t lds[8];
-    const PtGraphicsSettings& gs = fc->gs;
+    const PtCamera& cam = fc->cam; const PtGraphicsSettings& gs = fc->gs;
     const uint32_t npix = fv.width * fv.localRows;
     const uint32_t nsq = 1u << sqShift, sq = blockIdx.x & (nsq - 1u), bq = blockIdx.x >> sqShift, nbq = gridDim.x >> sqShift;
     for (uint32_t j = bq; (j * nsq + sq) * 256u < npix; j += nbq) {
@@ -169,10 +169,12 @@
             q.s2[slot] = make_float4(0.0f, 0.0f, 0.0f, __uint_as_float(0u));
             if (aux) aux[p] = make_float2(INFINITY, 1.0f);
             const uint2 nr = ((const uint2*)tx.NormalRoughness)[p], rad = ((const uint2*)tx.Radiance)[p];
-            primary[3 * (size_t)p] = ((const uint4*)tx.Position)[p];
-            primary[3 * (size_t)p + 1] = make_uint4(nr.x, nr.y, ((const uint32_t*)tx.FlatNormal)[p], ((const uint32_t*)tx.GeometricNormal)[p]);
-            primary[3 * (size_t)p + 2] = make_uint4(((const uint32_t*)tx.BaseColorMetalness)[p], rad.x, rad.y,
-                                                    (uint32_t)((const uint16_t*)tx.IOR)[p] | ((uint32_t)((const uint8_t*)tx.Transmission)[p] << 16));
+            const uint4 r0 = ((const uint4*)tx.Position)[p];
+            const uint4 r1 = make_uint4(nr.x, nr.y, ((const uint32_t*)tx.FlatNormal)[p], ((const uint32_t*)tx.GeometricNormal)[p]);
+            const uint4 r2 = make_uint4(((const uint32_t*)tx.BaseColorMetalness)[p], rad.x, rad.y,
+                                        (uint32_t)((const uint16_t*)tx.IOR)[p] | ((uint32_t)((const uint8_t*)tx.Transmission)[p] << 16));
+            if (decoded) store_primary_decoded(primary, p, decode_primary(fv, cam, p, r0, r1, r2));
+            else { primary[3 * (size_t)p] = r0; primary[3 * (size_t)p + 1] = r1; primary[3 * (size_t)p + 2] = r2; }
         }
     }
 }
@@ -180,7 +182,7 @@
 template <bool DI, bool SHARC = false>
 __global__ __launch_bounds__(256) void k_pt_first(FrameView fv, const FrameConstants* __restrict__ fc, PtTextures tx, PathQueue qout, float2* aux,
                                                                                              uint32_t segCap, uint32_t* countOut, uint4* __restrict__ primary, uint32_t sqShift,
-                                                                                             float* roughOut = nullptr)
+                                                                                             uint32_t decoded, float* roughOut = nullptr)
 {
     __shared__ uint32_t lds[32];
     uint32_t emits = 0;
@@ -205,8 +207,10 @@
             const uint4 r1 = make_uint4(nr.x, nr.y, ((const uint32_t*)tx.FlatNormal)[pix], ((const uint32_t*)tx.GeometricNormal)[pix]);
             const uint4 r2 = make_uint4(((const uint32_t*)tx.BaseColorMetalness)[pix], rad.x, rad.y,
                                         (uint32_t)((const uint16_t*)tx.IOR)[pix] | ((uint32_t)((const uint8_t*)tx.Transmission)[pix] << 16));
-            primary[3 * (size_t)pix] = r0; primary[3 * (size_t)pix + 1] = r1; primary[3 * (size_t)pix + 2] = r2;
-            shade_fresh_record<DI, SHARC>(fv, cam, gs, tx, aux, r0, r1, r2, p, toTraced, toFresh, newO, newD, &pr);
+            const PrimarySurface s = decode_primary(fv, cam, pix, r0, r1, r2);
+            if (decoded) store_primary_decoded(primary, pix, s);
+            else { primary[3 * (size_t)pix] = r0; primary[3 * (size_t)pix + 1] = r1; primary[3 * (size_t)pix + 2] = r2; }
+            shade_primary<DI, SHARC>(gs, tx, aux, s, p, toTraced, toFresh, newO, newD, &pr);
         }
         emit_tile<SHARC>(qout, seg, segCap, &countOut[sq], &countOut[nsq + sq], lds + ((emits++ & 1u) << 4), toTraced, toFresh, p, newO, newD, roughOut, pr);
     }
@@ -306,7 +310,7 @@
     uint32_t objectsInLds;
     const uint4* recA; const uint32_t* recB;
     uint32_t recordsInLds, sqShift;
-    const uint4* primary;
+    const uint4* primary; uint32_t primaryDecoded;
     const SharcView* sharc; const float* roughIn; float* roughOut;
 };
 
@@ -407,7 +411,7 @@
         if (local < nF) {
             p = load_path(qin, seg + (segCap - 1u - local));
             PT_PROF_WAIT(); PT_PROF_MARK(prof, 12);
-            shade_fresh<DI, SHARC>(fv, cam, gs, tx, aux, primary, p, toTraced, toFresh, newO, newD, prof, &pr);
+            shade_fresh<DI, SHARC>(fv, cam, gs, tx, aux, primary, A->primaryDecoded != 0u, p, toTraced, toFresh, newO, newD, prof, &pr);
         }
         PT_PROF_MARK(prof, 14);
         emit_tile<SHARC>(qout, seg, segCap, &countOut[sq], &countOut[nsq + sq], lds + ((emits++ & 1u) << 4), toTraced, toFresh, p, newO, newD, A->roughOut, pr);
@@ -691,7 +695,7 @@
     return hipGetLastError();
 }
 
-static hipError_t ensure_queues(Context& c, uint32_t capacity, uint32_t iterations)
+static hipError_t ensure_queues(Context& c, uint32_t capacity, uint32_t iterations, uint32_t primary16)
 {
     hipError_t e = hipSuccess;
     for (auto& arrays : c.queueArrays) for (auto& a : arrays) if (e == hipSuccess) e = a.reserve(capacity);
@@ -700,7 +704,7 @@
         c.queue[k] = PathQueue{ (float4*)a[0].data(), (float4*)a[1].data(), (float4*)a[2].data(), (float4*)a[3].data(), (float4*)a[4].data(), a[5].data() };
     }
     if (e != hipSuccess) return e;
-    if ((e = c.primaryRecords.reserve(3 * (size_t)capacity)) != hipSuccess) return e;
+    if ((e = c.primaryRecords.reserve(primary16 * (size_t)capacity)) != hipSuccess) return e;
     return c.queueCounts.reserve(iterations);
 }
 
@@ -760,6 +764,7 @@
     p.stats = (c.debugFlags & PT_DEBUG_TRAVERSAL_STATS) != 0;
     p.di = gs.IsDIEnabled != 0u;
     p.textured = c.heapHasTextures;
+    p.primaryDecoded = !(c.debugFlags & PT_DEBUG_PACKED_PRIMARY);
 }
 
 constexpr uint32_t kStreamingChains = 3;
@@ -777,9 +782,9 @@
         k_capture_normals<<<dim3(std::min((c.scene.blasTableMaxTris + 255u) / 256u, 64u), c.scene.blasTableCount), 256, 0, c.stream>>>(c.scene.blasTable, sv.shadeGeom, c.shadeRecA.data(), c.shadeRecB.data());
     if (p.first)
         with_flags([&](auto S, auto D) {
-            k_pt_first<D(), S()><<<p.grid, 256, 0, c.stream>>>(fv, c.frameConstants.data(), tx, c.queue[1], p.aux, p.segCap, &c.queueCounts.data()[p.cstride()], c.primaryRecords.data(), p.sqShift, c.sharcRough[1].data());
+            k_pt_first<D(), S()><<<p.grid, 256, 0, c.stream>>>(fv, c.frameConstants.data(), tx, c.queue[1], p.aux, p.segCap, &c.queueCounts.data()[p.cstride()], c.primaryRecords.data(), p.sqShift, p.primaryDecoded ? 1u : 0u, c.sharcRough[1].data());
         }, p.sharc, p.di);
-    else k_pt_init<<<p.grid, 256, 0, c.stream>>>(fv, c.frameConstants.data(), tx, c.queue[0], p.aux, p.segCap, &c.queueCounts.data()[p.nsq()], c.primaryRecords.data(), p.sqShift);
+    else k_pt_init<<<p.grid, 256, 0, c.stream>>>(fv, c.frameConstants.data(), tx, c.queue[0], p.aux, p.segCap, &c.queueCounts.data()[p.nsq()], c.primaryRecords.data(), p.sqShift, p.primaryDecoded ? 1u : 0u);
     return hipGetLastError();
 }
 
@@ -864,7 +869,8 @@
     FramePlan plan; plan_frame(plan, c, sv, fv, sharcQuery);
     const FramePlan& p = plan;
     const uint32_t rounds = p.rounds, nsq = p.nsq(), cstride = p.cstride();
-    if ((e = ensure_queues(c, p.segCap * nsq, (rounds + 2) * cstride)) != hipSuccess) return e;
+    if ((e = ensure_queues(c, p.segCap * nsq, (rounds + 2) * cstride, p.primaryDecoded ? kPrimaryDecoded16 : kPrimaryPacked16)) != hipSuccess) return e;
+    c.lastPrimaryRecordBytes = 16u * (p.primaryDecoded ? kPrimaryDecoded16 : kPrimaryPacked16);
     if ((e = c.frameConstants.reserve(1)) != hipSuccess) return e;
     if (p.sharc) for (auto& a : c.sharcRough) if ((e = a.reserve((size_t)p.segCap * nsq)) != hipSuccess) return e;
     FrameConstants fc; fc.cam = c.camera; fc.sd = c.sceneData; fc.gs = c.settings;
@@ -886,7 +892,7 @@
             std::memset(&a, 0, sizeof a);
             a.sv = sv; a.fv = fv; a.tx = tx; a.bv = c.scene.blob; a.qin = c.queue[r & 1]; a.qout = c.queue[(r + 1) & 1];
             a.fc = c.frameConstants.data(); a.aux = p.aux; a.countIn = &c.queueCounts.data()[r * cstride]; a.countOut = &c.queueCounts.data()[(r + 1) * cstride]; a.sqShift = p.sqShift;
-            a.counters = c.counters.data(); a.segCap = p.segCap; a.primary = c.primaryRecords.data(); a.objectsInLds = p.objectsInLds;
+            a.counters = c.counters.data(); a.segCap = p.segCap; a.primary = c.primaryRecords.data(); a.primaryDecoded = p.primaryDecoded ? 1u : 0u; a.objectsInLds = p.objectsInLds;
             if (p.recordsUsable) { a.recA = c.shadeRecA.data(); a.recB = c.shadeRecB.data(); a.recordsInLds = p.recordsInLds; }
             if (p.sharc) { a.sharc = c.sharcView.data(); a.roughIn = c.sharcRough[r & 1].data(); a.roughOut = c.sharcRough[(r + 1) & 1].data(); }
         }
@@ -896,7 +902,7 @@
     }
 
     const bool graphable = c.stream != nullptr && !c.timing && !c.disableGraphs &&
-                           (c.debugFlags & ~(PT_DEBUG_UNFUSED_ROUNDS | PT_DEBUG_TRAVERSAL_PHASED | PT_DEBUG_LOCKSTEP | PT_DEBUG_GATHER_LOCAL_ONLY | PT_DEBUG_GATHER_SELF_EXCHANGE | PT_DEBUG_SHARC_LOG_PATHS | PT_DEBUG_SHARC_SKIP_UPDATE)) == 0;
+                           (c.debugFlags & ~(PT_DEBUG_UNFUSED_ROUNDS | PT_DEBUG_TRAVERSAL_PHASED | PT_DEBUG_LOCKSTEP | PT_DEBUG_GATHER_LOCAL_ONLY | PT_DEBUG_GATHER_SELF_EXCHANGE | PT_DEBUG_SHARC_LOG_PATHS | PT_DEBUG_SHARC_SKIP_UPDATE | PT_DEBUG_PACKED_PRIMARY)) == 0;
     auto capture = [&](hipStream_t s, GraphExec& exec, auto&& body) -> hipError_t {
         if (exec) { hipStreamSynchronize(c.stream); exec.reset(); }
         hipGraph_t graph = nullptr;
diff --git a/directx-physically-based-raytracer_amd/csrc/pt_math.hpp b/directx-physically-based-raytracer_amd/csrc/pt_math.hpp
--- a/directx-physically-based-raytracer_amd/csrc/pt_math.hpp
+++ b/directx-physically-based-raytracer_amd/csrc/pt_math.hpp
@@ -276,6 +276,17 @@
         float r = (IORi - IORo) / (IORi + IORo);
         float r2 = r * r;
         F0 = V3(mad(metallic, baseColor.x - r2, r2), mad(metallic, baseColor.y - r2, r2), mad(metallic, baseColor.z - r2, r2));
+        Transmission = transmission;
+    }
+    PT_DEV void Restore(v3 baseColor, float metallic, float roughness, float IOR, float transmission, bool isFrontFace, v3 f0)
+    {
+        BaseColor = baseColor;
+        Metallic = metallic;
+        Albedo = baseColor * (1.0f - metallic);
+        Roughness = roughness;
+        IORi = 1.0f; IORo = IOR;
+        if (!isFrontFace) { IORi = IOR; IORo = 1.0f; }
+        F0 = f0;
         Transmission = transmission;
     }
 
diff --git a/directx-physically-based-raytracer_amd/csrc/pt_shade.hpp b/directx-physically-based-raytracer_amd/csrc/pt_shade.hpp
--- a/directx-physically-based-raytracer_amd/csrc/pt_shade.hpp
+++ b/directx-physically-based-raytracer_amd/csrc/pt_shade.hpp
@@ -395,32 +395,78 @@
     else toFresh = end_sample<DI, SHARC>(gs, tx, aux, p);
 }
 
-template <bool DI = false, bool SHARC = false>
-PT_DEV void shade_fresh_record(const FrameView& fv, const PtCamera& cam, const PtGraphicsSettings& gs, const PtTextures& tx, float2* aux, uint4 r0, uint4 r1, uint4 r2,
-                               PathRegs& p, bool& toTraced, bool& toFresh, v3& newO, v3& newD, float* previousRoughness = nullptr)
-{
-    const uint32_t pixel = p.pixel;
+struct PrimarySurface {
+    v3 Position; float PositionOffset;
+    v3 RayDirection, FlatNormal, GeometricNormal, ShadingNormal;
+    v3 BaseColor, F0; float Metallic, Roughness, IOR, Transmission;
+    uint32_t Radiance01, Radiance2;
+};
+constexpr uint32_t kPrimaryPacked16 = 3, kPrimaryDecoded16 = 7;
+
+PT_DEV PrimarySurface decode_primary(const FrameView& fv, const PtCamera& cam, uint32_t pixel, uint4 r0, uint4 r1, uint4 r2)
+{
     const uint32_t px = pixel % fv.width, py = global_row(fv, pixel / fv.width);
     float uu, vv;
     const RayDesc primaryRay = generate_pinhole_ray(cam, px, py, fv.width, fv.height, uu, vv);
-    const v3 rayDir = primaryRay.d;
     const float4 pos = make_float4(__uint_as_float(r0.x), __uint_as_float(r0.y), __uint_as_float(r0.z), __uint_as_float(r0.w));
     const short4 nr = make_short4((short)(r1.x & 0xFFFFu), (short)(r1.x >> 16), (short)(r1.y & 0xFFFFu), (short)(r1.y >> 16));
     const short2 fe = make_short2((short)(r1.z & 0xFFFFu), (short)(r1.z >> 16)), ge = make_short2((short)(r1.w & 0xFFFFu), (short)(r1.w >> 16));
     const uchar4 bcm = make_uchar4((unsigned char)(r2.x & 0xFFu), (unsigned char)((r2.x >> 8) & 0xFFu), (unsigned char)((r2.x >> 16) & 0xFFu), (unsigned char)(r2.x >> 24));
-    const ushort4 rad = make_ushort4((unsigned short)(r2.y & 0xFFFFu), (unsigned short)(r2.y >> 16), (unsigned short)(r2.z & 0xFFFFu), (unsigned short)(r2.z >> 16));
-    SurfaceHit h;
-    h.Position = V3(pos.x, pos.y, pos.z); h.PositionOffset = pos.w;
-    h.FlatNormal = oct_decode(snorm16_to_f32(fe.x), snorm16_to_f32(fe.y));
-    h.GeometricNormal = oct_decode(snorm16_to_f32(ge.x), snorm16_to_f32(ge.y));
-    h.ShadingNormal = V3(snorm16_to_f32(nr.x), snorm16_to_f32(nr.y), snorm16_to_f32(nr.z));
-    h.IsFrontFace = dot(h.GeometricNormal, rayDir) < 0.0f;
-    const v3 emission = V3(f16_to_f32(rad.x), f16_to_f32(rad.y), f16_to_f32(rad.z));
+    PrimarySurface s;
+    s.RayDirection = primaryRay.d;
+    s.Position = V3(pos.x, pos.y, pos.z); s.PositionOffset = pos.w;
+    s.FlatNormal = oct_decode(snorm16_to_f32(fe.x), snorm16_to_f32(fe.y));
+    s.GeometricNormal = oct_decode(snorm16_to_f32(ge.x), snorm16_to_f32(ge.y));
+    s.ShadingNormal = V3(snorm16_to_f32(nr.x), snorm16_to_f32(nr.y), snorm16_to_f32(nr.z));
+    const bool isFrontFace = dot(s.GeometricNormal, s.RayDirection) < 0.0f;
     const float metal = unorm8_to_f32(bcm.w);
     const float ior = f16_to_f32((uint16_t)(r2.w & 0xFFFFu));
     const float tr = metal < 1.0f ? unorm8_to_f32((uint8_t)((r2.w >> 16) & 0xFFu)) : 0.0f;
     BSDFSample bs;
-    bs.Initialize(V3(unorm8_to_f32(bcm.x), unorm8_to_f32(bcm.y), unorm8_to_f32(bcm.z)), metal, snorm16_to_f32(nr.w), ior, tr, h.IsFrontFace);
+    bs.Initialize(V3(unorm8_to_f32(bcm.x), unorm8_to_f32(bcm.y), unorm8_to_f32(bcm.z)), metal, snorm16_to_f32(nr.w), ior, tr, isFrontFace);
+    s.BaseColor = bs.BaseColor; s.F0 = bs.F0; s.Metallic = bs.Metallic; s.Roughness = bs.Roughness; s.IOR = ior; s.Transmission = bs.Transmission;
+    s.Radiance01 = r2.y; s.Radiance2 = r2.z;
+    return s;
+}
+
+PT_DEV void store_primary_decoded(uint4* __restrict__ primary, uint32_t pixel, const PrimarySurface& s)
+{
+    float4* d = (float4*)primary + kPrimaryDecoded16 * (size_t)pixel;
+    d[0] = make_float4(s.Position.x, s.Position.y, s.Position.z, s.PositionOffset);
+    d[1] = make_float4(s.RayDirection.x, s.RayDirection.y, s.RayDirection.z, s.Roughness);
+    d[2] = make_float4(s.FlatNormal.x, s.FlatNormal.y, s.FlatNormal.z, s.Metallic);
+    d[3] = make_float4(s.GeometricNormal.x, s.GeometricNormal.y, s.GeometricNormal.z, s.IOR);
+    d[4] = make_float4(s.ShadingNormal.x, s.ShadingNormal.y, s.ShadingNormal.z, s.Transmission);
+    d[5] = make_float4(s.BaseColor.x, s.BaseColor.y, s.BaseColor.z, __uint_as_float(s.Radiance01));
+    d[6] = make_float4(s.F0.x, s.F0.y, s.F0.z, __uint_as_float(s.Radiance2));
+}
+PT_DEV PrimarySurface load_primary_decoded(const uint4* __restrict__ primary, uint32_t pixel)
+{
+    const float4* d = (const float4*)primary + kPrimaryDecoded16 * (size_t)pixel;
+    const float4 a = d[0], b = d[1], c = d[2], e = d[3], f = d[4], g = d[5], h = d[6];
+    PrimarySurface s;
+    s.Position = V3(a.x, a.y, a.z); s.PositionOffset = a.w;
+    s.RayDirection = V3(b.x, b.y, b.z); s.Roughness = b.w;
+    s.FlatNormal = V3(c.x, c.y, c.z); s.Metallic = c.w;
+    s.GeometricNormal = V3(e.x, e.y, e.z); s.IOR = e.w;
+    s.ShadingNormal = V3(f.x, f.y, f.z); s.Transmission = f.w;
+    s.BaseColor = V3(g.x, g.y, g.z); s.Radiance01 = __float_as_uint(g.w);
+    s.F0 = V3(h.x, h.y, h.z); s.Radiance2 = __float_as_uint(h.w);
+    return s;
+}
+
+template <bool DI = false, bool SHARC = false>
+PT_DEV void shade_primary(const PtGraphicsSettings& gs, const PtTextures& tx, float2* aux, const PrimarySurface& s,
+                          PathRegs& p, bool& toTraced, bool& toFresh, v3& newO, v3& newD, float* previousRoughness = nullptr)
+{
+    const v3 rayDir = s.RayDirection;
+    SurfaceHit h;
+    h.Position = s.Position; h.PositionOffset = s.PositionOffset;
+    h.FlatNormal = s.FlatNormal; h.GeometricNormal = s.GeometricNormal; h.ShadingNormal = s.ShadingNormal;
+    h.IsFrontFace = dot(h.GeometricNormal, rayDir) < 0.0f;
+    const v3 emission = V3(f16_to_f32((uint16_t)(s.Radiance01 & 0xFFFFu)), f16_to_f32((uint16_t)(s.Radiance01 >> 16)), f16_to_f32((uint16_t)(s.Radiance2 & 0xFFFFu)));
+    BSDFSample bs;
+    bs.Restore(s.BaseColor, s.Metallic, s.Roughness, s.IOR, s.Transmission, h.IsFrontFace, s.F0);
     int lobe = 0;
     const bool first = p.sample == 0;
     if constexpr (SHARC) {
@@ -434,13 +480,20 @@
 }
 
 template <bool DI = false, bool SHARC = false>
-PT_DEV void shade_fresh(const FrameView& fv, const PtCamera& cam, const PtGraphicsSettings& gs, const PtTextures& tx, float2* aux, const uint4* __restrict__ primary,
+PT_DEV void shade_fresh(const FrameView& fv, const PtCamera& cam, const PtGraphicsSettings& gs, const PtTextures& tx, float2* aux, const uint4* __restrict__ primary, bool decoded,
                         PathRegs& p, bool& toTraced, bool& toFresh, v3& newO, v3& newD, RoundProf* prof = nullptr, float* previousRoughness = nullptr)
 {
     const uint32_t pixel = p.pixel;
-    const uint4 r0 = primary[3 * (size_t)pixel], r1 = primary[3 * (size_t)pixel + 1], r2 = primary[3 * (size_t)pixel + 2];
-    PT_PROF_WAIT(); PT_PROF_MARK(prof, 13);
-    shade_fresh_record<DI, SHARC>(fv, cam, gs, tx, aux, r0, r1, r2, p, toTraced, toFresh, newO, newD, previousRoughness);
+    PrimarySurface s;
+    if (decoded) {
+        s = load_primary_decoded(primary, pixel);
+        PT_PROF_WAIT(); PT_PROF_MARK(prof, 13);
+    } else {
+        const uint4 r0 = primary[3 * (size_t)pixel], r1 = primary[3 * (size_t)pixel + 1], r2 = primary[3 * (size_t)pixel + 2];
+        PT_PROF_WAIT(); PT_PROF_MARK(prof, 13);
+        s = decode_primary(fv, cam, pixel, r0, r1, r2);
+    }
+    shade_primary<DI, SHARC>(gs, tx, aux, s, p, toTraced, toFresh, newO, newD, previousRoughness);
 }
 
 template <bool SHARC = false>
diff --git a/directx-physically-based-raytracer_amd/csrc/pt_stream.hip b/directx-physically-based-raytracer_amd/csrc/pt_stream.hip
--- a/directx-physically-based-raytracer_amd/csrc/pt_stream.hip
+++ b/directx-physically-based-raytracer_amd/csrc/pt_stream.hip
@@ -6,7 +6,7 @@
 __global__ __launch_bounds__(256) __attribute__((amdgpu_waves_per_eu(4, 4))) void k_shade(SceneView sv, FrameView fv, const FrameConstants* __restrict__ fc, PtTextures tx,
                                                PathQueue qin, PathQueue qout, float2* aux, uint32_t segCap, const uint32_t* countIn, uint32_t* countOut,
                                                const uint4* __restrict__ primary, BlobView bv, const uint4* __restrict__ recA, const uint32_t* __restrict__ recB, uint32_t sqShift,
-                                               uint32_t sqBase, uint32_t sqCount, const SharcView* sharc = nullptr, const float* roughIn = nullptr, float* roughOut = nullptr)
+                                               uint32_t sqBase, uint32_t sqCount, uint32_t primaryDecoded, const SharcView* sharc = nullptr, const float* roughIn = nullptr, float* roughOut = nullptr)
 {
     BlobReader<false> blob; blob.p = bv.base;
     ShadeTables tables; tables.recA = recA; tables.recB = recB;
@@ -39,7 +39,7 @@
         float pr = 0.0f;
         if (local < nF) {
             p = load_path(qin, seg + (segCap - 1u - local));
-            shade_fresh<DI, SHARC>(fv, cam, gs, tx, aux, primary, p, toTraced, toFresh, newO, newD, nullptr, &pr);
+            shade_fresh<DI, SHARC>(fv, cam, gs, tx, aux, primary, primaryDecoded != 0u, p, toTraced, toFresh, newO, newD, nullptr, &pr);
         }
         emit_tile<SHARC>(qout, seg, segCap, &countOut[sq], &countOut[nsq + sq], lds + ((emits++ & 1u) << 4), toTraced, toFresh, p, newO, newD, roughOut, pr);
     }
@@ -241,7 +241,7 @@
     const uint32_t* countIn = &c.queueCounts.data()[round * p.cstride()]; uint32_t* countOut = &c.queueCounts.data()[(round + 1u) * p.cstride()];
     with_flags([&](auto D, auto T, auto S) {
         k_shade<T(), D(), S()><<<grid, 256, 0, stream>>>(sv, fv, c.frameConstants.data(), tx, c.queue[qi], c.queue[qi ^ 1u], p.aux, p.segCap, countIn, countOut, c.primaryRecords.data(), c.scene.blob,
-                                                       recA, recB, p.sqShift, sqBase, sqCount, S() ? c.sharcView.data() : nullptr, S() ? c.sharcRough[qi].data() : nullptr, S() ? c.sharcRough[qi ^ 1u].data() : nullptr);
+                                                       recA, recB, p.sqShift, sqBase, sqCount, p.primaryDecoded ? 1u : 0u, S() ? c.sharcView.data() : nullptr, S() ? c.sharcRough[qi].data() : nullptr, S() ? c.sharcRough[qi ^ 1u].data() : nullptr);
     }, p.di, p.textured, p.sharc);
     return hipGetLastError();
 }
diff --git a/directx-physically-based-raytracer_amd/layouts.py b/directx-physically-based-raytracer_amd/layouts.py
--- a/directx-physically-based-raytracer_amd/layouts.py
+++ b/directx-physically-based-raytracer_amd/layouts.py
@@ -249,6 +249,7 @@
     "offsets": [0, 96, 108, 112, 124], "itemsize": 128})
 SHARC_VERTEX_HIT, SHARC_VERTEX_MISS, SHARC_VERTEX_ENDED, SHARC_VERTEX_RESAMPLED = 1, 2, 4, 8
 DEBUG_SHARC_LOG_PATHS, DEBUG_SHARC_SKIP_UPDATE = 0x100, 0x200
+DEBUG_PACKED_PRIMARY = 0x800
 
 
 def check_sharc_settings(s):
diff --git a/directx-physically-based-raytracer_amd/ptamd.py b/directx-physically-based-raytracer_amd/ptamd.py
--- a/directx-physically-based-raytracer_amd/ptamd.py
+++ b/directx-physically-based-raytracer_amd/ptamd.py
@@ -12,7 +12,7 @@
 EXPORTS = [
     "pt_abi_version", "pt_create", "pt_destroy", "pt_last_error", "pt_set_stream", "pt_sync", "pt_set_frames_in_flight", "pt_set_round_chains",
     "pt_heap_resize", "pt_heap_set_buffer", "pt_heap_set_texture", "pt_build_bottom_level", "pt_update_bottom_level", "pt_release_bottom_level", "pt_skin_mesh",
-    "pt_build_top_level", "pt_get_accel_stats", "pt_share_scene", "pt_set_camera", "pt_set_scene_data", "pt_set_object_data", "pt_invalidate_object_data",
+    "pt_build_top_level", "pt_get_accel_stats", "pt_get_shading_record_stats", "pt_share_scene", "pt_set_camera", "pt_set_scene_data", "pt_set_object_data", "pt_invalidate_object_data",
     "pt_set_instance_data", "pt_set_sharding", "pt_local_rows", "pt_deinterleave_bands", "pt_gbuffer_render",
     "pt_comm_get_unique_id", "pt_comm_init", "pt_comm_adopt", "pt_comm_destroy", "pt_gather_bands", "pt_gather_plan",
     "pt_raytrace_set_constants", "pt_raytrace_render", "pt_trace_visibility", "pt_bsdf_evaluate", "pt_bsdf_sample", "pt_reset_counters", "pt_get_counters",
@@ -86,6 +86,10 @@
                 ("TriangleSizeBytes", C.c_uint32), ("MaxBottomLevelDepth", C.c_uint32), ("TopLevelDepth", C.c_uint32),
                 ("BlobBytes", C.c_uint64), ("SharedScene", C.c_uint32), ("NormalRecords", C.c_uint32),
                 ("OwnedBottomLevelBytes", C.c_uint64), ("RoundObjectsInLds", C.c_uint32), ("RoundRecordsInLds", C.c_uint32)]
+
+
+class ShadingRecordStats(C.Structure):
+    _fields_ = [("PrimaryRecordsDecoded", C.c_uint32), ("PrimaryRecordBytes", C.c_uint32)]
 
 
 _BSDF_MATERIAL = [("BaseColor", C.c_float * 3), ("Metallic", C.c_float), ("Roughness", C.c_float), ("IOR", C.c_float),
@@ -139,6 +143,7 @@
         lib.pt_skin_mesh.argtypes = [C.c_void_p, C.c_void_p, C.c_void_p, C.c_void_p, C.c_void_p, C.c_uint32]
         lib.pt_build_top_level.argtypes = [C.c_void_p, C.c_void_p, C.c_uint32, C.c_uint32]
         lib.pt_get_accel_stats.argtypes = [C.c_void_p, C.c_void_p]
+        lib.pt_get_shading_record_stats.argtypes = [C.c_void_p, C.c_void_p]
         lib.pt_share_scene.argtypes = [C.c_void_p, C.c_void_p]
         for f in (lib.pt_set_camera, lib.pt_set_scene_data, lib.pt_set_sharding, lib.pt_raytrace_set_constants,
                   lib.pt_raytrace_render, lib.pt_get_counters):
@@ -309,6 +314,11 @@
         self.check(self.lib.pt_get_accel_stats(self.handle, C.byref(s)))
         return s
 
+    def shading_record_stats(self):
+        s = ShadingRecordStats()
+        self.check(self.lib.pt_get_shading_record_stats(self.handle, C.byref(s)))
+        return s
+
     @staticmethod
     def comm_unique_id():
         lib = load_library()
diff --git a/include/ptamd.h b/include/ptamd.h
--- a/include/ptamd.h
+++ b/include/ptamd.h
@@ -188,6 +188,12 @@
     uint32_t RoundObjectsInLds, RoundRecordsInLds;
 } PtAccelStats;
 int  pt_get_accel_stats(PtContext* ctx, PtAccelStats* out);
+
+typedef struct PtShadingRecordStats {
+    uint32_t PrimaryRecordsDecoded;
+    uint32_t PrimaryRecordBytes;
+} PtShadingRecordStats;
+int  pt_get_shading_record_stats(PtContext* ctx, PtShadingRecordStats* out);
 
 int  pt_share_scene(PtContext* ctx, PtContext* source);
 
@@ -413,6 +419,7 @@
 #define PT_DEBUG_GATHER_SELF_EXCHANGE 0x80u
 #define PT_DEBUG_SHARC_LOG_PATHS 0x100u
 #define PT_DEBUG_SHARC_SKIP_UPDATE 0x200u
+#define PT_DEBUG_PACKED_PRIMARY  0x800u
 int  pt_set_debug_flags(PtContext* ctx, uint32_t flags);
 int  pt_debug_read_mismatch(PtContext* ctx, float* out16);
 
```

New measurement: 11530. -4.8%, worse.
